# jbelyeu/unfazed

Measured on NVIDIA B200. Metric: DNMs phased/sec, higher is better.
Workload: dtype int32/u8 + f64 allele balance

## Files before the change

include/unfazed_sm100.h:

```cpp
#ifndef UNFAZED_SM100_H
#define UNFAZED_SM100_H

#include <stdint.h>

#ifdef __cplusplus
extern "C" {
#endif

#define UNFZ_ABI_VERSION 2

#define UNFZ_CLS_HET        0x01
#define UNFZ_CLS_CAND       0x02
#define UNFZ_CLS_ALT_IS_DAD 0x04
#define UNFZ_CLS_KID_ALT    0x08

#define UNFZ_MODE_READ    0
#define UNFZ_MODE_CNV_DEL 1
#define UNFZ_MODE_CNV_DUP 2
#define UNFZ_MODE_CNV_NA  3

#define UNFZ_RS_GOOD_CONC 0x01
#define UNFZ_RS_GOOD_DISC 0x02
#define UNFZ_RS_NONE_OK   0x04
#define UNFZ_RS_EXT_OK    0x08
#define UNFZ_RS_INS_OK    0x10
#define UNFZ_RS_HAS_MATE  0x20

#define UNFZ_KIND_SKIP  0
#define UNFZ_KIND_SNV   1
#define UNFZ_KIND_INDEL 2
#define UNFZ_KIND_SV    3

#define UNFZ_ORIGIN_NONE 0
#define UNFZ_ORIGIN_DAD  1
#define UNFZ_ORIGIN_MOM  2
#define UNFZ_ORIGIN_BOTH 3

#define UNFZ_EV_READBACKED        0x01
#define UNFZ_EV_ALLELE_BALANCE    0x02
#define UNFZ_EV_AMBIG_READBACKED  0x04
#define UNFZ_EV_AMBIG_ALLELE_BAL  0x08
#define UNFZ_EV_AMBIG_BOTH        0x10
#define UNFZ_EV_SEX_CHROM         0x20

typedef struct {
    int64_t         n_rows;
    int32_t         n_blocks;
    int32_t         _pad;
    const int64_t*  blk_off;
    const int32_t*  pos;
    const uint8_t*  ref;
    const uint8_t*  alt;
    const uint32_t* meta;
    const float*    rec;
    const int32_t*  dep;
} UnfzSiteCols;

typedef struct {
    int32_t  start;
    int32_t  tlen;
    int32_t  mate;
    uint32_t cigar_off;
    uint32_t qoff_lo;
    int32_t  l_seq;
    uint16_t flag;
    uint16_t n_cigar;
    uint8_t  mapq;
    uint8_t  aux;
    uint8_t  qoff_hi;
    uint8_t  pad;
} UnfzRead;

typedef struct {
    int64_t         n_reads;
    int32_t         n_blocks;
    int32_t         _pad;
    const int64_t*  blk_off;
    const int32_t*  blk_sblk;
    const double*   blk_cul;
    const UnfzRead* hdr;
    const int32_t*  start;
    const uint32_t* cigar;
    const uint32_t* lowq;
    const uint32_t* nmask;
    const uint8_t*  seq2;
    int64_t         n_qual;
    int64_t         n_cigar;
} UnfzReadCols;

typedef struct {
    int32_t  end;
    int32_t  fmark;
    uint16_t flags;
    uint16_t cnt;
    uint32_t hoff;
    int32_t  start;
    int32_t  mate;
    int32_t  row_lb;
    int32_t  _pad;
} UnfzReadSum;

typedef struct {
    double  ab_homref[2];
    double  ab_homalt[2];
    double  ab_het[2];
    double  min_gt_qual;
    int32_t min_depth;
    int32_t min_map_qual;
    int32_t readlen;
    int32_t ext_read_goal;
    int32_t no_extended;
    int32_t evidence_min_ratio;
    int32_t split_error_margin;
    int32_t _pad;
} UnfzParams;

typedef struct {
    int32_t sblk;
    int32_t lo_pos;
    int32_t hi_pos;
    int32_t mult;
    int32_t dnm;
    int32_t excl_lo;
    int32_t excl_hi;
    int32_t mode;
} UnfzSegIn;

typedef struct {
    int32_t pos;
    int32_t end;
    int32_t rblk;
    int32_t kind;
    int32_t seg_lo;
    int32_t seg_hi;
    int32_t ref_off;
    int32_t ref_len;
    int32_t alt_off;
    int32_t alt_len;
    int32_t cnv_entry;
    int32_t flags;
} UnfzDnm;

typedef struct {
    int32_t n_dad_sites, n_mom_sites;
    int32_t n_dad_reads, n_mom_reads;
    int32_t cnv_dad, cnv_mom;
    int32_t has_record;
    int32_t status;
} UnfzTally;

typedef struct {
    int32_t origin;
    int32_t evidence_count;
    int32_t evidence_types;
    int32_t emitted;
} UnfzCall;

typedef struct UnfzCtx UnfzCtx;

int         unfz_abi_version(void);
int         unfz_ctx_create(int device, UnfzCtx** out);
void        unfz_ctx_destroy(UnfzCtx* ctx);
const char* unfz_last_error(UnfzCtx* ctx);

int unfz_ctx_set_guard(UnfzCtx*, const int32_t* flag);
int unfz_check_caps(UnfzCtx*, int32_t k, const int64_t* const* h_totals, const int64_t* h_caps, int32_t* flag,
                    int64_t* actual, void* stream);

int64_t unfz_scan_work_bytes(int64_t n);
int unfz_exclusive_scan_i64(UnfzCtx*, const int64_t* in, int64_t* out, int64_t n, void* work, void* stream);
int unfz_exclusive_scan_u8_i32(UnfzCtx*, const uint8_t* in, int32_t* out, int64_t n, void* work, void* stream);
int unfz_exclusive_scan_u32(UnfzCtx*, const uint32_t* in, uint32_t* out , int64_t n, int64_t* total_out,
                            void* work, void* stream);
int unfz_exclusive_scan_rows_i64(UnfzCtx*, const int64_t* in, int64_t* out, int32_t n_rows, int64_t n, void* stream);

int unfz_window_search(UnfzCtx*, const UnfzSiteCols* sites, const UnfzSegIn* segs, int32_t n_segs,
                       int32_t* seg_row_lo, int64_t* seg_count, void* stream);

int unfz_classify_sites(UnfzCtx*, const UnfzSiteCols* sites, const UnfzSegIn* segs,
                        const int32_t* seg_row_lo, const int64_t* seg_pair_off, int32_t n_segs,
                        int64_t n_pairs, const UnfzParams* h_params, uint8_t* out_class, void* stream);

int unfz_compact_sites(UnfzCtx*, const UnfzDnm* dnms, int32_t n_dnms, const UnfzSegIn* segs,
                       const int32_t* seg_row_lo, const int64_t* seg_pair_off, const uint8_t* cls,
                       int32_t* het_list, int32_t* n_het, uint32_t* cand_list, int32_t* n_cand,
                       int32_t* cnv_dad, int32_t* cnv_mom, uint8_t* row_mark, void* stream);

int unfz_pack_site_rows(UnfzCtx*, int64_t n_rows, const int32_t* pos, const uint8_t* flag, const uint8_t* gt,
                        const float* gq, const int32_t* rd, const int32_t* ad, uint32_t* meta, float* rec,
                        int32_t* dep, void* stream);

int unfz_expand_nlist(UnfzCtx*, const UnfzReadCols* reads, UnfzRead* hdr_rw, uint32_t* nmask_rw,
                      const int64_t* nidx, int64_t n_idx, void* stream);
int unfz_read_starts(UnfzCtx*, const UnfzReadCols* reads, int32_t* start_rw, void* stream);

int32_t unfz_read_scan_tile_reads(int32_t max_l_seq);
int unfz_read_scan(UnfzCtx*, const UnfzReadCols* reads, const UnfzSiteCols* sites,
                   const int32_t* mark_prefix, const UnfzParams* h_params,
                   int32_t max_l_seq , UnfzReadSum* out,
                   int32_t* blk_maxspan ,
                   uint32_t* tile_tot ,
                   uint32_t* tile_info ,
                   void* stream);

int unfz_read_site_alleles(UnfzCtx*, const UnfzReadCols* reads, const UnfzSiteCols* sites,
                           const uint8_t* row_mark, const int32_t* mark_prefix,
                           const UnfzReadSum* rsum, const uint32_t* tile_base,
                           int32_t tile_reads, uint32_t* hits, const uint32_t* tile_info ,
                           void* stream);

int unfz_chain_size(UnfzCtx*, const UnfzDnm* dnms, int32_t n_dnms, const UnfzSegIn* segs,
                    const int64_t* seg_pair_off, const UnfzSiteCols* sites,
                    const UnfzReadCols* reads, const UnfzReadSum* rsum, const int32_t* blk_maxspan,
                    const int32_t* het_list, const int32_t* n_het, const uint32_t* cand_list,
                    const int32_t* n_cand, int32_t* win ,
                    int64_t* need,
                    int32_t* site_lo, int32_t* site_n ,
                    int32_t* seed_win , void* stream);

int unfz_chain_tally(UnfzCtx*, const UnfzDnm* dnms, int32_t n_dnms, const UnfzSegIn* segs,
                     const int64_t* seg_pair_off, const UnfzSiteCols* sites,
                     const UnfzReadCols* reads, const UnfzReadSum* rsum, const int32_t* blk_maxspan,
                     const uint32_t* hits, const uint32_t* hit_tile_base, int32_t hit_tile_reads,
                     const int32_t* mark_prefix,
                     const int32_t* het_list, const int32_t* n_het, const uint32_t* cand_list,
                     const int32_t* n_cand, const uint8_t* alleles, const int32_t* win,
                     const int32_t* site_lo, const int32_t* site_n, const int32_t* seed_win, const int64_t* off, const int64_t* h_totals ,
                     const UnfzParams* h_params, void* scratch, int64_t scratch_bytes,
                     uint8_t* slot_label, uint8_t* slot_evid, uint8_t* cand_evid,
                     UnfzTally* tally,
                     int64_t* ev_need ,
                     void* stream);

int unfz_evidence_lists(UnfzCtx*, const UnfzDnm* dnms, int32_t n_dnms, const int64_t* seg_pair_off,
                        const UnfzSiteCols* sites, const uint32_t* cand_list, const int32_t* n_cand,
                        const uint8_t* cand_evid, const int32_t* win, const int64_t* slot_off,
                        const uint8_t* slot_evid, const int64_t* ev_off, int32_t* ev_read_dad, int32_t* ev_read_mom,
                        int32_t* ev_pos_dad, int32_t* ev_pos_mom, void* stream);
int64_t unfz_chain_scratch_bytes(int64_t slots, int64_t incs, int64_t seeds, int64_t seed_incs,
                                 int64_t het_sites, int64_t cand_sites, int64_t n_dnms);

int64_t unfz_insert_size_work_bytes(void);
int unfz_insert_size_order_stats(UnfzCtx*, const UnfzReadCols* reads, const int64_t* h_first, const int64_t* h_count,
                                 int32_t n_ranges, int32_t readlen, const uint64_t* h_ranks, void* work,
                                 uint32_t* out, void* stream);

int unfz_summarize(UnfzCtx*, const UnfzDnm* dnms, int32_t n_dnms, const UnfzTally* tally,
                   const int32_t* cnv_dad, const int32_t* cnv_mom, const int32_t* n_cand,
                   const UnfzParams* h_params,
                   UnfzCall* calls_strict, UnfzCall* calls_ambiguous, void* stream);

typedef struct {
    const UnfzSiteCols* sites;
    const UnfzReadCols* reads;
    const UnfzParams*   h_params;
    const UnfzDnm*  dnms;     int32_t n_dnms;  int32_t n_segs;
    const UnfzSegIn* segs;    const uint8_t* alleles;
    int32_t max_l_seq;        int32_t tile_reads;
    int64_t n_tiles;
    int64_t cap_pairs, cap_hits, cap_chain[6];
    int32_t* seg_row_lo;  int64_t* seg_count;  int64_t* seg_pair_off;  void* scan_work;
    uint8_t* row_mark;    int32_t* mark_prefix;
    int32_t* guard;       int64_t* actual;
    int32_t* n_het;  int32_t* n_cand;  int32_t* cnv_dad;  int32_t* cnv_mom;
    UnfzTally* tally;  UnfzCall* calls_strict;  UnfzCall* calls_ambiguous;  int32_t* win;
    int32_t* blk_maxspan;  int64_t* need;  int64_t* off;
    UnfzReadSum* rsum;  uint32_t* tile_tot;  uint32_t* tile_base;  uint32_t* tile_info;
    uint8_t* cls;  int32_t* het_list;  uint32_t* cand_list;  int32_t* site_lo;  int32_t* site_n;  int32_t* seed_win;
    uint8_t* cand_evid;
    uint32_t* hits;  void* scratch;  int64_t scratch_bytes;  uint8_t* slot_label;  uint8_t* slot_evid;
    int64_t* ev_need;  int64_t* ev_off;  int32_t* ev_read_dad;  int32_t* ev_read_mom;  int32_t* ev_pos_dad;  int32_t* ev_pos_mom;
} UnfzBatch;
int unfz_run_batch(UnfzCtx*, const UnfzBatch* h_batch, void* stream);

typedef struct { void* ptr; int64_t bytes; } UnfzSpan;
int unfz_run_batch_graph(UnfzCtx*, const UnfzBatch* h_batch, const UnfzSpan* h_zero, int32_t n_zero,
                         void* h_dst, const void* d_src, int64_t d2h_bytes, void* stream);
int unfz_batch_struct_bytes(void);

#ifdef __cplusplus
}
#endif
#endif
```

unfazed_b200/_lib.py:

```python
from __future__ import annotations

import ctypes as C
import os

import numpy as np

_HERE = os.path.dirname(os.path.abspath(__file__))
LIB_PATH = os.environ.get("UNFZ_LIB") or os.path.join(_HERE, "libunfazed_sm100.so")

c_void_p, c_int32, c_int64, c_double = C.c_void_p, C.c_int32, C.c_int64, C.c_double


class SiteCols(C.Structure):
    _fields_ = [
        ("n_rows", c_int64), ("n_blocks", c_int32), ("_pad", c_int32),
        ("blk_off", c_void_p), ("pos", c_void_p), ("ref", c_void_p), ("alt", c_void_p),
        ("meta", c_void_p), ("rec", c_void_p), ("dep", c_void_p),
    ]


class ReadCols(C.Structure):
    _fields_ = [
        ("n_reads", c_int64), ("n_blocks", c_int32), ("_pad", c_int32),
        ("blk_off", c_void_p), ("blk_sblk", c_void_p), ("blk_cul", c_void_p),
        ("hdr", c_void_p), ("start", c_void_p), ("cigar", c_void_p), ("lowq", c_void_p), ("nmask", c_void_p), ("seq2", c_void_p),
        ("n_qual", c_int64), ("n_cigar", c_int64),
    ]


class Params(C.Structure):
    _fields_ = [
        ("ab_homref", c_double * 2), ("ab_homalt", c_double * 2), ("ab_het", c_double * 2),
        ("min_gt_qual", c_double),
        ("min_depth", c_int32), ("min_map_qual", c_int32), ("readlen", c_int32),
        ("ext_read_goal", c_int32), ("no_extended", c_int32), ("evidence_min_ratio", c_int32),
        ("split_error_margin", c_int32), ("_pad", c_int32),
    ]


class Batch(C.Structure):
    _fields_ = [
        ("sites", c_void_p), ("reads", c_void_p), ("h_params", c_void_p),
        ("dnms", c_void_p), ("n_dnms", c_int32), ("n_segs", c_int32),
        ("segs", c_void_p), ("alleles", c_void_p),
        ("max_l_seq", c_int32), ("tile_reads", c_int32),
        ("n_tiles", c_int64),
        ("cap_pairs", c_int64), ("cap_hits", c_int64), ("cap_chain", c_int64 * 6),
        ("seg_row_lo", c_void_p), ("seg_count", c_void_p), ("seg_pair_off", c_void_p), ("scan_work", c_void_p),
        ("row_mark", c_void_p), ("mark_prefix", c_void_p),
        ("guard", c_void_p), ("actual", c_void_p),
        ("n_het", c_void_p), ("n_cand", c_void_p), ("cnv_dad", c_void_p), ("cnv_mom", c_void_p),
        ("tally", c_void_p), ("calls_strict", c_void_p), ("calls_ambiguous", c_void_p), ("win", c_void_p),
        ("blk_maxspan", c_void_p), ("need", c_void_p), ("off", c_void_p),
        ("rsum", c_void_p), ("tile_tot", c_void_p), ("tile_base", c_void_p), ("tile_info", c_void_p),
        ("cls", c_void_p), ("het_list", c_void_p), ("cand_list", c_void_p), ("site_lo", c_void_p), ("site_n", c_void_p),
        ("seed_win", c_void_p), ("cand_evid", c_void_p),
        ("hits", c_void_p), ("scratch", c_void_p), ("scratch_bytes", c_int64), ("slot_label", c_void_p), ("slot_evid", c_void_p),
        ("ev_need", c_void_p), ("ev_off", c_void_p), ("ev_read_dad", c_void_p), ("ev_read_mom", c_void_p),
        ("ev_pos_dad", c_void_p), ("ev_pos_mom", c_void_p),
    ]


class Span(C.Structure):
    _fields_ = [("ptr", c_void_p), ("bytes", c_int64)]


SEG_DTYPE = np.dtype([
    ("sblk", "<i4"), ("lo_pos", "<i4"), ("hi_pos", "<i4"), ("mult", "<i4"),
    ("dnm", "<i4"), ("excl_lo", "<i4"), ("excl_hi", "<i4"), ("mode", "<i4"),
])
DNM_DTYPE = np.dtype([
    ("pos", "<i4"), ("end", "<i4"), ("rblk", "<i4"), ("kind", "<i4"), ("seg_lo", "<i4"), ("seg_hi", "<i4"),
    ("ref_off", "<i4"), ("ref_len", "<i4"), ("alt_off", "<i4"), ("alt_len", "<i4"),
    ("cnv_entry", "<i4"), ("flags", "<i4"),
])
TALLY_DTYPE = np.dtype([
    ("n_dad_sites", "<i4"), ("n_mom_sites", "<i4"), ("n_dad_reads", "<i4"), ("n_mom_reads", "<i4"),
    ("cnv_dad", "<i4"), ("cnv_mom", "<i4"), ("has_record", "<i4"), ("status", "<i4"),
])
CALL_DTYPE = np.dtype([("origin", "<i4"), ("evidence_count", "<i4"), ("evidence_types", "<i4"), ("emitted", "<i4")])
RSUM_DTYPE = np.dtype([("end", "<i4"), ("fmark", "<i4"), ("flags", "<u2"), ("cnt", "<u2"), ("hoff", "<u4"),
                       ("start", "<i4"), ("mate", "<i4"), ("row_lb", "<i4"), ("pad", "<i4")])
assert SEG_DTYPE.itemsize == 32 and DNM_DTYPE.itemsize == 48 and RSUM_DTYPE.itemsize == 32

CLS_HET, CLS_CAND, CLS_ALT_IS_DAD, CLS_KID_ALT = 1, 2, 4, 8
MODE_READ, MODE_CNV_DEL, MODE_CNV_DUP, MODE_CNV_NA = 0, 1, 2, 3
KIND_SKIP, KIND_SNV, KIND_INDEL, KIND_SV = 0, 1, 2, 3
ORIGIN_NONE, ORIGIN_DAD, ORIGIN_MOM, ORIGIN_BOTH = 0, 1, 2, 3
EV_READBACKED, EV_ALLELE_BALANCE, EV_AMBIG_READBACKED, EV_AMBIG_ALLELE_BAL, EV_AMBIG_BOTH, EV_SEX_CHROM = 1, 2, 4, 8, 16, 32
DNM_AUTOPHASE, DNM_AUTOPHASE_Y, DNM_SV_QUIRK, DNM_FALLBACK_FETCH = 1, 2, 4, 8
ABI_VERSION = 2
RS_GOOD_CONC, RS_GOOD_DISC, RS_NONE_OK, RS_EXT_OK, RS_INS_OK, RS_HAS_MATE = 1, 2, 4, 8, 16, 32

_P = c_void_p
SYMBOLS = {
    "unfz_abi_version": (C.c_int, []),
    "unfz_ctx_create": (C.c_int, [C.c_int, C.POINTER(_P)]),
    "unfz_ctx_destroy": (None, [_P]),
    "unfz_last_error": (C.c_char_p, [_P]),
    "unfz_ctx_set_guard": (C.c_int, [_P, _P]),
    "unfz_check_caps": (C.c_int, [_P, c_int32, _P, _P, _P, _P, _P]),
    "unfz_run_batch": (C.c_int, [_P, C.POINTER(Batch), _P]),
    "unfz_run_batch_graph": (C.c_int, [_P, C.POINTER(Batch), _P, c_int32, _P, _P, c_int64, _P]),
    "unfz_batch_struct_bytes": (C.c_int, []),
    "unfz_scan_work_bytes": (c_int64, [c_int64]),
    "unfz_exclusive_scan_i64": (C.c_int, [_P, _P, _P, c_int64, _P, _P]),
    "unfz_exclusive_scan_u8_i32": (C.c_int, [_P, _P, _P, c_int64, _P, _P]),
    "unfz_exclusive_scan_u32": (C.c_int, [_P, _P, _P, c_int64, _P, _P, _P]),
    "unfz_exclusive_scan_rows_i64": (C.c_int, [_P, _P, _P, c_int32, c_int64, _P]),
    "unfz_window_search": (C.c_int, [_P, C.POINTER(SiteCols), _P, c_int32, _P, _P, _P]),
    "unfz_classify_sites": (C.c_int, [_P, C.POINTER(SiteCols), _P, _P, _P, c_int32, c_int64, C.POINTER(Params), _P, _P]),
    "unfz_compact_sites": (C.c_int, [_P, _P, c_int32, _P, _P, _P, _P, _P, _P, _P, _P, _P, _P, _P, _P]),
    "unfz_pack_site_rows": (C.c_int, [_P, c_int64, _P, _P, _P, _P, _P, _P, _P, _P, _P, _P]),
    "unfz_expand_nlist": (C.c_int, [_P, C.POINTER(ReadCols), _P, _P, _P, c_int64, _P]),
    "unfz_read_scan_tile_reads": (c_int32, [c_int32]),
    "unfz_read_scan": (C.c_int, [_P, C.POINTER(ReadCols), C.POINTER(SiteCols), _P, C.POINTER(Params), c_int32, _P, _P, _P, _P, _P]),
    "unfz_read_site_alleles": (C.c_int, [_P, C.POINTER(ReadCols), C.POINTER(SiteCols), _P, _P, _P, _P, c_int32, _P, _P, _P]),
    "unfz_read_starts": (C.c_int, [_P, C.POINTER(ReadCols), _P, _P]),
    "unfz_chain_size": (C.c_int, [_P, _P, c_int32, _P, _P, C.POINTER(SiteCols), C.POINTER(ReadCols), _P, _P,
                                  _P, _P, _P, _P, _P, _P, _P, _P, _P, _P]),
    "unfz_chain_scratch_bytes": (c_int64, [c_int64] * 7),
    "unfz_chain_tally": (C.c_int, [_P, _P, c_int32, _P, _P, C.POINTER(SiteCols), C.POINTER(ReadCols), _P, _P, _P, _P, c_int32, _P,
                                   _P, _P, _P, _P, _P, _P, _P, _P, _P, _P, _P, C.POINTER(Params), _P, c_int64,
                                   _P, _P, _P, _P, _P, _P]),
    "unfz_evidence_lists": (C.c_int, [_P, _P, c_int32, _P, C.POINTER(SiteCols), _P, _P, _P, _P, _P, _P, _P, _P, _P, _P, _P, _P]),
    "unfz_insert_size_work_bytes": (c_int64, []),
    "unfz_insert_size_order_stats": (C.c_int, [_P, C.POINTER(ReadCols), _P, _P, c_int32, c_int32, _P, _P, _P, _P]),
    "unfz_summarize": (C.c_int, [_P, _P, c_int32, _P, _P, _P, _P, C.POINTER(Params), _P, _P, _P]),
}

_lib = None


class LibraryMissing(RuntimeError):
    pass


def load():
    global _lib
    if _lib is not None:
        return _lib
    if not os.path.exists(LIB_PATH):
        raise LibraryMissing(
            "%s not found: build it with `python -c 'import __graft_entry__ as g; g.build()'` "
            "or `make -C unfazed_b200/csrc`" % LIB_PATH)
    lib = C.CDLL(LIB_PATH)
    for name, (res, args) in SYMBOLS.items():
        fn = getattr(lib, name)
        fn.restype = res
        fn.argtypes = args
    if lib.unfz_abi_version() != ABI_VERSION:
        raise LibraryMissing("ABI version mismatch in %s" % LIB_PATH)
    if lib.unfz_batch_struct_bytes() != C.sizeof(Batch):
        raise LibraryMissing("UnfzBatch layout mismatch between %s and _lib.Batch" % LIB_PATH)
    _lib = lib
    return lib
```

unfazed_b200/csrc/abi.cu:

```cuda
#include <stdlib.h>

#include "common.cuh"

extern "C" int unfz_abi_version(void) { return UNFZ_ABI_VERSION; }

extern "C" int unfz_ctx_create(int device, UnfzCtx** out) {
    if (!out) return -1;
    *out = nullptr;
    int count = 0;
    if (cudaGetDeviceCount(&count) != cudaSuccess || device < 0 || device >= count) return -2;
    cudaDeviceProp prop;
    if (cudaGetDeviceProperties(&prop, device) != cudaSuccess) return -3;
    if (prop.major < 10) return -4;
    if (cudaSetDevice(device) != cudaSuccess) return -5;
    UnfzCtx* c = new UnfzCtx();
    c->device = device;
    c->sm_count = prop.multiProcessorCount;
    c->guard = nullptr;
    c->scan_smem_attr = 0;
    c->chain_carveout_set = false;
    c->cls_params = nullptr;
    c->cls_tab_dev = nullptr;
    memset(c->graphs, 0, sizeof(c->graphs));
    c->graph_tick = 0;
    c->err[0] = 0;
    *out = c;
    return 0;
}

extern "C" void unfz_ctx_destroy(UnfzCtx* ctx) {
    if (!ctx) return;
    for (auto& g : ctx->graphs)
        if (g.key) cudaGraphExecDestroy(g.exec);
    free(ctx->cls_params);
    if (ctx->cls_tab_dev) cudaFree(ctx->cls_tab_dev);
    delete ctx;
}

extern "C" const char* unfz_last_error(UnfzCtx* ctx) { return ctx ? ctx->err : "null context"; }

namespace {
struct CapArgs {
    const int64_t* totals[8];
    int64_t caps[8];
};
__global__ void check_caps_kernel(CapArgs a, int k, int32_t* flag, int64_t* actual) {
    const int i = threadIdx.x;
    if (i < k) {
        const int64_t v = *a.totals[i];
        actual[i] = v;
        if (v > a.caps[i]) atomicOr(flag, 1);
    }
}
}

extern "C" int unfz_ctx_set_guard(UnfzCtx* ctx, const int32_t* flag) {
    if (!ctx) return -1;
    ctx->guard = flag;
    return 0;
}

extern "C" int unfz_check_caps(UnfzCtx* ctx, int32_t k, const int64_t* const* totals, const int64_t* caps,
                               int32_t* flag, int64_t* actual, void* stream) {
    if (k < 0 || k > 8) return unfz_fail(ctx, -30, "unfz_check_caps: at most 8 totals");
    if (k == 0) return 0;
    CapArgs a;
    for (int i = 0; i < 8; ++i) { a.totals[i] = i < k ? totals[i] : nullptr; a.caps[i] = i < k ? caps[i] : 0; }
    check_caps_kernel<<<1, 32, 0, (cudaStream_t)stream>>>(a, k, flag, actual);
    UNFZ_LAUNCH_CHECK(ctx);
    return 0;
}

#define UNFZ_RC(expr) do { const int rc_ = (expr); if (rc_ != 0) { ctx->guard = nullptr; return rc_; } } while (0)

extern "C" int unfz_batch_struct_bytes(void) { return (int)sizeof(UnfzBatch); }

extern "C" int unfz_run_batch(UnfzCtx* ctx, const UnfzBatch* b, void* s) {
    if (!ctx || !b) return -1;
    const int32_t n = b->n_dnms, S = b->n_segs;
    const int64_t V = b->sites->n_rows;
    ctx->guard = b->guard;
    UNFZ_RC(unfz_window_search(ctx, b->sites, b->segs, S, b->seg_row_lo, b->seg_count, s));
    UNFZ_RC(unfz_exclusive_scan_i64(ctx, b->seg_count, b->seg_pair_off, S, b->scan_work, s));
    {
        const int64_t* t[1] = {b->seg_pair_off + S};
        const int64_t c[1] = {b->cap_pairs};
        UNFZ_RC(unfz_check_caps(ctx, 1, t, c, b->guard, b->actual, s));
    }
    UNFZ_RC(unfz_classify_sites(ctx, b->sites, b->segs, b->seg_row_lo, b->seg_pair_off, S, b->cap_pairs, b->h_params, b->cls, s));
    UNFZ_RC(unfz_compact_sites(ctx, b->dnms, n, b->segs, b->seg_row_lo, b->seg_pair_off, b->cls, b->het_list, b->n_het,
                               b->cand_list, b->n_cand, b->cnv_dad, b->cnv_mom, b->row_mark, s));
    UNFZ_RC(unfz_exclusive_scan_u8_i32(ctx, b->row_mark, b->mark_prefix, V, b->scan_work, s));
    if (b->reads != nullptr) {
        int64_t* total_hits = b->off + 6 * ((int64_t)n + 1);
        UNFZ_RC(unfz_read_scan(ctx, b->reads, b->sites, b->mark_prefix, b->h_params, b->max_l_seq, b->rsum,
                               b->blk_maxspan, b->tile_tot, b->tile_info, s));
        UNFZ_RC(unfz_exclusive_scan_u32(ctx, b->tile_tot, b->tile_base, b->n_tiles, total_hits, b->scan_work, s));
        UNFZ_RC(unfz_chain_size(ctx, b->dnms, n, b->segs, b->seg_pair_off, b->sites, b->reads, b->rsum, b->blk_maxspan,
                                b->het_list, b->n_het, b->cand_list, b->n_cand, b->win, b->need, b->site_lo, b->site_n,
                                b->seed_win, s));
        UNFZ_RC(unfz_exclusive_scan_rows_i64(ctx, b->need, b->off, 6, n, s));
        {
            const int64_t* t[7];
            int64_t c[7];
            for (int i = 0; i < 6; ++i) { t[i] = b->off + (int64_t)(i + 1) * (n + 1) - 1; c[i] = b->cap_chain[i]; }
            t[6] = total_hits;
            c[6] = b->cap_hits;
            UNFZ_RC(unfz_check_caps(ctx, 7, t, c, b->guard, b->actual + 1, s));
        }
        UNFZ_RC(unfz_read_site_alleles(ctx, b->reads, b->sites, b->row_mark, b->mark_prefix, b->rsum, b->tile_base,
                                       b->tile_reads, b->hits, b->tile_info, s));
        UNFZ_RC(unfz_chain_tally(ctx, b->dnms, n, b->segs, b->seg_pair_off, b->sites, b->reads, b->rsum, b->blk_maxspan,
                                 b->hits, b->tile_base, b->tile_reads, b->mark_prefix, b->het_list, b->n_het, b->cand_list,
                                 b->n_cand, b->alleles, b->win, b->site_lo, b->site_n, b->seed_win, b->off, b->cap_chain,
                                 b->h_params, b->scratch, b->scratch_bytes, b->slot_label, b->slot_evid, b->cand_evid,
                                 b->tally, b->ev_need, s));
        if (b->ev_need != nullptr) {
            UNFZ_RC(unfz_exclusive_scan_rows_i64(ctx, b->ev_need, b->ev_off, 4, n, s));
            UNFZ_RC(unfz_evidence_lists(ctx, b->dnms, n, b->seg_pair_off, b->sites, b->cand_list, b->n_cand, b->cand_evid,
                                        b->win, b->off, b->slot_evid, b->ev_off, b->ev_read_dad, b->ev_read_mom, b->ev_pos_dad,
                                        b->ev_pos_mom, s));
        }
    }
    UNFZ_RC(unfz_summarize(ctx, b->dnms, n, b->tally, b->cnv_dad, b->cnv_mom, b->n_cand, b->h_params, b->calls_strict,
                           b->calls_ambiguous, s));
    ctx->guard = nullptr;
    return 0;
}

static uint64_t fnv1a(uint64_t h, const void* p, size_t n) {
    const unsigned char* b = static_cast<const unsigned char*>(p);
    for (size_t i = 0; i < n; ++i) { h ^= b[i]; h *= 1099511628211ull; }
    return h;
}

extern "C" int unfz_run_batch_graph(UnfzCtx* ctx, const UnfzBatch* b, const UnfzSpan* zero, int32_t n_zero,
                                    void* h_dst, const void* d_src, int64_t d2h_bytes, void* stream) {
    if (!ctx || !b) return -1;
    cudaStream_t s = (cudaStream_t)stream;
    uint64_t key = 1469598103934665603ull;
    key = fnv1a(key, b, sizeof(*b));
    key = fnv1a(key, b->sites, sizeof(*b->sites));
    if (b->reads) key = fnv1a(key, b->reads, sizeof(*b->reads));
    key = fnv1a(key, b->h_params, sizeof(*b->h_params));
    key = fnv1a(key, zero, sizeof(UnfzSpan) * (size_t)(n_zero > 0 ? n_zero : 0));
    key = fnv1a(key, &h_dst, sizeof(h_dst));
    key = fnv1a(key, &d_src, sizeof(d_src));
    key = fnv1a(key, &d2h_bytes, sizeof(d2h_bytes));
    if (key == 0) key = 1;
    UnfzGraphSlot* slot = nullptr;
    UnfzGraphSlot* victim = nullptr;
    for (auto& g : ctx->graphs) {
        if (g.key == key) { slot = &g; break; }
        if (!victim || (victim->key != 0 && (g.key == 0 || g.tick < victim->tick))) victim = &g;
    }
    if (!slot) {
        cudaGraph_t graph = nullptr;
        { const int rc0 = unfz_classify_prepare(ctx, b->h_params); if (rc0) return rc0; }
        UNFZ_CHECK(ctx, cudaStreamBeginCapture(s, cudaStreamCaptureModeThreadLocal));
        int rc = 0;
        for (int i = 0; i < n_zero && rc == 0; ++i)
            if (zero[i].bytes > 0 && cudaMemsetAsync(zero[i].ptr, 0, (size_t)zero[i].bytes, s) != cudaSuccess) rc = -40;
        if (rc == 0) rc = unfz_run_batch(ctx, b, s);
        if (rc == 0 && d2h_bytes > 0 && cudaMemcpyAsync(h_dst, d_src, (size_t)d2h_bytes, cudaMemcpyDeviceToHost, s) != cudaSuccess) rc = -41;
        const cudaError_t e = cudaStreamEndCapture(s, &graph);
        if (rc != 0 || e != cudaSuccess) {
            if (graph) cudaGraphDestroy(graph);
            cudaGetLastError();
            return rc != 0 ? rc : unfz_fail(ctx, -42, "unfz_run_batch_graph: stream capture failed (legacy default stream?)");
        }
        cudaGraphExec_t exec = nullptr;
        const cudaError_t ei = cudaGraphInstantiate(&exec, graph, 0);
        cudaGraphDestroy(graph);
        if (ei != cudaSuccess) return unfz_fail(ctx, -43, cudaGetErrorString(ei));
        if (victim->key) cudaGraphExecDestroy(victim->exec);
        victim->key = key;
        victim->exec = exec;
        slot = victim;
    }
    slot->tick = ++ctx->graph_tick;
    UNFZ_CHECK(ctx, cudaGraphLaunch(slot->exec, s));
    return 0;
}
```

unfazed_b200/csrc/chain.cu:

```cuda
#include <stdlib.h>

#include <type_traits>

#include "common.cuh"

namespace {

constexpr unsigned long long KEY_NONE = ~0ull;
#ifndef UNFZ_CHAIN_WIDE_MIN_INC
#define UNFZ_CHAIN_WIDE_MIN_INC 2048
#endif
constexpr int CH_SMEM_SITES = 128;

struct __align__(16) SlotRec {
    unsigned long long key;
    int32_t dense;
    int32_t pad;
};

struct Scratch {
    SlotRec* slot;
    int32_t* inc_r; int32_t* inc_x; int32_t* inc_site; uint8_t* inc_al;
    int32_t* seed_e; uint8_t* seed_hap; uint32_t* seed_reg;
    int32_t* sinc_px; int32_t* sinc_site; uint32_t* sinc_sidx; uint8_t* sinc_al;
    int32_t* x_of; int32_t* prim;
    uint32_t* p_ord; int32_t* p_fpos; int32_t* p_tmp; unsigned long long* p_minkey; uint8_t* p_label;
    int32_t* adj; int32_t* adj_off; int32_t* front0; int32_t* front1;
    int32_t* spos; uint8_t* sref; uint8_t* salt; int32_t* site_off; int32_t* cand_off;
    unsigned long long* bestkey; int32_t* site_cnt; int32_t* site_base; int32_t* active;
    int32_t* cpos;
    int32_t* meta;
};

struct ChainArgs {
    const UnfzDnm* dnms; int32_t n_dnms;
    const UnfzSegIn* segs; const int64_t* seg_pair_off;
    UnfzSiteCols sites; UnfzReadCols reads;
    const UnfzReadSum* rsum; const int32_t* blk_maxspan; const uint32_t* hits; const int32_t* mp;
    const int32_t* het_list; const int32_t* n_het; const uint32_t* cand_list; const int32_t* n_cand;
    const uint8_t* alleles; const int32_t* win; const int64_t* off;
    int32_t split_margin;
    const uint32_t* hit_tile_base; int32_t hit_tile_reads;
    const int32_t* site_lo; const int32_t* site_n; const int32_t* seed_win;
    int32_t readlen, ext_goal, no_extended;
    uint8_t* slot_label; uint8_t* slot_evid; uint8_t* cand_evid; UnfzTally* tally;
    int64_t* ev_need;
    const int32_t* guard;
    Scratch S;
};

#ifdef CH_PREFETCH
__device__ __forceinline__ void prefetch_l2(const void* p) { asm volatile("prefetch.global.L2 [%0];" ::"l"(p)); }
#endif

__device__ __forceinline__ int32_t rs_start(const UnfzReadSum* __restrict__ S, int64_t r) { return __ldg(&S[r].start); }
__device__ __forceinline__ int32_t rs_mate(const UnfzReadSum* __restrict__ S, int64_t r) { return __ldg(&S[r].mate); }

__device__ __forceinline__ int64_t lb_start(const int32_t* __restrict__ R, int64_t lo, int64_t hi, int64_t v) {
    while (lo < hi) {
        const int64_t mid = (lo + hi) >> 1;
        if ((int64_t)__ldg(R + mid) < v) lo = mid + 1; else hi = mid;
    }
    return lo;
}

__device__ __forceinline__ int cigar_qpos2(const uint32_t* __restrict__ cg, int n_cigar, int32_t start, int32_t p) {
    int32_t cur = start;
    int q = 0;
    for (int k = 0; k < n_cigar; ++k) {
        const uint32_t w = __ldg(cg + k);
        const uint32_t op = w & 15u;
        const int32_t ln = (int32_t)(w >> 4);
        if (op == 0 || op == 7 || op == 8) {
            if (p < cur + ln) return p >= cur ? q + (p - cur) : -1;
            cur += ln; q += ln;
        } else if (op == 1 || op == 4) {
            q += ln;
        } else if (op == 2 || op == 3) {
            if (p < cur + ln) return -1;
            cur += ln;
        }
    }
    return -1;
}

__device__ __forceinline__ uint32_t plane_bit(const uint32_t* __restrict__ plane, int64_t g) {
    return (__ldg(plane + (g >> 5)) >> (g & 31)) & 1u;
}
__device__ __forceinline__ char base_char(const UnfzReadCols& R, int64_t g) {
    const uint32_t code = (__ldg(R.seq2 + (g >> 2)) >> ((g & 3) << 1)) & 3u;
    if (plane_bit(R.nmask, g)) return code == 0 ? 'N' : '?';
    return "ACGT"[code];
}
__device__ __forceinline__ char hit_char(uint32_t w) {
    const uint32_t code = (w >> 24) & 3u;
    if (w & (0x80u << 16)) return code == 0 ? 'N' : '?';
    return "ACGT"[code];
}

__device__ __forceinline__ uint32_t hit_lookup(const ChainArgs& A, int64_t e, int64_t row) {
    const UnfzReadSum s = load_rsum(A.rsum + e);
    const int mp = __ldg(A.mp + row);
    const uint32_t tb = __ldg(A.hit_tile_base + (uint32_t)e / (uint32_t)A.hit_tile_reads);
    const int k = mp - s.fmark;
    if (k < 0 || k >= (int)s.cnt) return 0;
    return __ldg(A.hits + (int64_t)tb + s.hoff + k);
}

__device__ bool pair_ok(const ChainArgs& A, int64_t r, bool ext) {
    const UnfzReadSum s = load_rsum(A.rsum + r);
    uint32_t need = UNFZ_RS_GOOD_CONC | UNFZ_RS_INS_OK | UNFZ_RS_HAS_MATE | UNFZ_RS_NONE_OK;
    if (ext) need |= UNFZ_RS_EXT_OK;
    const bool ok_r = (s.flags & need) == need;
    const int64_t m = ok_r ? (int64_t)s.mate : r;
    const UnfzReadSum sm = load_rsum(A.rsum + m);
    const uint32_t needm = UNFZ_RS_GOOD_CONC | UNFZ_RS_NONE_OK;
    const int32_t r0 = s.start, r1 = s.end, m0 = sm.start, m1 = sm.end;
    return ok_r && (sm.flags & needm) == needm && !((m0 <= r0 && r0 <= m1) || (m0 <= r1 && r1 <= m1));
}

struct QPos { int q; int l_seq; int64_t g0; int32_t mate; };
__device__ __forceinline__ QPos qpos_of(const ChainArgs& A, int64_t e, int32_t p) {
    const UnfzRead h = load_read(A.reads.hdr + e);
    QPos o;
    if (h.aux & 0x40u) o.q = (p >= h.start && p < h.start + h.l_seq) ? (int)(p - h.start) : -1;
    else o.q = cigar_qpos2(A.reads.cigar + h.cigar_off, h.n_cigar, h.start, p);
    o.l_seq = h.l_seq;
    o.g0 = read_qoff(h);
    o.mate = h.mate;
    return o;
}

__device__ int seed_snv(const ChainArgs& A, const UnfzDnm& dn, int64_t r) {
    QPos h = qpos_of(A, r, dn.pos);
    int q = h.q;
    if (q < 0) {
        h = qpos_of(A, h.mate, dn.pos);
        q = h.q;
        if (q < 0) return 0;
    }
    if (q < 4 || q > A.readlen - 4) return 0;
    const int n = dn.ref_len > dn.alt_len ? dn.ref_len : dn.alt_len;
    if (!(h.l_seq > q + n)) return 0;
    const int64_t g = h.g0 + q;
    bool is_ref = true;
    for (int i = 0; i < dn.ref_len; ++i)
        if (base_char(A.reads, g + i) != (char)A.alleles[dn.ref_off + i]) { is_ref = false; break; }
    if (is_ref) return 1;
    bool is_alt = true;
    for (int i = 0; i < dn.alt_len; ++i)
        if (base_char(A.reads, g + i) != (char)A.alleles[dn.alt_off + i]) { is_alt = false; break; }
    return is_alt ? 2 : 0;
}

__device__ int seed_indel(const ChainArgs& A, const UnfzDnm& dn, int64_t r) {
    const UnfzRead h = load_read(A.reads.hdr + r);
    const uint32_t* cg = A.reads.cigar + h.cigar_off;
    const bool simple = (h.aux & 0x40u) != 0;
    const int q = simple ? ((dn.pos >= h.start && dn.pos < h.start + h.l_seq) ? (int)(dn.pos - h.start) : -1)
                         : cigar_qpos2(cg, h.n_cigar, h.start, dn.pos);
    if (q < 0) return 0;
    const int n = dn.ref_len > dn.alt_len ? dn.ref_len : dn.alt_len;
    const int64_t g0 = read_qoff(h);
    for (int i = q; i < q + n && i < h.l_seq; ++i)
        if (plane_bit(A.reads.lowq, g0 + i)) return 0;
    if (simple) return (7 < q && q < h.l_seq - 7) ? 1 : 0;
    bool has_id = false;
    int64_t eo = 0, npos = 0;
    for (int k = 0; k < h.n_cigar; ++k) {
        const uint32_t w = __ldg(cg + k);
        const uint32_t op = w & 15u;
        const int64_t ln = w >> 4;
        if ((op == 1 || op == 2) && eo < (int64_t)q + n && eo + ln > q) has_id = true;
        eo += ln;
        if (op == 0 || op == 1 || op == 4 || op == 7 || op == 8) npos += ln;
    }
    if (has_id) return 2;
    if (7 < q && q < npos - 7) return 1;
    return 0;
}


__device__ bool sv_bad_ends(const uint32_t* __restrict__ cg, int n) {
    int s_m = 0, left = 10;
    for (int k = 0; k < n && left > 0; ++k) {
        const uint32_t w = __ldg(cg + k);
        const int take = min(left, (int)(w >> 4));
        if ((w & 15u) == 0 || (w & 15u) == 7) s_m += take;
        left -= take;
    }
    int e_m = 0;
    left = 10;
    for (int k = n - 1; k >= 0 && left > 0; --k) {
        const uint32_t w = __ldg(cg + k);
        const int take = min(left, (int)(w >> 4));
        if ((w & 15u) == 0 || (w & 15u) == 7) e_m += take;
        left -= take;
    }
    return e_m < 7 && s_m < 7;
}

__device__ bool sv_goodok(const ChainArgs& A, int64_t r) {
    const UnfzReadSum s = load_rsum(A.rsum + r);
    const uint32_t need = UNFZ_RS_GOOD_DISC | UNFZ_RS_HAS_MATE;
    if ((s.flags & need) != need) return false;
    const int64_t m = rs_mate(A.rsum, r);
    return (load_rsum(A.rsum + m).flags & UNFZ_RS_GOOD_DISC) != 0;
}

__device__ bool sv_banned(const ChainArgs& A, int64_t r) {
    if (!sv_goodok(A, r)) return false;
    const UnfzRead h = load_read(A.reads.hdr + r);
    return sv_bad_ends(A.reads.cigar + h.cigar_off, h.n_cigar);
}

__device__ int sv_support(const ChainArgs& A, const UnfzDnm& dn, int64_t r, int64_t position, double cul) {
    const UnfzRead h = load_read(A.reads.hdr + r);
    const UnfzReadSum s = load_rsum(A.rsum + r);
    const int64_t r0 = h.start, r1 = s.end;
    if (h.aux & 2u) {
        const int64_t em = A.split_margin;
        if ((position - em <= r0 && r0 <= position + em) || (position - em <= r1 && r1 <= position + em)) return 1;
        return 0;
    }
    long long ins = (long long)h.tlen - 2ll * A.readlen;
    if (ins < 0) ins = -ins;
    const double var_len = fabs((double)dn.end - (double)dn.pos);
    if ((double)ins > cul) {
        const double ratio = fabs(var_len / (double)ins);
        if (0.7 < ratio && ratio < 1.3) {
            const int64_t m0 = rs_start(A.rsum, h.mate);
            const int64_t left0 = min(m0, r0), right0 = max(m0, r0);
            const int64_t w = (int64_t)cul;
            if ((dn.pos - w) < left0 && left0 < (dn.pos + w) && (dn.end - w) < right0 && right0 < (dn.end + w)) return 2;
            return 0;
        }
    }
    const uint32_t* cg = A.reads.cigar + h.cigar_off;
    int k = cigar_qpos2(cg, h.n_cigar, h.start, (int32_t)position);
    if (k < 0) k = cigar_qpos2(cg, h.n_cigar, h.start, (int32_t)position - 1);
    if (k < 0) k = cigar_qpos2(cg, h.n_cigar, h.start, (int32_t)position + 1);
    if (k < 0) return 0;
    int64_t npos = 0, lead = 0, trail = 0;
    bool seen = false;
    for (int i = 0; i < h.n_cigar; ++i) {
        const uint32_t w = __ldg(cg + i);
        const uint32_t op = w & 15u;
        const int64_t ln = w >> 4;
        if (op == 0 || op == 7 || op == 8) { npos += ln; seen = true; trail = 0; }
        else if (op == 1 || op == 4) { npos += ln; if (!seen) lead += ln; else trail += ln; }
    }
    if (k < 2 || k > npos - 4) return 0;
    const int64_t first_al = lead, last_al = npos - 1 - trail;
    const bool before_none = first_al >= k - 1;
    const bool after_none = (k + 1 < npos) && last_al <= k;
    return (before_none || after_none) ? 2 : 0;
}


__device__ int bisect_pivot(const int32_t* __restrict__ spos, int n, int32_t start, int32_t end) {
    int lo = 0, hi = n - 1, plo = -1, phi = -1;
    while (hi > -1) {
        if (lo > hi) break;
        if (lo == plo && hi == phi) break;
        plo = lo; phi = hi;
        const int mid = (hi + lo) / 2;
        const int32_t x = spos[mid];
        if (start <= x && x < end) return mid;
        else if (x > start) hi = mid - 1;
        else if (x < start) lo = mid + 1;
    }
    return -1;
}

__device__ uint8_t allele_info(const ChainArgs& A, const Scratch& S, int64_t e0, int64_t row, char ref, char alt) {
    if (e0 < 0) return 0;
    const int64_t e1 = rs_mate(A.rsum, e0);
    const uint32_t h0 = hit_lookup(A, e0, row);
    uint32_t h = h0;
    if (!(h0 & 0xffffu)) {
        if (e1 < 0) return 0;
        h = hit_lookup(A, e1, row);
        if (!(h & 0xffffu)) return 0;
    }
    const int q = (int)(h & 0xffffu) - 1;
    if (q < 4 || q > A.readlen - 4) return 0;
    if (!(h & (1u << 26))) return 0;
    const char c = hit_char(h);
    const uint8_t code = c == ref ? 1 : (c == alt ? 2 : 0);
    if (!code) return 0;
    uint8_t out = code;
    if ((h0 & 0xffffu) && !(h0 & (1u << 16))) out |= code << 2;
    return out;
}

#ifdef CH_DEBUG
__device__ unsigned long long g_ch_dbg[16];
#define CH_MARK(i) do { if (threadIdx.x == 0) { const long long t_ = clock64(); atomicAdd(&g_ch_dbg[i], (unsigned long long)(t_ - ch_t0)); ch_t0 = t_; } } while (0)
#else
#define CH_MARK(i)
#endif

#ifndef CH_THREADS_N
#define CH_THREADS_N 128
#endif
#ifndef CH_MINB
#define CH_MINB 16
#endif
#ifndef CH_BFS_MINB
#define CH_BFS_MINB 8
#endif
#define CH_NS cta_small
#include "chain_cta.inc"
#undef CH_NS
#undef CH_THREADS_N
#undef CH_MINB
#undef CH_BFS_MINB
#define CH_NS cta_wide
#define CH_THREADS_N 512
#define CH_MINB 4
#define CH_BFS_MINB 2
#include "chain_cta.inc"
#undef CH_NS
#undef CH_THREADS_N
#undef CH_MINB
#undef CH_BFS_MINB


__global__ void __launch_bounds__(128)
evidence_lists_kernel(const UnfzDnm* __restrict__ dnms, int32_t n_dnms, const int64_t* __restrict__ seg_pair_off,
                      const int32_t* __restrict__ site_pos, const uint32_t* __restrict__ cand_list,
                      const int32_t* __restrict__ n_cand, const uint8_t* __restrict__ cand_evid,
                      const int32_t* __restrict__ win, const int64_t* __restrict__ slot_off,
                      const uint8_t* __restrict__ slot_evid, const int64_t* __restrict__ ev_off,
                      int32_t* __restrict__ ev_read_dad, int32_t* __restrict__ ev_read_mom,
                      int32_t* __restrict__ ev_pos_dad, int32_t* __restrict__ ev_pos_mom,
                      const int32_t* __restrict__ guard) {
    UNFZ_GUARD(guard);
    const int lane = threadIdx.x & 31;
    const int d = (blockIdx.x * blockDim.x + threadIdx.x) >> 5;
    if (d >= n_dnms) return;
    const unsigned below = (1u << lane) - 1u;
    const int64_t n1 = (int64_t)n_dnms + 1;
    int64_t kd = ev_off[d], km = ev_off[n1 + d];
    if (ev_off[d + 1] > kd || ev_off[n1 + d + 1] > km) {
        const int64_t nd = n_dnms;
        const int64_t a_lo = win[d], a_hi = win[nd + d], b_lo = win[2 * nd + d], b_hi = win[3 * nd + d];
        const int na = (int)(a_hi - a_lo), W = na + (int)(b_hi - b_lo);
        const uint8_t* ev = slot_evid + slot_off[d];
        for (int x0 = 0; x0 < W; x0 += 32) {
            const int x = x0 + lane;
            const uint8_t e = x < W ? ev[x] : 0;
            const int32_t r = (int32_t)(x < na ? a_lo + x : b_lo + (x - na));
            const unsigned bd = __ballot_sync(0xffffffffu, e & 1), bm = __ballot_sync(0xffffffffu, e & 2);
            if (e & 1) ev_read_dad[kd + __popc(bd & below)] = r;
            if (e & 2) ev_read_mom[km + __popc(bm & below)] = r;
            kd += __popc(bd);
            km += __popc(bm);
        }
    }
    kd = ev_off[2 * n1 + d];
    km = ev_off[3 * n1 + d];
    if (ev_off[2 * n1 + d + 1] > kd || ev_off[3 * n1 + d + 1] > km) {
        const UnfzDnm dn = dnms[d];
        const int64_t lbase = seg_pair_off[dn.seg_lo];
        const int nc = n_cand[d];
        for (int j0 = 0; j0 < nc; j0 += 32) {
            const int j = j0 + lane;
            const uint8_t e = j < nc ? cand_evid[lbase + j] : 0;
            const int32_t p = e ? __ldg(site_pos + (int64_t)(cand_list[lbase + j] & 0x3fffffffu)) : 0;
            const unsigned bd = __ballot_sync(0xffffffffu, e & 1), bm = __ballot_sync(0xffffffffu, e & 2);
            if (e & 1) ev_pos_dad[kd + __popc(bd & below)] = p;
            if (e & 2) ev_pos_mom[km + __popc(bm & below)] = p;
            kd += __popc(bd);
            km += __popc(bm);
        }
    }
}

__device__ __forceinline__ int64_t warp_sum64(int64_t v) {
#pragma unroll
    for (int o = 16; o > 0; o >>= 1) v += __shfl_xor_sync(0xffffffffu, v, o);
    return v;
}
__device__ __forceinline__ int64_t warp_min64(int64_t v) {
#pragma unroll
    for (int o = 16; o > 0; o >>= 1) v = min(v, __shfl_xor_sync(0xffffffffu, v, o));
    return v;
}
__device__ __forceinline__ int64_t warp_max64(int64_t v) {
#pragma unroll
    for (int o = 16; o > 0; o >>= 1) v = max(v, __shfl_xor_sync(0xffffffffu, v, o));
    return v;
}

__device__ __forceinline__ int64_t warp_lb_start(const int32_t* __restrict__ R, int64_t lo, int64_t hi, int64_t v, int lane) {
    while (hi - lo > 32) {
        const int64_t step = (hi - lo + 32) / 33;
        const int64_t i = lo + (int64_t)(lane + 1) * step - 1;
        const bool lt = i < hi && (int64_t)__ldg(R + i) < v;
        const int k = __popc(__ballot_sync(0xffffffffu, lt));
        const int64_t nhi = k < 32 ? min(hi, lo + (int64_t)(k + 1) * step - 1) : hi;
        lo += (int64_t)k * step;
        hi = nhi;
    }
    const bool lt = lo + lane < hi && (int64_t)__ldg(R + lo + lane) < v;
    return lo + __popc(__ballot_sync(0xffffffffu, lt));
}
__device__ __forceinline__ int64_t lb_start_near(const int32_t* __restrict__ R, int64_t lo, int64_t hi, int64_t v) {
    int64_t step = 32, top = lo;
    while (top + step < hi && (int64_t)__ldg(R + top + step - 1) < v) { top += step; step <<= 1; }
    return lb_start(R, top, min(hi, top + step), v);
}

constexpr int CS_HP = 128;

__global__ void __launch_bounds__(128)
chain_size_kernel(const UnfzDnm* __restrict__ dnms, int32_t n_dnms, const int64_t* __restrict__ seg_pair_off,
                  UnfzSiteCols sites, UnfzReadCols reads, const UnfzReadSum* __restrict__ rsum,
                  const int32_t* __restrict__ blk_maxspan, const int32_t* __restrict__ het_list,
                  const int32_t* __restrict__ n_het, const uint32_t* __restrict__ cand_list,
                  const int32_t* __restrict__ n_cand, int32_t* __restrict__ win, int64_t* __restrict__ need,
                  int32_t* __restrict__ site_lo, int32_t* __restrict__ site_n, int32_t* __restrict__ seed_win,
                  const int32_t* __restrict__ guard) {
    UNFZ_GUARD(guard);
    __shared__ int32_t s_hp[4][CS_HP];
    const int lane = threadIdx.x & 31;
    const int d = (blockIdx.x * blockDim.x + threadIdx.x) >> 5;
    if (d >= n_dnms) return;
    int32_t* hp = s_hp[threadIdx.x >> 5];
    const UnfzDnm dn = dnms[d];
    int64_t nd[6] = {0, 0, 0, 0, 0, 0};
    int64_t a_lo = 0, a_hi = 0, b_lo = 0, b_hi = 0;
    const int nh = n_het[d], nc = n_cand[d];
    if (!(dn.kind == UNFZ_KIND_SKIP || dn.rblk < 0 || nc <= 0 || dn.seg_hi <= dn.seg_lo)) {
        const int64_t lbase = seg_pair_off[dn.seg_lo];
        const int32_t* H = het_list + lbase;
        const int64_t blk_lo = reads.blk_off[dn.rblk], blk_hi = reads.blk_off[dn.rblk + 1];
        const int64_t maxspan = blk_maxspan[dn.rblk];
        const double cul = reads.blk_cul[dn.rblk];
        const bool sv = dn.kind == UNFZ_KIND_SV;
        int64_t sa_lo, sa_hi, sb_lo = 0, sb_hi = 0;
        if (sv) {
            const double l0 = (double)dn.pos - cul, l1 = (double)dn.end - cul;
            sa_lo = l0 > 0.0 ? (int64_t)l0 : 0; sa_hi = (int64_t)((double)dn.pos + cul);
            sb_lo = l1 > 0.0 ? (int64_t)l1 : 0; sb_hi = (int64_t)((double)dn.end + cul);
        } else {
            sa_lo = (dn.flags & 8) ? (int64_t)dn.pos : (int64_t)dn.pos - 1;
            sa_hi = (int64_t)dn.pos + 1;
        }
        const int64_t mid = sv ? ((int64_t)dn.pos + (int64_t)dn.end) / 2 : (int64_t)1 << 40;
        int64_t minA = sa_lo, maxA = sa_hi, minB = sv ? sb_lo : ((int64_t)1 << 40), maxB = sv ? sb_hi : -1;
        int64_t incs = 0;
        for (int i = lane; i < nh; i += 32) {
            const int64_t p = sites.pos[H[i]];
            if (i < CS_HP) hp[i] = (int32_t)p;
            if (p < mid) { minA = min(minA, p); maxA = max(maxA, p + 1); }
            else { minB = min(minB, p); maxB = max(maxB, p + 1); }
            const int64_t a = lb_start(reads.start, blk_lo, blk_hi, p - maxspan + 1);
            const int64_t b = lb_start_near(reads.start, a, blk_hi, p + 1);
            site_lo[lbase + i] = (int32_t)(a - blk_lo);
            site_n[lbase + i] = (int32_t)(b - a);
            incs += b - a;
        }
        minA = warp_min64(minA); maxA = warp_max64(maxA); minB = warp_min64(minB); maxB = warp_max64(maxB);
        nd[1] = warp_sum64(incs);
        __syncwarp();
        a_lo = warp_lb_start(reads.start, blk_lo, blk_hi, minA - maxspan + 1, lane);
        a_hi = warp_lb_start(reads.start, a_lo, blk_hi, maxA, lane);
        if (maxB > minB) {
            b_lo = warp_lb_start(reads.start, blk_lo, blk_hi, minB - maxspan + 1, lane);
            b_hi = warp_lb_start(reads.start, b_lo, blk_hi, maxB, lane);
            if (b_lo <= a_hi) { a_hi = max(a_hi, b_hi); a_lo = min(a_lo, b_lo); b_lo = b_hi = 0; }
        }
        nd[0] = ((a_hi - a_lo) + (b_hi - b_lo) + 3) & ~(int64_t)3;
        int64_t seeds = 0, sincs = 0;
        for (int wdx = 0; wdx < (sv ? 2 : 1); ++wdx) {
            const int64_t flo = wdx ? sb_lo : sa_lo, fhi = wdx ? sb_hi : sa_hi;
            const int64_t a = warp_lb_start(reads.start, blk_lo, blk_hi, flo - maxspan + 1, lane);
            const int64_t b = warp_lb_start(reads.start, a, blk_hi, fhi, lane);
            if (lane == 0) { seed_win[4 * (int64_t)d + 2 * wdx] = (int32_t)a; seed_win[4 * (int64_t)d + 2 * wdx + 1] = (int32_t)b; }
            seeds += 2 * (b - a);
            for (int64_t r = a + lane; r < b; r += 32) {
                const int64_t ents[2] = {r, (int64_t)rsum[r].mate};
                for (int t = 0; t < 2; ++t) {
                    const int64_t e = ents[t];
                    if (e < 0) continue;
                    const int64_t st = rsum[e].start, en = rsum[e].end;
                    int l = 0, h = nh;
                    int u;
                    if (nh <= CS_HP) {
                        while (l < h) { const int m2 = (l + h) >> 1; if (hp[m2] < st) l = m2 + 1; else h = m2; }
                        u = l; h = nh;
                        while (u < h) { const int m2 = (u + h) >> 1; if (hp[m2] <= en) u = m2 + 1; else h = m2; }
                    } else {
                        while (l < h) { const int m2 = (l + h) >> 1; if (sites.pos[H[m2]] < st) l = m2 + 1; else h = m2; }
                        u = l; h = nh;
                        while (u < h) { const int m2 = (u + h) >> 1; if (sites.pos[H[m2]] <= en) u = m2 + 1; else h = m2; }
                    }
                    sincs += u - l;
                }
            }
        }
        nd[2] = seeds;
        nd[3] = warp_sum64(sincs);
        nd[4] = nh;
        nd[5] = nc;
    }
    if (lane == 0) {
        win[d] = (int32_t)a_lo; win[(int64_t)n_dnms + d] = (int32_t)a_hi;
        win[2 * (int64_t)n_dnms + d] = (int32_t)b_lo; win[3 * (int64_t)n_dnms + d] = (int32_t)b_hi;
        for (int k = 0; k < 6; ++k) need[(int64_t)k * n_dnms + d] = nd[k];
    }
}

__device__ UnfzCall summarize_one(const UnfzDnm& dn, int nd_reads, int nm_reads, int nd_sites, int nm_sites,
                                  int cd, int cm, bool has_read_rec, bool has_cnv_rec, int ratio, bool include_ambiguous) {
    UnfzCall c;
    c.origin = UNFZ_ORIGIN_NONE; c.evidence_count = 0; c.evidence_types = 0; c.emitted = 0;
    const bool autoph = dn.flags & 1;
    const bool sv_quirk = dn.flags & 4;
    if (autoph && !sv_quirk) {
        c.origin = (dn.flags & 2) ? UNFZ_ORIGIN_DAD : UNFZ_ORIGIN_MOM;
        c.evidence_count = 1;
        c.evidence_types = UNFZ_EV_SEX_CHROM;
        c.emitted = 1;
        return c;
    }
    if (!autoph && !has_read_rec && !has_cnv_rec) return c;
    if (sv_quirk) { nd_reads = nm_reads = nd_sites = nm_sites = 0; cd = cm = 2; }
    if (!has_read_rec && !sv_quirk) nd_reads = nm_reads = nd_sites = nm_sites = 0;
    if (!has_cnv_rec && !sv_quirk) cd = cm = 0;
    int origin = UNFZ_ORIGIN_NONE, count = 0, types = 0;
    bool ambig = false;
    if (nd_reads > 0 && nd_reads >= ratio * nm_reads) { origin = UNFZ_ORIGIN_DAD; count = nd_sites; types |= UNFZ_EV_READBACKED; }
    else if (nm_reads > 0 && nm_reads >= ratio * nd_reads) { origin = UNFZ_ORIGIN_MOM; count = nm_sites; types |= UNFZ_EV_READBACKED; }
    else if (nd_reads > 0 && nm_reads > 0) { origin = UNFZ_ORIGIN_BOTH; count = nd_reads + nm_reads; types |= UNFZ_EV_AMBIG_READBACKED; ambig = true; }
    if (cd > 0 && cd >= ratio * cm) {
        if (origin == UNFZ_ORIGIN_MOM && !(types & UNFZ_EV_READBACKED)) {
            origin = UNFZ_ORIGIN_NONE; count += cd + cm; types = UNFZ_EV_AMBIG_BOTH; ambig = true;
        } else {
            origin = UNFZ_ORIGIN_DAD; count = cd;
            if (types & UNFZ_EV_AMBIG_READBACKED) { types &= ~UNFZ_EV_AMBIG_READBACKED; ambig = false; }
            types |= UNFZ_EV_ALLELE_BALANCE;
        }
    } else if (cm > 0 && cm >= ratio * cd) {
        if (origin == UNFZ_ORIGIN_DAD && !(types & UNFZ_EV_READBACKED)) {
            origin = UNFZ_ORIGIN_NONE; count += cd + cm; types = UNFZ_EV_AMBIG_BOTH; ambig = true;
        } else {
            origin = UNFZ_ORIGIN_MOM; count = cm;
            if (types & UNFZ_EV_AMBIG_READBACKED) types &= ~UNFZ_EV_AMBIG_READBACKED;
            types |= UNFZ_EV_ALLELE_BALANCE;
        }
    } else if ((cd + cm) > 0 && !(types & UNFZ_EV_READBACKED)) {
        origin = UNFZ_ORIGIN_NONE; count += cd + cm; types |= UNFZ_EV_AMBIG_ALLELE_BAL; ambig = true;
    }
    c.origin = origin; c.evidence_count = count; c.evidence_types = types;
    c.emitted = ((origin == UNFZ_ORIGIN_NONE || ambig) && !include_ambiguous) ? 0 : 1;
    return c;
}

__global__ void summarize_kernel(const UnfzDnm* __restrict__ dnms, int32_t n_dnms, const UnfzTally* __restrict__ tally,
                                 const int32_t* __restrict__ cnv_dad, const int32_t* __restrict__ cnv_mom,
                                 const int32_t* __restrict__ n_cand, int ratio, UnfzCall* __restrict__ strict,
                                 UnfzCall* __restrict__ ambiguous) {
    const int d = blockIdx.x * blockDim.x + threadIdx.x;
    if (d >= n_dnms) return;
    const UnfzDnm dn = dnms[d];
    const UnfzTally t = tally[d];
    int cd = 0, cm = 0;
    bool has_cnv = false;
    if (dn.cnv_entry >= 0) {
        cd = cnv_dad[dn.cnv_entry];
        cm = cnv_mom[dn.cnv_entry];
        has_cnv = n_cand[dn.cnv_entry] > 0;
    }
    strict[d] = summarize_one(dn, t.n_dad_reads, t.n_mom_reads, t.n_dad_sites, t.n_mom_sites, cd, cm,
                              t.has_record != 0, has_cnv, ratio, false);
    ambiguous[d] = summarize_one(dn, t.n_dad_reads, t.n_mom_reads, t.n_dad_sites, t.n_mom_sites, cd, cm,
                                 t.has_record != 0, has_cnv, ratio, true);
}

template <typename T>
char* carve(char*& p, int64_t n) {
    char* out = p;
    p += ((n * (int64_t)sizeof(T)) + 15) & ~(int64_t)15;
    return out;
}

Scratch carve_all(char* base, int64_t slots, int64_t incs, int64_t seeds, int64_t sincs, int64_t hets, int64_t cands,
                  int64_t n_dnms, int64_t* total) {
    Scratch S;
    char* p = base;
    const int64_t pairs = incs + seeds, adjs = incs + sincs;
    S.slot = (SlotRec*)carve<SlotRec>(p, slots);
    S.p_minkey = (unsigned long long*)carve<unsigned long long>(p, pairs);
    S.inc_r = (int32_t*)carve<int32_t>(p, incs); S.inc_x = (int32_t*)carve<int32_t>(p, incs);
    S.inc_site = (int32_t*)carve<int32_t>(p, incs); S.inc_al = (uint8_t*)carve<uint8_t>(p, incs);
    S.seed_e = (int32_t*)carve<int32_t>(p, seeds); S.seed_hap = (uint8_t*)carve<uint8_t>(p, seeds);
    S.seed_reg = (uint32_t*)carve<uint32_t>(p, seeds);
    S.sinc_px = (int32_t*)carve<int32_t>(p, sincs); S.sinc_site = (int32_t*)carve<int32_t>(p, sincs);
    S.sinc_sidx = (uint32_t*)carve<uint32_t>(p, sincs); S.sinc_al = (uint8_t*)carve<uint8_t>(p, sincs);
    S.x_of = (int32_t*)carve<int32_t>(p, pairs); S.prim = (int32_t*)carve<int32_t>(p, pairs);
    S.p_ord = (uint32_t*)carve<uint32_t>(p, pairs); S.p_fpos = (int32_t*)carve<int32_t>(p, pairs);
    S.p_tmp = (int32_t*)carve<int32_t>(p, pairs); S.p_label = (uint8_t*)carve<uint8_t>(p, pairs);
    S.adj = (int32_t*)carve<int32_t>(p, adjs); S.adj_off = (int32_t*)carve<int32_t>(p, pairs + 2 * n_dnms + 2);
    S.front0 = (int32_t*)carve<int32_t>(p, pairs); S.front1 = (int32_t*)carve<int32_t>(p, pairs);
    S.spos = (int32_t*)carve<int32_t>(p, hets); S.sref = (uint8_t*)carve<uint8_t>(p, hets);
    S.salt = (uint8_t*)carve<uint8_t>(p, hets); S.site_off = (int32_t*)carve<int32_t>(p, hets + n_dnms + 1);
    S.cand_off = (int32_t*)carve<int32_t>(p, hets + n_dnms + 1);
    S.bestkey = (unsigned long long*)carve<unsigned long long>(p, hets);
    S.site_cnt = (int32_t*)carve<int32_t>(p, hets); S.site_base = (int32_t*)carve<int32_t>(p, hets);
    S.active = (int32_t*)carve<int32_t>(p, hets);
    S.cpos = (int32_t*)carve<int32_t>(p, cands);
    S.meta = (int32_t*)carve<int32_t>(p, n_dnms * 8);
    *total = (int64_t)(p - base);
    return S;
}

}

extern "C" int64_t unfz_chain_scratch_bytes(int64_t slots, int64_t incs, int64_t seeds, int64_t seed_incs,
                                            int64_t het_sites, int64_t cand_sites, int64_t n_dnms) {
    int64_t total = 0;
    carve_all(nullptr, slots, incs, seeds, seed_incs, het_sites, cand_sites, n_dnms, &total);
    return total + 256;
}

extern "C" int unfz_chain_size(UnfzCtx* ctx, const UnfzDnm* dnms, int32_t n_dnms, const UnfzSegIn* segs,
                               const int64_t* seg_pair_off, const UnfzSiteCols* sites, const UnfzReadCols* reads,
                               const UnfzReadSum* rsum, const int32_t* blk_maxspan, const int32_t* het_list,
                               const int32_t* n_het, const uint32_t* cand_list, const int32_t* n_cand,
                               int32_t* win, int64_t* need, int32_t* site_lo, int32_t* site_n, int32_t* seed_win,
                               void* stream) {
    (void)segs;
    if (n_dnms <= 0) return 0;
    chain_size_kernel<<<(n_dnms + 3) / 4, 128, 0, (cudaStream_t)stream>>>(
        dnms, n_dnms, seg_pair_off, *sites, *reads, rsum, blk_maxspan, het_list, n_het, cand_list, n_cand, win, need,
        site_lo, site_n, seed_win, ctx->guard);
    UNFZ_LAUNCH_CHECK(ctx);
    return 0;
}

#ifdef CH_DEBUG
extern "C" int unfz_debug_chain(unsigned long long* out16) {
    cudaDeviceSynchronize();
    cudaMemcpyFromSymbol(out16, g_ch_dbg, sizeof(g_ch_dbg));
    unsigned long long z[16] = {0};
    cudaMemcpyToSymbol(g_ch_dbg, z, sizeof(z));
    return 0;
}
#endif

extern "C" int unfz_chain_tally(UnfzCtx* ctx, const UnfzDnm* dnms, int32_t n_dnms, const UnfzSegIn* segs,
                                const int64_t* seg_pair_off, const UnfzSiteCols* sites, const UnfzReadCols* reads,
                                const UnfzReadSum* rsum, const int32_t* blk_maxspan, const uint32_t* hits,
                                const uint32_t* hit_tile_base, int32_t hit_tile_reads, const int32_t* mark_prefix, const int32_t* het_list, const int32_t* n_het,
                                const uint32_t* cand_list, const int32_t* n_cand, const uint8_t* alleles,
                                const int32_t* win, const int32_t* site_lo, const int32_t* site_n, const int32_t* seed_win,
                                const int64_t* off, const int64_t* h_totals, const UnfzParams* hp, void* scratch, int64_t scratch_bytes,
                                uint8_t* slot_label, uint8_t* slot_evid, uint8_t* cand_evid, UnfzTally* tally,
                                int64_t* ev_need, void* stream) {
    if (n_dnms <= 0) return 0;
    ChainArgs A;
    A.ev_need = ev_need;
    A.dnms = dnms; A.n_dnms = n_dnms; A.segs = segs; A.seg_pair_off = seg_pair_off;
    A.sites = *sites; A.reads = *reads; A.rsum = rsum; A.blk_maxspan = blk_maxspan; A.hits = hits; A.mp = mark_prefix;
    A.het_list = het_list; A.n_het = n_het; A.cand_list = cand_list; A.n_cand = n_cand; A.alleles = alleles;
    A.win = win; A.off = off; A.split_margin = hp->split_error_margin;
    A.hit_tile_base = hit_tile_base; A.hit_tile_reads = hit_tile_reads;
    A.site_lo = site_lo; A.site_n = site_n; A.seed_win = seed_win;
    A.readlen = hp->readlen;
    A.ext_goal = hp->ext_read_goal;
    A.no_extended = hp->no_extended;
    A.slot_label = slot_label; A.slot_evid = slot_evid; A.cand_evid = cand_evid; A.tally = tally;
    int64_t total = 0;
    uintptr_t base = ((uintptr_t)scratch + 255) & ~(uintptr_t)255;
    A.S = carve_all((char*)base, h_totals[0], h_totals[1], h_totals[2], h_totals[3], h_totals[4], h_totals[5], n_dnms, &total);
    if ((int64_t)(base - (uintptr_t)scratch) + total > scratch_bytes) return unfz_fail(ctx, -20, "chain scratch too small");
    A.guard = ctx->guard;
    if (!ctx->chain_carveout_set) {
        UNFZ_CHECK(ctx, cudaFuncSetAttribute(cta_small::chain_bfs_kernel, cudaFuncAttributePreferredSharedMemoryCarveout, 100));
        UNFZ_CHECK(ctx, cudaFuncSetAttribute(cta_wide::chain_bfs_kernel, cudaFuncAttributePreferredSharedMemoryCarveout, 100));
        ctx->chain_carveout_set = true;
    }
    bool wide = h_totals[1] / n_dnms >= UNFZ_CHAIN_WIDE_MIN_INC;
    if (const char* force = getenv("UNFZ_CHAIN_SHAPE")) wide = force[0] == 'w' ? true : (force[0] == 's' ? false : wide);
    if (wide) {
        cta_wide::chain_setup_kernel<<<n_dnms, cta_wide::CH_THREADS, 0, (cudaStream_t)stream>>>(A);
        UNFZ_LAUNCH_CHECK(ctx);
        cta_wide::chain_bfs_kernel<<<n_dnms, cta_wide::CH_THREADS, 0, (cudaStream_t)stream>>>(A);
        UNFZ_LAUNCH_CHECK(ctx);
        cta_wide::chain_evidence_kernel<<<n_dnms, cta_wide::CH_THREADS, 0, (cudaStream_t)stream>>>(A);
        UNFZ_LAUNCH_CHECK(ctx);
        return 0;
    }
    cta_small::chain_setup_kernel<<<n_dnms, cta_small::CH_THREADS, 0, (cudaStream_t)stream>>>(A);
    UNFZ_LAUNCH_CHECK(ctx);
    cta_small::chain_bfs_kernel<<<n_dnms, cta_small::CH_THREADS, 0, (cudaStream_t)stream>>>(A);
    UNFZ_LAUNCH_CHECK(ctx);
    cta_small::chain_evidence_kernel<<<n_dnms, cta_small::CH_THREADS, 0, (cudaStream_t)stream>>>(A);
    UNFZ_LAUNCH_CHECK(ctx);
    return 0;
}

extern "C" int unfz_evidence_lists(UnfzCtx* ctx, const UnfzDnm* dnms, int32_t n_dnms, const int64_t* seg_pair_off,
                                   const UnfzSiteCols* sites, const uint32_t* cand_list, const int32_t* n_cand,
                                   const uint8_t* cand_evid, const int32_t* win, const int64_t* slot_off,
                                   const uint8_t* slot_evid, const int64_t* ev_off, int32_t* ev_read_dad, int32_t* ev_read_mom,
                                   int32_t* ev_pos_dad, int32_t* ev_pos_mom, void* stream) {
    if (n_dnms <= 0) return 0;
    evidence_lists_kernel<<<(n_dnms + 3) / 4, 128, 0, (cudaStream_t)stream>>>(
        dnms, n_dnms, seg_pair_off, sites->pos, cand_list, n_cand, cand_evid, win, slot_off, slot_evid, ev_off,
        ev_read_dad, ev_read_mom, ev_pos_dad, ev_pos_mom, ctx->guard);
    UNFZ_LAUNCH_CHECK(ctx);
    return 0;
}

extern "C" int unfz_summarize(UnfzCtx* ctx, const UnfzDnm* dnms, int32_t n_dnms, const UnfzTally* tally,
                              const int32_t* cnv_dad, const int32_t* cnv_mom, const int32_t* n_cand,
                              const UnfzParams* hp, UnfzCall* calls_strict, UnfzCall* calls_ambiguous, void* stream) {
    if (n_dnms <= 0) return 0;
    summarize_kernel<<<(n_dnms + 127) / 128, 128, 0, (cudaStream_t)stream>>>(
        dnms, n_dnms, tally, cnv_dad, cnv_mom, n_cand, hp->evidence_min_ratio, calls_strict, calls_ambiguous);
    UNFZ_LAUNCH_CHECK(ctx);
    return 0;
}
```

unfazed_b200/csrc/chain_cta.inc:

```
namespace CH_NS {
constexpr int CH_THREADS = CH_THREADS_N;
constexpr int CH_WARPS = CH_THREADS / 32;
__device__ __forceinline__ int block_prefix(bool flag, int* total) {
    __shared__ int wsum[CH_WARPS];
    const unsigned b = __ballot_sync(0xffffffffu, flag);
    const int lane = threadIdx.x & 31, w = threadIdx.x >> 5;
    if (lane == 0) wsum[w] = __popc(b);
    __syncthreads();
    int base = 0, tot = 0;
#pragma unroll
    for (int i = 0; i < CH_WARPS; ++i) { if (i < w) base += wsum[i]; tot += wsum[i]; }
    __syncthreads();
    *total = tot;
    return base + __popc(b & ((1u << lane) - 1u));
}

__device__ __forceinline__ int block_prefix_sum(int v, int* total) {
    __shared__ int wsum3[CH_WARPS];
    const int lane = threadIdx.x & 31, w = threadIdx.x >> 5;
    int x = v;
#pragma unroll
    for (int o = 1; o < 32; o <<= 1) { const int y = __shfl_up_sync(0xffffffffu, x, o); if (lane >= o) x += y; }
    if (lane == 31) wsum3[w] = x;
    __syncthreads();
    int base = 0, tot = 0;
#pragma unroll
    for (int i = 0; i < CH_WARPS; ++i) { if (i < w) base += wsum3[i]; tot += wsum3[i]; }
    __syncthreads();
    *total = tot;
    return base + x - v;
}

__device__ __forceinline__ int block_sum(int v) {
    __shared__ int wsum2[CH_WARPS];
#pragma unroll
    for (int o = 16; o > 0; o >>= 1) v += __shfl_xor_sync(0xffffffffu, v, o);
    if ((threadIdx.x & 31) == 0) wsum2[threadIdx.x >> 5] = v;
    __syncthreads();
    int tot = 0;
#pragma unroll
    for (int i = 0; i < CH_WARPS; ++i) tot += wsum2[i];
    __syncthreads();
    return tot;
}

template <typename PT, typename ST>
struct BfsView {
    uint32_t* ord; int32_t* fpos; int32_t* tmp; unsigned long long* minkey; uint8_t* label;
    PT* inc_px; ST* inc_site; uint8_t* inc_al;
    PT* sinc_px; ST* sinc_site; uint32_t* sinc_sidx; uint8_t* sinc_al;
    PT* adj; PT* adj_off;
    PT* front[2];
    const int32_t* spos; const int32_t* site_off; unsigned long long* bestkey; int32_t* site_cnt; int32_t* site_base;
    ST* active;
};

template <typename PT, typename ST>
__device__ void bfs_levels(const BfsView<PT, ST>& V, int nh, int n_inc, int n_front0) {
    __shared__ int s_nact, s_nnext;
    const int tid = threadIdx.x, lane = tid & 31, warp = tid >> 5;
    int n_front = n_front0;
    PT* fcur = V.front[0];
    PT* fnext = V.front[1];
    for (;;) {
        for (int i = tid; i < nh; i += CH_THREADS) V.bestkey[i] = KEY_NONE;
        if (tid == 0) { s_nact = 0; s_nnext = 0; }
        __syncthreads();
        for (int f = tid; f < n_front; f += CH_THREADS) {
            const int p = (int)fcur[f];
            const uint8_t fh = (V.label[p] & 2) ? 2 : 1;
            const unsigned long long okey = (unsigned long long)V.ord[p] << 36;
            const int32_t fp = V.fpos[p];
            const int q1 = (int)V.adj_off[p + 1];
            for (int q = (int)V.adj_off[p]; q < q1; ++q) {
                const int e = (int)V.adj[q];
                const bool sd = e >= n_inc;
                const int kk = sd ? e - n_inc : e;
                const int i = sd ? (int)V.sinc_site[kk] : (int)V.inc_site[kk];
                if (V.spos[i] == fp) continue;
                const uint8_t al = sd ? V.sinc_al[kk] : V.inc_al[kk];
                const uint32_t sidx = sd ? V.sinc_sidx[kk] : (uint32_t)i;
                atomicMin(V.bestkey + i, okey | ((unsigned long long)sidx << 4) | (unsigned long long)((fh << 2) | (al & 3)));
            }
        }
        __syncthreads();
        for (int i = tid; i < nh; i += CH_THREADS)
            if (V.bestkey[i] != KEY_NONE) V.active[atomicAdd(&s_nact, 1)] = (ST)i;
        __syncthreads();
        const int n_act = s_nact;
        if (n_act == 0) break;
        for (int a = warp; a < n_act; a += CH_WARPS) {
            const int i = (int)V.active[a];
            const unsigned long long bk = V.bestkey[i];
            const int k1 = V.site_off[i + 1];
            for (int k = V.site_off[i] + lane; k < k1; k += 32) {
                const int p = (int)V.inc_px[k];
                if (V.label[p] == 0 && (V.inc_al[k] >> 2)) atomicMin(V.minkey + p, bk);
            }
        }
        __syncthreads();
        for (int a = warp; a < n_act; a += CH_WARPS) {
            const int i = (int)V.active[a];
            const unsigned long long bk = V.bestkey[i];
            const int k0 = V.site_off[i], k1 = V.site_off[i + 1];
            int cnt = 0;
            for (int kb = k0; kb < k1; kb += 32) {
                const int k = kb + lane;
                bool claim = false;
                int p = 0;
                uint8_t ta = 0;
                if (k < k1) {
                    p = (int)V.inc_px[k];
                    ta = V.inc_al[k] >> 2;
                    claim = V.label[p] == 0 && ta && V.minkey[p] == bk;
                }
                const unsigned b = __ballot_sync(0xffffffffu, claim);
                if (claim) {
                    const uint8_t fh = (uint8_t)((bk >> 2) & 3), fa = (uint8_t)(bk & 3);
                    const uint8_t nh_ = (ta == fa) ? fh : (uint8_t)(3 - fh);
                    V.tmp[p] = (i << 8) | (nh_ << 4) | 1;
                    V.ord[p] = (uint32_t)(cnt + __popc(b & ((1u << lane) - 1u)));
                }
                cnt += __popc(b);
            }
            if (lane == 0) V.site_cnt[i] = cnt;
        }
        __syncthreads();
        int assigned = 0;
        for (int a = tid; a < n_act; a += CH_THREADS) {
            const int i = (int)V.active[a];
            const int c = V.site_cnt[i];
            int base = 0;
            if (c > 0) {
                const unsigned long long bk = V.bestkey[i];
                for (int b = 0; b < n_act; ++b) {
                    const int j = (int)V.active[b];
                    if (V.site_cnt[j] > 0 && V.bestkey[j] < bk) base += V.site_cnt[j];
                }
            }
            V.site_base[i] = base;
            assigned += c;
        }
        assigned = block_sum(assigned);
        if (assigned == 0) break;
        for (int a = warp; a < n_act; a += CH_WARPS) {
            const int i = (int)V.active[a];
            const unsigned long long bk = V.bestkey[i];
            const int k1 = V.site_off[i + 1];
            for (int k = V.site_off[i] + lane; k < k1; k += 32) {
                const int p = (int)V.inc_px[k];
                if (V.label[p] != 0) continue;
                const int t = V.tmp[p];
                if (!(t & 1)) { V.minkey[p] = KEY_NONE; continue; }
                if ((t >> 8) != i || V.minkey[p] != bk || !(V.inc_al[k] >> 2)) continue;
                const uint8_t nhap = (t >> 4) & 3;
                V.ord[p] = ((nhap == 1 ? 0u : 1u) << 24) | ((uint32_t)V.site_base[i] + V.ord[p]);
                V.fpos[p] = V.spos[i];
                V.tmp[p] = 0;
                V.label[p] = nhap;
                fnext[atomicAdd(&s_nnext, 1)] = (PT)p;
            }
        }
        __syncthreads();
        n_front = s_nnext;
        { PT* t_ = fcur; fcur = fnext; fnext = t_; }
        __syncthreads();
    }
    __syncthreads();
}

constexpr int META_INTS = 8;

__global__ void __launch_bounds__(CH_THREADS, CH_MINB)
chain_setup_kernel(ChainArgs A) {
    UNFZ_GUARD(A.guard);
#ifdef CH_DEBUG
    long long ch_t0 = clock64();
#endif
    const int d = blockIdx.x;
    const int tid = threadIdx.x, lane = tid & 31, warp = tid >> 5;
    const UnfzDnm dn = A.dnms[d];
    const Scratch& S0 = A.S;

    UnfzTally T;
    T.n_dad_sites = T.n_mom_sites = T.n_dad_reads = T.n_mom_reads = 0;
    T.cnv_dad = T.cnv_mom = 0;
    T.has_record = 0;
    T.status = 0;
    const int nh = A.n_het[d], nc = A.n_cand[d];
    if (dn.kind == UNFZ_KIND_SKIP || dn.rblk < 0 || nc <= 0 || dn.seg_hi <= dn.seg_lo) {
        if (tid == 0) {
            A.tally[d] = T;
            if (A.ev_need) for (int q = 0; q < 4; ++q) A.ev_need[(int64_t)q * A.n_dnms + d] = 0;
            S0.meta[(int64_t)d * META_INTS] = -1;
        }
        return;
    }
    const int64_t lbase = A.seg_pair_off[dn.seg_lo];
    const int32_t* H = A.het_list + lbase;
    const uint32_t* C = A.cand_list + lbase;
    const int64_t* off = A.off;
    const int64_t n1 = (int64_t)A.n_dnms + 1;
    const int64_t o_slot = off[0 * n1 + d], o_inc = off[1 * n1 + d], o_seed = off[2 * n1 + d];
    const int64_t o_sinc = off[3 * n1 + d], o_het = off[4 * n1 + d], o_cand = off[5 * n1 + d];
    const int64_t cap_inc = off[1 * n1 + d + 1] - o_inc, cap_seed = off[2 * n1 + d + 1] - o_seed;
    const int64_t cap_sinc = off[3 * n1 + d + 1] - o_sinc;
    const int64_t o_pair = o_inc + o_seed, o_adj = o_inc + o_sinc;

    SlotRec* rec = S0.slot + o_slot;
    int32_t* inc_r = S0.inc_r + o_inc; int32_t* inc_x = S0.inc_x + o_inc; int32_t* inc_site = S0.inc_site + o_inc;
    int32_t* seed_e = S0.seed_e + o_seed; uint8_t* seed_hap = S0.seed_hap + o_seed; uint32_t* seed_reg = S0.seed_reg + o_seed;
    int32_t* x_of = S0.x_of + o_pair; int32_t* prim = S0.prim + o_pair;
    __shared__ int32_t sh_spos[CH_SMEM_SITES], sh_site_off[CH_SMEM_SITES + 1], sh_cand_off[CH_SMEM_SITES + 1];
    __shared__ int32_t sh_site_cnt[CH_SMEM_SITES], sh_site_base[CH_SMEM_SITES];
    __shared__ uint8_t sh_sref[CH_SMEM_SITES], sh_salt[CH_SMEM_SITES];
    const bool small_sites = nh <= CH_SMEM_SITES;
    int32_t* spos = small_sites ? sh_spos : S0.spos + o_het;
    uint8_t* sref = small_sites ? sh_sref : S0.sref + o_het;
    uint8_t* salt = small_sites ? sh_salt : S0.salt + o_het;
    int32_t* site_off = small_sites ? sh_site_off : S0.site_off + o_het + d;
    int32_t* cand_off = small_sites ? sh_cand_off : S0.cand_off + o_het + d;
    int32_t* site_cnt = small_sites ? sh_site_cnt : S0.site_cnt + o_het;
    int32_t* site_base = small_sites ? sh_site_base : S0.site_base + o_het;
    int32_t* cpos = S0.cpos + o_cand;

    const UnfzReadCols& R = A.reads;
    const int64_t blk_lo = R.blk_off[dn.rblk];
    const int64_t nd_ = A.n_dnms;
    const int64_t a_lo = A.win[d], a_hi = A.win[nd_ + d], b_lo = A.win[2 * nd_ + d], b_hi = A.win[3 * nd_ + d];
    auto slot_of = [&](int64_t r) -> int {
        if (r >= a_lo && r < a_hi) return (int)(r - a_lo);
        if (r >= b_lo && r < b_hi) return (int)((a_hi - a_lo) + (r - b_lo));
        return -1;
    };
    auto canon = [&](int64_t r) -> int {
        const int64_t m = rs_mate(A.rsum, r);
        const int sr = slot_of(r), sm = m >= 0 ? slot_of(m) : -1;
        if (sr < 0) return sm;
        if (sm < 0) return sr;
        return m < r ? sm : sr;
    };
    const double cul = R.blk_cul[dn.rblk];

    auto init_slot = [&](int x) { *reinterpret_cast<int4*>(rec + x) = make_int4(0, 0, -1, 0); };
#ifdef CH_PREFETCH
    {
        const char* p0 = reinterpret_cast<const char*>(A.rsum + a_lo);
        const char* p1 = reinterpret_cast<const char*>(A.rsum + a_hi);
        for (const char* q = p0 + (size_t)tid * 128; q < p1; q += (size_t)CH_THREADS * 128) prefetch_l2(q);
        p0 = reinterpret_cast<const char*>(R.hdr + a_lo);
        p1 = reinterpret_cast<const char*>(R.hdr + a_hi);
        for (const char* q = p0 + (size_t)tid * 128; q < p1; q += (size_t)CH_THREADS * 128) prefetch_l2(q);
        if (b_hi > b_lo) {
            p0 = reinterpret_cast<const char*>(A.rsum + b_lo);
            p1 = reinterpret_cast<const char*>(A.rsum + b_hi);
            for (const char* q = p0 + (size_t)tid * 128; q < p1; q += (size_t)CH_THREADS * 128) prefetch_l2(q);
            p0 = reinterpret_cast<const char*>(R.hdr + b_lo);
            p1 = reinterpret_cast<const char*>(R.hdr + b_hi);
            for (const char* q = p0 + (size_t)tid * 128; q < p1; q += (size_t)CH_THREADS * 128) prefetch_l2(q);
        }
    }
#endif
    for (int i = tid; i < nh; i += CH_THREADS) {
        const int64_t row = H[i];
        spos[i] = __ldg(A.sites.pos + row);
        sref[i] = __ldg(A.sites.ref + row);
        salt[i] = __ldg(A.sites.alt + row);
    }
    for (int j = tid; j < nc; j += CH_THREADS) {
        cpos[j] = __ldg(A.sites.pos + (int64_t)(C[j] & 0x3fffffffu));
    }
    __syncthreads();

    CH_MARK(0);
    int n_seed = 0;
    if (dn.kind == UNFZ_KIND_SNV || dn.kind == UNFZ_KIND_INDEL) {
        const int64_t flo = (dn.flags & 8) ? (int64_t)dn.pos : (int64_t)dn.pos - 1;
        const int64_t lo = A.seed_win[4 * (int64_t)d], hi = A.seed_win[4 * (int64_t)d + 1];
        for (int64_t base = lo; base < hi; base += CH_THREADS) {
            const int64_t r = base + tid;
            int hap = 0;
            if (r < hi && (int64_t)A.rsum[r].end > flo && pair_ok(A, r, false))
                hap = dn.kind == UNFZ_KIND_SNV ? seed_snv(A, dn, r) : seed_indel(A, dn, r);
            int tot;
            const int k = n_seed + 2 * block_prefix(hap != 0, &tot);
            if (hap && k + 1 < cap_seed) {
                seed_e[k] = (int32_t)r; seed_hap[k] = (uint8_t)hap;
                seed_e[k + 1] = rs_mate(A.rsum, r); seed_hap[k + 1] = (uint8_t)hap;
            }
            n_seed += 2 * tot;
        }
        if (n_seed > cap_seed) { n_seed = (int)cap_seed & ~1; T.status |= 1; }
    } else if (dn.kind == UNFZ_KIND_SV) {
        int64_t e_lo = 0, e_hi = 0, e_flo = 0, e_fhi = 0;
        for (int wdx = 0; wdx < 2; ++wdx) {
            const int64_t position = wdx == 0 ? dn.pos : dn.end;
            const double dlo = (double)position - cul;
            const int64_t flo = dlo > 0.0 ? (int64_t)dlo : 0;
            const int64_t fhi = (int64_t)((double)position + cul);
            const int64_t lo = A.seed_win[4 * (int64_t)d + 2 * wdx], hi = A.seed_win[4 * (int64_t)d + 2 * wdx + 1];
            if (wdx == 1) { e_lo = lo; e_hi = hi; e_flo = flo; e_fhi = fhi; }
            for (int64_t base = lo; base < hi; base += CH_THREADS) {
                const int64_t r = base + tid;
                int sup = 0;
                if (r < hi && (int64_t)A.rsum[r].end > flo && sv_goodok(A, r)) {
                    const UnfzRead h = load_read(R.hdr + r);
                    const int64_t m = h.mate;
                    const bool skip = m < r && m >= lo && (int64_t)A.rsum[m].end > flo && sv_banned(A, m);
                    if (!skip && !sv_bad_ends(R.cigar + h.cigar_off, h.n_cigar)) sup = sv_support(A, dn, r, position, cul);
                }
                int tot;
                const int k = n_seed + 2 * block_prefix(sup != 0, &tot);
                if (sup && k + 1 < cap_seed) {
                    const int32_t m = rs_mate(A.rsum, r);
                    seed_e[k] = sup == 1 ? (int32_t)r : m; seed_hap[k] = 2;
                    seed_e[k + 1] = sup == 1 ? m : (int32_t)r; seed_hap[k + 1] = 2;
                }
                n_seed += 2 * tot;
            }
        }
        if (n_seed > cap_seed) { n_seed = (int)cap_seed & ~1; T.status |= 1; }
        __syncthreads();
        int kept = 0;
        for (int base = 0; base < n_seed; base += CH_THREADS) {
            const int k = base + tid;
            bool keep = false;
            int32_t e = 0;
            if (k < n_seed) {
                e = seed_e[k];
                const int64_t m = rs_mate(A.rsum, e);
                auto in_end_fetch = [&](int64_t z) {
                    return z >= e_lo && z < e_hi && (int64_t)A.rsum[z].end > e_flo && (int64_t)rs_start(A.rsum, z) < e_fhi;
                };
                const bool banned = (in_end_fetch(e) && sv_banned(A, e)) || (m >= 0 && in_end_fetch(m) && sv_banned(A, m));
                keep = !banned;
            }
            int tot;
            const int kk = kept + block_prefix(keep, &tot);
            if (keep) { seed_e[kk] = e; seed_hap[kk] = 2; }
            kept += tot;
            __syncthreads();
        }
        n_seed = kept < 2 ? 0 : kept;
    }
    __syncthreads();

    CH_MARK(1);
    for (int k = tid; k < n_seed; k += CH_THREADS) { const int x = canon(seed_e[k]); if (x >= 0) init_slot(x); }
    __syncthreads();
    int n_inc = 0, n_sinc = 0;
    int P = 0;
    const int nh_reg = A.no_extended ? 0 : nh;
    if (!A.no_extended) {
        for (int i = tid; i < nh; i += CH_THREADS) {
            site_base[i] = A.site_lo[lbase + i];
            site_cnt[i] = A.site_n[lbase + i];
        }
        __syncthreads();
        if (warp == 0) {
            int run = 0;
            for (int b0 = 0; b0 < nh; b0 += 32) {
                const int i = b0 + lane;
                const int v = i < nh ? site_cnt[i] : 0;
                int x = v;
#pragma unroll
                for (int o = 1; o < 32; o <<= 1) { const int y = __shfl_up_sync(0xffffffffu, x, o); if (lane >= o) x += y; }
                if (i < nh) cand_off[i] = run + x - v;
                run += __shfl_sync(0xffffffffu, x, 31);
            }
            if (lane == 0) cand_off[nh] = run;
        }
        for (int i = tid; i <= nh; i += CH_THREADS) site_off[i] = 0x7fffffff;
        __syncthreads();
        const int n_candidates = cand_off[nh];
    CH_MARK(2);
        constexpr int CH_SB = 32;
        __shared__ uint32_t s_bal[CH_SB * CH_WARPS];
        __shared__ int32_t s_bpre[CH_SB * CH_WARPS];
        __shared__ int32_t s_btot;
        for (int c0 = 0; c0 < n_candidates; c0 += CH_SB * CH_THREADS) {
            const int nb = min(CH_SB, (n_candidates - c0 + CH_THREADS - 1) / CH_THREADS);
            int i0 = 0;
            if (c0 + tid < n_candidates) {
                int lo = 0, hi = nh;
                while (hi - lo > 1) { const int mid = (lo + hi) >> 1; if (cand_off[mid] <= c0 + tid) lo = mid; else hi = mid; }
                i0 = lo;
            }
            int i = i0;
#pragma unroll 4
            for (int b = 0; b < nb; ++b) {
                const int c = c0 + b * CH_THREADS + tid;
                bool ok = false;
                if (c < n_candidates) {
                    while (cand_off[i + 1] <= c) ++i;
                    const int64_t r = blk_lo + site_base[i] + (c - cand_off[i]);
                    const int32_t p = spos[i];
                    bool ov = A.rsum[r].end > p;
                    if (ov && site_cnt[i] > A.ext_goal) {
                        int idx = 0;
                        for (int64_t q = blk_lo + site_base[i]; q < r; ++q) idx += A.rsum[q].end > p;
                        ov = idx <= A.ext_goal;
                    }
                    ok = ov && pair_ok(A, r, true);
                }
                const unsigned bal = __ballot_sync(0xffffffffu, ok);
                if (lane == 0) s_bal[b * CH_WARPS + warp] = bal;
            }
            __syncthreads();
            if (warp == 0) {
                int run = 0;
                for (int j0 = 0; j0 < nb * CH_WARPS; j0 += 32) {
                    const int j = j0 + lane;
                    const int v = j < nb * CH_WARPS ? __popc(s_bal[j]) : 0;
                    int x = v;
#pragma unroll
                    for (int o = 1; o < 32; o <<= 1) { const int y = __shfl_up_sync(0xffffffffu, x, o); if (lane >= o) x += y; }
                    if (j < nb * CH_WARPS) s_bpre[j] = run + x - v;
                    run += __shfl_sync(0xffffffffu, x, 31);
                }
                if (lane == 0) s_btot = run;
            }
            __syncthreads();
            i = i0;
            for (int b = 0; b < nb; ++b) {
                const int c = c0 + b * CH_THREADS + tid;
                const unsigned bal = s_bal[b * CH_WARPS + warp];
                if (c < n_candidates && ((bal >> lane) & 1u)) {
                    while (cand_off[i + 1] <= c) ++i;
                    const int64_t r = blk_lo + site_base[i] + (c - cand_off[i]);
                    const int k = n_inc + s_bpre[b * CH_WARPS + warp] + __popc(bal & ((1u << lane) - 1u));
                    if (k < cap_inc) {
                        inc_r[k] = (int32_t)r;
                        inc_x[k] = canon(r);
                        inc_site[k] = i;
                    }
                }
            }
            n_inc += s_btot;
            __syncthreads();
        }
    CH_MARK(3);
        if (n_inc > cap_inc) { n_inc = (int)cap_inc; T.status |= 2; }
        __syncthreads();
        for (int k = tid; k < n_inc; k += CH_THREADS) {
            if (k == 0 || inc_site[k - 1] != inc_site[k]) site_off[inc_site[k]] = k;
            init_slot(inc_x[k]);
        }
        __syncthreads();
        for (int k = tid; k < n_inc; k += CH_THREADS)
            atomicMax(&rec[inc_x[k]].key, ((unsigned long long)(uint32_t)(inc_site[k] + 1) << 32) | (uint32_t)inc_r[k]);
        __syncthreads();
        for (int base = 0; base < n_inc; base += CH_THREADS) {
            const int k = base + tid;
            bool rep = false;
            int x = 0;
            if (k < n_inc) {
                x = inc_x[k];
                rep = rec[x].key == (((unsigned long long)(uint32_t)(inc_site[k] + 1) << 32) | (uint32_t)inc_r[k]);
            }
            int tot;
            const int id = P + block_prefix(rep, &tot);
            if (rep) { rec[x].dense = id; x_of[id] = x; prim[id] = inc_r[k]; }
            P += tot;
        }
        if (tid == 0) {
            int nxt = n_inc;
            site_off[nh] = n_inc;
            for (int i = nh - 1; i >= 0; --i) { if (site_off[i] == 0x7fffffff) site_off[i] = nxt; else nxt = site_off[i]; }
        }
        __syncthreads();
    }
    CH_MARK(4);
    int n_ref_entries = 0;
    for (int base = 0; base < n_seed; base += CH_THREADS) {
        const int k = base + tid;
        int tot;
        block_prefix(k < n_seed && seed_hap[k] == 1, &tot);
        n_ref_entries += tot;
    }
    for (int k = tid; k < n_inc; k += CH_THREADS) rec[inc_x[k]].key = 0ull;
    for (int k = tid; k < n_seed; k += CH_THREADS) { const int x = canon(seed_e[k]); if (x >= 0) rec[x].key = 0ull; }
    __syncthreads();
    {
        int ref_seen = 0, alt_seen = 0;
        for (int base = 0; base < n_seed; base += CH_THREADS) {
            const int k = base + tid;
            const bool live = k < n_seed;
            const int hap = live ? seed_hap[k] : 0;
            int tot_ref, tot_alt;
            const int pr = block_prefix(hap == 1, &tot_ref);
            const int pa = block_prefix(hap == 2, &tot_alt);
            if (live) {
                const int32_t e = seed_e[k];
                const int x = canon(e);
                const unsigned reg = hap == 1 ? (unsigned)(ref_seen + pr) : (unsigned)(n_ref_entries + alt_seen + pa);
                const unsigned visit = hap == 2 ? (unsigned)(alt_seen + pa) : (unsigned)(ref_seen + pr);
                seed_reg[k] = reg;
                seed_e[k] = x >= 0 ? e : -1 - e;
                if (x >= 0) atomicMax(&rec[x].key, ((unsigned long long)(reg + 1u) << 32) | (uint32_t)e);
                (void)visit;
            }
            ref_seen += tot_ref;
            alt_seen += tot_alt;
        }
        __syncthreads();
        for (int base = 0; base < n_seed; base += CH_THREADS) {
            const int k = base + tid;
            bool rep = false, fresh = false;
            int x = -1;
            int32_t e = -1;
            if (k < n_seed && (e = seed_e[k]) >= 0) {
                x = canon(e);
                rep = rec[x].key == (((unsigned long long)(seed_reg[k] + 1u) << 32) | (uint32_t)e);
                fresh = rep && rec[x].dense < 0;
            }
            int tot;
            const int id = P + block_prefix(fresh, &tot);
            if (fresh) { rec[x].dense = id; x_of[id] = x; }
            if (rep) prim[fresh ? id : rec[x].dense] = e;
            P += tot;
        }
        __syncthreads();
    }
    if ((int64_t)P > cap_inc + cap_seed) { P = (int)(cap_inc + cap_seed); T.status |= 8; }

    int n_front0 = 0;
    auto setup = [&](auto& V) {
        using PT = typename std::remove_reference<decltype(V.inc_px[0])>::type;
        using ST = typename std::remove_reference<decltype(V.inc_site[0])>::type;
        __shared__ int s_front;
        for (int p = tid; p < P; p += CH_THREADS) {
            V.ord[p] = 0xffffffffu; V.fpos[p] = -1; V.tmp[p] = 0; V.minkey[p] = KEY_NONE; V.label[p] = 0;
        }
        if (tid == 0) s_front = 0;
        for (int k = tid; k < n_inc; k += CH_THREADS) {
            const int px = rec[inc_x[k]].dense;
            const int st = inc_site[k];
            V.inc_px[k] = (PT)px;
            V.inc_site[k] = (ST)st;
        }
        __syncthreads();
        int ref_seen = 0, alt_seen = 0, ns_total = 0;
        for (int base = 0; base < n_seed; base += CH_THREADS) {
            const int k = base + tid;
            const bool live = k < n_seed;
            const int hap = live ? seed_hap[k] : 0;
            int tot_ref, tot_alt;
            const int pr = block_prefix(hap == 1, &tot_ref);
            const int pa = block_prefix(hap == 2, &tot_alt);
            int n_match = 0, piv = -1, px = -1;
            int32_t st = 0, en = 0;
            unsigned reg = 0;
            if (live && seed_e[k] >= 0) {
                const int32_t e = seed_e[k];
                const int x = canon(e);
                px = rec[x].dense;
                reg = seed_reg[k];
                const unsigned visit = hap == 2 ? (unsigned)(alt_seen + pa) : (unsigned)(ref_seen + pr);
                atomicMin(V.ord + px, (hap == 2 ? 0u : (1u << 24)) | (visit & 0xffffffu));
                atomicOr(V.tmp + px, hap);
                if (rec[x].key == (((unsigned long long)(reg + 1u) << 32) | (uint32_t)e))
                    V.front[0][atomicAdd(&s_front, 1)] = (PT)px;
                if (nh_reg > 0) {
                    st = rs_start(A.rsum, e);
                    en = A.rsum[e].end;
                    piv = bisect_pivot(spos, nh_reg, st, en);
                    if (piv >= 0) {
                        n_match = 1;
                        for (int j = piv + 1; j < nh_reg && st <= spos[j] && spos[j] <= en; ++j) ++n_match;
                        for (int j = piv - 1; j >= 0 && st <= spos[j] && spos[j] <= en; --j) ++n_match;
                    }
                }
            }
            int tm;
            const int off_m = block_prefix_sum(n_match, &tm);
            if (n_match > 0) {
                int w = 0;
                const unsigned keybase = (unsigned)nh + reg * (unsigned)(nh + 1);
                const int dst0 = ns_total + off_m;
                auto push = [&](int i) {
                    const int dst = dst0 + w;
                    if (dst < cap_sinc) { V.sinc_px[dst] = (PT)px; V.sinc_site[dst] = (ST)i; V.sinc_sidx[dst] = keybase + (unsigned)w; }
                    ++w;
                };
                push(piv);
                for (int j = piv + 1; j < nh_reg && st <= spos[j] && spos[j] <= en; ++j) push(j);
                for (int j = piv - 1; j >= 0 && st <= spos[j] && spos[j] <= en; --j) push(j);
            }
            ref_seen += tot_ref;
            alt_seen += tot_alt;
            ns_total += tm;
        }
        n_sinc = ns_total;
        if (n_sinc > cap_sinc) { n_sinc = (int)cap_sinc; T.status |= 4; }
        __syncthreads();
        n_front0 = s_front;
        for (int p = tid; p < P; p += CH_THREADS) { V.label[p] = (uint8_t)V.tmp[p]; V.tmp[p] = 0; }
        __syncthreads();
        if (A.no_extended) return;
    CH_MARK(5);
        for (int k = tid; k < n_inc; k += CH_THREADS) {
            const int i = (int)V.inc_site[k], px = (int)V.inc_px[k];
            const uint8_t al = allele_info(A, S0, (int64_t)prim[px], (int64_t)H[i], (char)sref[i], (char)salt[i]);
            V.inc_al[k] = al;
            if (al & 3) atomicAdd(V.tmp + px, 1);
        }
        for (int k = tid; k < n_sinc; k += CH_THREADS) {
            const int i = (int)V.sinc_site[k], px = (int)V.sinc_px[k];
            const uint8_t al = allele_info(A, S0, (int64_t)prim[px], (int64_t)H[i], (char)sref[i], (char)salt[i]);
            V.sinc_al[k] = al;
            if (al & 3) atomicAdd(V.tmp + px, 1);
        }
        __syncthreads();
        int run = 0;
        for (int base = 0; base < P; base += CH_THREADS) {
            const int p = base + tid;
            const int c = p < P ? V.tmp[p] : 0;
            int tot;
            const int o = run + block_prefix_sum(c, &tot);
            if (p < P) { V.adj_off[p] = (PT)o; V.tmp[p] = 0; }
            run += tot;
        }
        if (tid == 0) V.adj_off[P] = (PT)run;
        __syncthreads();
        for (int k = tid; k < n_inc; k += CH_THREADS)
            if (V.inc_al[k] & 3) { const int px = (int)V.inc_px[k]; V.adj[(int)V.adj_off[px] + atomicAdd(V.tmp + px, 1)] = (PT)k; }
        for (int k = tid; k < n_sinc; k += CH_THREADS)
            if (V.sinc_al[k] & 3) { const int px = (int)V.sinc_px[k]; V.adj[(int)V.adj_off[px] + atomicAdd(V.tmp + px, 1)] = (PT)(n_inc + k); }
        __syncthreads();
        for (int p = tid; p < P; p += CH_THREADS) V.tmp[p] = 0;
        __syncthreads();
    };
    BfsView<int32_t, int32_t> VG;
    VG.ord = S0.p_ord + o_pair; VG.fpos = S0.p_fpos + o_pair; VG.tmp = S0.p_tmp + o_pair; VG.minkey = S0.p_minkey + o_pair;
    VG.label = S0.p_label + o_pair;
    VG.inc_px = inc_x; VG.inc_site = inc_site; VG.inc_al = S0.inc_al + o_inc;
    VG.sinc_px = S0.sinc_px + o_sinc; VG.sinc_site = S0.sinc_site + o_sinc;
    VG.sinc_sidx = S0.sinc_sidx + o_sinc; VG.sinc_al = S0.sinc_al + o_sinc;
    VG.adj = S0.adj + o_adj; VG.adj_off = S0.adj_off + o_pair + 2 * (int64_t)d;
    VG.front[0] = S0.front0 + o_pair; VG.front[1] = S0.front1 + o_pair;
    VG.spos = spos; VG.site_off = site_off; VG.bestkey = nullptr; VG.site_cnt = site_cnt; VG.site_base = site_base;
    VG.active = S0.active + o_het;

    setup(VG);
    __syncthreads();
    if (small_sites) {
        int32_t* g_spos = S0.spos + o_het;
        int32_t* g_off = S0.site_off + o_het + d;
        for (int i = tid; i < nh; i += CH_THREADS) g_spos[i] = spos[i];
        for (int i = tid; i <= nh; i += CH_THREADS) g_off[i] = A.no_extended ? 0 : site_off[i];
    }
    if (tid == 0) {
        int32_t* m = S0.meta + (int64_t)d * META_INTS;
        m[0] = P; m[1] = n_inc; m[2] = n_sinc; m[3] = n_front0; m[4] = T.status;
    }
    CH_MARK(6);
}

constexpr int SM_P = 512;
constexpr int SM_I = 768;
constexpr int SM_SI = 256;

__global__ void __launch_bounds__(CH_THREADS, CH_BFS_MINB)
chain_bfs_kernel(ChainArgs A) {
    UNFZ_GUARD(A.guard);
    const int d = blockIdx.x;
    const int tid = threadIdx.x;
    const Scratch& S0 = A.S;
    const int32_t* meta = S0.meta + (int64_t)d * META_INTS;
    const int P = meta[0], n_inc = meta[1], n_sinc = meta[2], n_front0 = meta[3];
    if (P <= 0 || n_front0 <= 0 || A.no_extended) return;
    const int nh = A.n_het[d];
    const int64_t* off = A.off;
    const int64_t n1 = (int64_t)A.n_dnms + 1;
    const int64_t o_inc = off[1 * n1 + d], o_seed = off[2 * n1 + d], o_sinc = off[3 * n1 + d], o_het = off[4 * n1 + d];
    const int64_t o_pair = o_inc + o_seed, o_adj = o_inc + o_sinc;
    BfsView<int32_t, int32_t> G;
    G.ord = S0.p_ord + o_pair; G.fpos = S0.p_fpos + o_pair; G.tmp = S0.p_tmp + o_pair; G.minkey = S0.p_minkey + o_pair;
    G.label = S0.p_label + o_pair;
    G.inc_px = S0.inc_x + o_inc; G.inc_site = S0.inc_site + o_inc; G.inc_al = S0.inc_al + o_inc;
    G.sinc_px = S0.sinc_px + o_sinc; G.sinc_site = S0.sinc_site + o_sinc;
    G.sinc_sidx = S0.sinc_sidx + o_sinc; G.sinc_al = S0.sinc_al + o_sinc;
    G.adj = S0.adj + o_adj; G.adj_off = S0.adj_off + o_pair + 2 * (int64_t)d;
    G.front[0] = S0.front0 + o_pair; G.front[1] = S0.front1 + o_pair;
    G.spos = S0.spos + o_het; G.site_off = S0.site_off + o_het + d; G.bestkey = S0.bestkey + o_het;
    G.site_cnt = S0.site_cnt + o_het; G.site_base = S0.site_base + o_het; G.active = S0.active + o_het;
    const int n_adj = G.adj_off[P];
    if (!(nh <= CH_SMEM_SITES && P <= SM_P && n_inc <= SM_I && n_sinc <= SM_SI)) {
        bfs_levels(G, nh, n_inc, n_front0);
        return;
    }
    __shared__ __align__(8) unsigned long long sm_minkey[SM_P], sm_bestkey[CH_SMEM_SITES];
    __shared__ uint32_t sm_ord[SM_P], sm_sinc_sidx[SM_SI];
    __shared__ int32_t sm_fpos[SM_P], sm_tmp[SM_P], sm_spos[CH_SMEM_SITES], sm_site_off[CH_SMEM_SITES + 1];
    __shared__ int32_t sm_site_cnt[CH_SMEM_SITES], sm_site_base[CH_SMEM_SITES];
    __shared__ uint16_t sm_inc_px[SM_I], sm_sinc_px[SM_SI], sm_adj[SM_I + SM_SI], sm_adj_off[SM_P + 2], sm_front[2][SM_P];
    __shared__ uint8_t sm_label[SM_P], sm_inc_site[SM_I], sm_inc_al[SM_I], sm_sinc_site[SM_SI], sm_sinc_al[SM_SI];
    __shared__ uint8_t sm_active[CH_SMEM_SITES];
    for (int p = tid; p < P; p += CH_THREADS) {
        sm_ord[p] = G.ord[p]; sm_label[p] = G.label[p]; sm_adj_off[p] = (uint16_t)G.adj_off[p];
        sm_fpos[p] = -1; sm_tmp[p] = 0; sm_minkey[p] = KEY_NONE;
    }
    if (tid == 0) sm_adj_off[P] = (uint16_t)n_adj;
    for (int k = tid; k < n_inc; k += CH_THREADS) {
        sm_inc_px[k] = (uint16_t)G.inc_px[k]; sm_inc_site[k] = (uint8_t)G.inc_site[k]; sm_inc_al[k] = G.inc_al[k];
    }
    for (int k = tid; k < n_sinc; k += CH_THREADS) {
        sm_sinc_px[k] = (uint16_t)G.sinc_px[k]; sm_sinc_site[k] = (uint8_t)G.sinc_site[k];
        sm_sinc_sidx[k] = G.sinc_sidx[k]; sm_sinc_al[k] = G.sinc_al[k];
    }
    for (int q = tid; q < n_adj; q += CH_THREADS) sm_adj[q] = (uint16_t)G.adj[q];
    for (int f = tid; f < n_front0; f += CH_THREADS) sm_front[0][f] = (uint16_t)G.front[0][f];
    for (int i = tid; i < nh; i += CH_THREADS) sm_spos[i] = G.spos[i];
    for (int i = tid; i <= nh; i += CH_THREADS) sm_site_off[i] = G.site_off[i];
    __syncthreads();
    BfsView<uint16_t, uint8_t> V;
    V.ord = sm_ord; V.fpos = sm_fpos; V.tmp = sm_tmp; V.minkey = sm_minkey; V.label = sm_label;
    V.inc_px = sm_inc_px; V.inc_site = sm_inc_site; V.inc_al = sm_inc_al;
    V.sinc_px = sm_sinc_px; V.sinc_site = sm_sinc_site; V.sinc_sidx = sm_sinc_sidx; V.sinc_al = sm_sinc_al;
    V.adj = sm_adj; V.adj_off = sm_adj_off; V.front[0] = sm_front[0]; V.front[1] = sm_front[1];
    V.spos = sm_spos; V.site_off = sm_site_off; V.bestkey = sm_bestkey; V.site_cnt = sm_site_cnt; V.site_base = sm_site_base;
    V.active = sm_active;
    bfs_levels(V, nh, n_inc, n_front0);
    for (int p = tid; p < P; p += CH_THREADS) G.label[p] = sm_label[p];
}

__global__ void __launch_bounds__(CH_THREADS, CH_MINB)
chain_evidence_kernel(ChainArgs A) {
    UNFZ_GUARD(A.guard);
#ifdef CH_DEBUG
    long long ch_t0 = clock64();
#endif
    const int d = blockIdx.x;
    const int tid = threadIdx.x;
    const Scratch& S0 = A.S;
    const int32_t* meta = S0.meta + (int64_t)d * META_INTS;
    const int P = meta[0];
    if (P < 0) return;
    const UnfzDnm dn = A.dnms[d];
    UnfzTally T;
    T.n_dad_sites = T.n_mom_sites = T.n_dad_reads = T.n_mom_reads = 0;
    T.cnv_dad = T.cnv_mom = 0;
    T.has_record = 0;
    T.status = meta[4];
    const int nc = A.n_cand[d];
    const int64_t lbase = A.seg_pair_off[dn.seg_lo];
    const uint32_t* C = A.cand_list + lbase;
    const int64_t* off = A.off;
    const int64_t n1 = (int64_t)A.n_dnms + 1;
    const int64_t o_slot = off[0 * n1 + d], o_inc = off[1 * n1 + d], o_seed = off[2 * n1 + d], o_cand = off[5 * n1 + d];
    const int64_t o_pair = o_inc + o_seed;
    uint8_t* label_out = A.slot_label + o_slot; uint8_t* evid_out = A.slot_evid + o_slot;
    const int32_t* x_of = S0.x_of + o_pair; const int32_t* prim = S0.prim + o_pair;
    const int32_t* cpos = S0.cpos + o_cand;
    uint8_t* cev = A.cand_evid + lbase;

    CH_MARK(7);
    int has_rec = 0, dr = 0, mr = 0;
    const uint8_t* final_label = S0.p_label + o_pair;
    for (int p = tid; p < P; p += CH_THREADS) {
        const uint8_t lab = final_label[p];
        if (!lab) continue;
        const int64_t e0 = prim[p];
        const int64_t ents[2] = {e0, (int64_t)rs_mate(A.rsum, e0)};
        uint8_t ev = 0;
        for (int t = 0; t < 2; ++t) {
            const int64_t e = ents[t];
            if (e < 0) continue;
            const int32_t st = rs_start(A.rsum, e), en = A.rsum[e].end;
            int lb = 0, hi = nc;
            while (lb < hi) { const int mid = (lb + hi) >> 1; if (cpos[mid] < st) lb = mid + 1; else hi = mid; }
            if (lb >= nc || cpos[lb] >= en) continue;
            int ub = lb;
            while (ub < nc && cpos[ub] <= en) ++ub;
            bool consistent = true;
            for (int j = lb + 1; j < ub; ++j)
                if ((C[j] ^ C[lb]) & 0x80000000u) { consistent = false; break; }
            if (!consistent) continue;
            has_rec = 1;
            for (int j = lb; j < ub; ++j) {
                const uint32_t cw = C[j];
                const int64_t row = cw & 0x3fffffffu;
                const uint32_t h = hit_lookup(A, e, row);
                if (!(h & 0xffffu)) continue;
                const char c = hit_char(h);
                bool origin_ref;
                if (c == (char)__ldg(A.sites.ref + row)) origin_ref = true;
                else if (c == (char)__ldg(A.sites.alt + row)) origin_ref = false;
                else continue;
                const bool alt_is_dad = (cw & 0x80000000u) != 0;
                uint8_t bits = 0;
                for (int hp = 1; hp <= 2; ++hp) {
                    if (!(lab & hp)) continue;
                    const bool to_alt = origin_ref == (hp == 1);
                    bits |= (to_alt == alt_is_dad) ? 1 : 2;
                }
                ev |= bits;
                unsigned* wp = reinterpret_cast<unsigned*>(reinterpret_cast<uintptr_t>(cev + j) & ~(uintptr_t)3);
                atomicOr(wp, (unsigned)bits << (8 * (reinterpret_cast<uintptr_t>(cev + j) & 3)));
            }
        }
        const int x = x_of[p];
        label_out[x] = lab;
        evid_out[x] = ev;
        dr += ev & 1;
        mr += (ev >> 1) & 1;
    }
    __syncthreads();

    CH_MARK(8);
    int ds = 0, ms = 0, esd = 0, esm = 0;
    for (int j = tid; j < nc; j += CH_THREADS) {
        const uint8_t b = cev[j];
        esd += b & 1;
        esm += (b >> 1) & 1;
        for (int bit = 1; bit <= 2; ++bit) {
            if (!(b & bit)) continue;
            bool first = true;
            for (int j2 = j - 1; j2 >= 0 && cpos[j2] == cpos[j]; --j2)
                if (cev[j2] & bit) { first = false; break; }
            if (first) { if (bit == 1) ++ds; else ++ms; }
        }
    }
    if (A.ev_need) { esd = block_sum(esd); esm = block_sum(esm); }
    ds = block_sum(ds); ms = block_sum(ms); dr = block_sum(dr); mr = block_sum(mr);
    has_rec = block_sum(has_rec);
    if (tid == 0) {
        T.n_dad_sites = ds; T.n_mom_sites = ms; T.n_dad_reads = dr; T.n_mom_reads = mr;
        T.has_record = has_rec > 0;
        A.tally[d] = T;
        if (A.ev_need) {
            const int64_t n = A.n_dnms;
            A.ev_need[d] = dr; A.ev_need[n + d] = mr; A.ev_need[2 * n + d] = esd; A.ev_need[3 * n + d] = esm;
        }
    }
    CH_MARK(9);
}

}
```

unfazed_b200/engine.py:

```python
from __future__ import annotations

import contextlib
import ctypes as C
import collections
import os
from dataclasses import dataclass, field
from typing import Dict, List, Optional

import numpy as np
import torch

from . import _lib as L
from .plan import Plan
from .schema import ReadTable, SiteTable, min_base_qual


def make_params(ab_homref=(0.0, 0.2), ab_homalt=(0.8, 1.0), ab_het=(0.2, 0.8), min_gt_qual=20, min_depth=10,
                min_map_qual=1, readlen=151, insert_size_max_sample=1000000, no_extended=False,
                evidence_min_ratio=10, split_error_margin=5) -> L.Params:
    p = L.Params()
    p.ab_homref[0], p.ab_homref[1] = float(ab_homref[0]), float(ab_homref[1])
    p.ab_homalt[0], p.ab_homalt[1] = float(ab_homalt[0]), float(ab_homalt[1])
    p.ab_het[0], p.ab_het[1] = float(ab_het[0]), float(ab_het[1])
    p.min_gt_qual = float(min_gt_qual)
    p.min_depth = int(min_depth)
    p.min_map_qual = int(min_map_qual)
    p.readlen = int(readlen)
    p.ext_read_goal = int(min(insert_size_max_sample, 2**31 - 1))
    p.no_extended = int(bool(no_extended))
    p.evidence_min_ratio = int(evidence_min_ratio)
    p.split_error_margin = int(split_error_margin)
    return p


def pack_site_rows(pos, flag, gt, gq, rd, ad):
    g = gt.to(torch.int32)
    meta = (flag.to(torch.int32) | (g[0] << 8) | (g[1] << 16) | (g[2] << 24)).contiguous()
    rec = torch.stack([pos.view(torch.float32), gq[0], gq[1], gq[2]], dim=1).contiguous()
    dep = torch.stack([rd[0], ad[0], rd[1], ad[1], rd[2], ad[2]], dim=1).contiguous()
    return meta, rec, dep


class DeviceSites:
    def __init__(self, table: SiteTable, device: torch.device, pin: bool = False, engine: "Engine" = None):
        self.table = table
        self.n_rows = table.n_rows
        up = lambda a: _to_device(np.ascontiguousarray(a), device, pin)
        self.blk_off = up(table.blk_off.astype(np.int64))
        self.pos, self.ref, self.alt = up(table.pos), up(table.ref), up(table.alt)
        flag, gt, gq, rd, ad = up(table.flag), up(table.gt), up(table.gq), up(table.rd), up(table.ad)
        self.h2d_bytes = sum(t.numel() * t.element_size() for t in (self.pos, self.ref, self.alt, flag, gt, gq, rd, ad))
        if engine is not None:
            V = max(self.n_rows, 1)
            self.meta = torch.empty((V,), dtype=torch.int32, device=device)
            self.rec = torch.empty((V, 4), dtype=torch.float32, device=device)
            self.dep = torch.empty((V, 6), dtype=torch.int32, device=device)
            st = C.c_void_p(torch.cuda.current_stream(device).cuda_stream)
            engine._check(engine.lib.unfz_pack_site_rows(engine.ctx, self.n_rows, self.pos.data_ptr(), flag.data_ptr(), gt.data_ptr(),
                                                         gq.data_ptr(), rd.data_ptr(), ad.data_ptr(), self.meta.data_ptr(),
                                                         self.rec.data_ptr(), self.dep.data_ptr(), st), "pack_site_rows")
        else:
            self.meta, self.rec, self.dep = pack_site_rows(self.pos, flag, gt, gq, rd, ad)
        self.cols = make_site_cols(table.n_rows, table.n_blocks, self.blk_off, self.pos, self.ref, self.alt,
                                   self.meta, self.rec, self.dep)

    @property
    def nbytes(self) -> int:
        return self.h2d_bytes


def make_site_cols(n_rows, n_blocks, blk_off, pos, ref, alt, meta, rec, dep) -> L.SiteCols:
    c = L.SiteCols()
    c.n_rows, c.n_blocks = n_rows, n_blocks
    c.blk_off, c.pos, c.ref, c.alt = blk_off.data_ptr(), pos.data_ptr(), ref.data_ptr(), alt.data_ptr()
    c.meta, c.rec, c.dep = meta.data_ptr(), rec.data_ptr(), dep.data_ptr()
    return c


class PackedReads:

    def __init__(self, table: ReadTable, min_bq: int, pin: bool = False):
        self.table, self.min_bq = table, int(min_bq)
        conv = (lambda a: torch.from_numpy(np.ascontiguousarray(a)).pin_memory().numpy()) if pin else np.ascontiguousarray
        self.hdr = conv(table.hdr.view(np.uint8).reshape(-1))
        self.cigar = conv(table.cigar)
        self.lowq = conv(table.lowq_plane(self.min_bq))
        self.seq2 = conv(table.seq2)
        self.nidx = conv(table.n_index())

    @property
    def nbytes(self) -> int:
        return sum(int(a.nbytes) for a in (self.hdr, self.cigar, self.lowq, self.seq2, self.nidx))


class DeviceReads:
    def __init__(self, table, device: torch.device, pin: bool = False, min_bq: int = 20, engine: "Engine" = None):
        packed = table if isinstance(table, PackedReads) else PackedReads(table, min_bq)
        table = packed.table
        self.table, self.min_bq = table, packed.min_bq
        self.n_reads = table.n_reads
        self.max_l_seq = table.max_l_seq()
        up = lambda a, pad=0: _to_device(a, device, pin, pad)
        self.blk_off = up(np.ascontiguousarray(table.blk_off.astype(np.int64)))
        self.hdr = up(packed.hdr)
        self.cigar = up(packed.cigar)
        nq = int(table.qual.shape[0])
        plane_bytes = (nq + 7) // 8
        self.lowq = up(packed.lowq, 48 + (-plane_bytes) % 4)
        self.seq2 = up(packed.seq2, 16)
        self.nidx = up(packed.nidx)
        self.nmask = torch.zeros(self.lowq.shape[0], dtype=torch.uint8, device=device)
        self.h2d_bytes = packed.nbytes
        self.blk_sblk = torch.full((max(table.n_blocks, 1),), -1, dtype=torch.int32, device=device)
        self.blk_cul = torch.zeros((max(table.n_blocks, 1),), dtype=torch.float64, device=device)
        c = L.ReadCols()
        c.n_reads, c.n_blocks = table.n_reads, table.n_blocks
        c.blk_off, c.blk_sblk, c.blk_cul = self.blk_off.data_ptr(), self.blk_sblk.data_ptr(), self.blk_cul.data_ptr()
        self.start = torch.empty((max(table.n_reads, 1),), dtype=torch.int32, device=device)
        c.hdr, c.cigar, c.seq2 = self.hdr.data_ptr(), self.cigar.data_ptr(), self.seq2.data_ptr()
        c.start = self.start.data_ptr()
        c.lowq, c.nmask = self.lowq.data_ptr(), self.nmask.data_ptr()
        c.n_qual, c.n_cigar = nq, int(table.cigar.shape[0])
        self.cols = c
        st = C.c_void_p(torch.cuda.current_stream(device).cuda_stream)
        if engine is not None:
            engine._check(engine.lib.unfz_read_starts(engine.ctx, C.byref(c), self.start.data_ptr(), st), "read_starts")
        else:
            self.start.copy_(self.hdr.view(torch.int32).view(-1, 8)[:, 0]) if table.n_reads else None
        if engine is not None and packed.nidx.shape[0]:
            engine._check(engine.lib.unfz_expand_nlist(engine.ctx, C.byref(c), self.hdr.data_ptr(), self.nmask.data_ptr(),
                                                       self.nidx.data_ptr(), int(packed.nidx.shape[0]), st), "expand_nlist")

    @property
    def nbytes(self) -> int:
        return self.h2d_bytes


def _to_device(a: np.ndarray, device, pin: bool, pad: int = 0) -> torch.Tensor:
    t = torch.from_numpy(a.view(np.uint8).reshape(-1)) if a.dtype.fields is not None else torch.from_numpy(a)
    if not t.is_pinned() and (pin or t.numel() * t.element_size() <= (1 << 20)):
        t = t.pin_memory()
    out = torch.empty(t.shape[:-1] + (t.shape[-1] + pad,), dtype=t.dtype, device=device) if pad else torch.empty_like(t, device=device)
    if pad:
        out[..., t.shape[-1]:].zero_()
        out[..., : t.shape[-1]].copy_(t, non_blocking=True)
    else:
        out.copy_(t, non_blocking=True)
    return out


@dataclass
class BatchResult:
    plan: Plan
    n_pairs: int
    n_hits: int
    seg_row_lo: np.ndarray
    seg_pair_off: np.ndarray
    n_het: np.ndarray
    n_cand: np.ndarray
    cnv_dad: np.ndarray
    cnv_mom: np.ndarray
    tally: Optional[np.ndarray] = None
    calls_strict: Optional[np.ndarray] = None
    calls_ambiguous: Optional[np.ndarray] = None
    win: Optional[np.ndarray] = None
    slot_off: Optional[np.ndarray] = None
    ev: Optional[dict] = None
    timings_ms: Dict[str, float] = field(default_factory=dict)
    launches: int = 0
    _dev: dict = field(default_factory=dict)

    def _np(self, name):
        key = "_np_" + name
        if key not in self._dev:
            self._dev[key] = self._dev[name].cpu().numpy()
        return self._dev[key]

    def class_codes(self) -> np.ndarray:
        return self._np("cls")

    def het_rows(self, d: int) -> np.ndarray:
        base = int(self.seg_pair_off[self.plan.dnm["seg_lo"][d]]) if self.plan.dnm["seg_hi"][d] > self.plan.dnm["seg_lo"][d] else 0
        return self._np("het_list")[base: base + int(self.n_het[d])]

    def cand_words(self, d: int) -> np.ndarray:
        base = int(self.seg_pair_off[self.plan.dnm["seg_lo"][d]]) if self.plan.dnm["seg_hi"][d] > self.plan.dnm["seg_lo"][d] else 0
        return self._np("cand_list")[base: base + int(self.n_cand[d])]

    def cand_evidence(self, d: int) -> np.ndarray:
        base = int(self.seg_pair_off[self.plan.dnm["seg_lo"][d]]) if self.plan.dnm["seg_hi"][d] > self.plan.dnm["seg_lo"][d] else 0
        return self._np("cand_evid")[base: base + int(self.n_cand[d])]

    def slot_labels(self, d: int) -> np.ndarray:
        a, b = int(self.slot_off[d]), int(self.slot_off[d + 1])
        return self._np("slot_label")[a:b]

    def slot_evidence(self, d: int) -> np.ndarray:
        a, b = int(self.slot_off[d]), int(self.slot_off[d + 1])
        return self._np("slot_evid")[a:b]

    def slot_reads(self, d: int, slots: np.ndarray) -> np.ndarray:
        a_lo, a_hi, b_lo, _b_hi = (int(x) for x in self.win[:, d])
        na = a_hi - a_lo
        slots = np.asarray(slots, dtype=np.int64)
        return np.where(slots < na, a_lo + slots, b_lo + (slots - na))

    def read_summaries(self) -> np.ndarray:
        return self._np("rsum").view(L.RSUM_DTYPE)


class PendingBatch:

    def __init__(self, finish):
        self._finish = finish

    def finish(self) -> "BatchResult":
        f, self._finish = self._finish, None
        if f is None:
            raise RuntimeError("PendingBatch.finish() called twice")
        return f()


class Engine:

    def __init__(self, device: int = 0):
        if not torch.cuda.is_available():
            raise RuntimeError("unfazed_b200 needs a CUDA device (sm_100a); none is visible -- there is no CPU path")
        self.lib = L.load()
        self.device = torch.device("cuda", device)
        torch.cuda.set_device(self.device)
        ctx = C.c_void_p()
        rc = self.lib.unfz_ctx_create(device, C.byref(ctx))
        if rc != 0:
            raise RuntimeError("unfz_ctx_create failed (%d): libunfazed_sm100.so targets sm_100a only" % rc)
        self.ctx = ctx
        self.stream = torch.cuda.Stream(self.device)
        self.stream2 = torch.cuda.Stream(self.device)
        self.use_graph = not os.environ.get("UNFZ_NO_GRAPH")
        self._caps = None
        self.spec_fallbacks = 0
        self._pinned_free: Dict[int, list] = {}
        self._stage_new: list = []
        self._stage_busy: list = []
        self._pool_limit = int(0.35 * torch.cuda.get_device_properties(self.device).total_memory)

    def on_stream(self):
        cur = torch.cuda.current_stream(self.device)
        if cur == self.stream:
            return contextlib.nullcontext()
        self.stream.wait_stream(cur)
        return torch.cuda.stream(self.stream)

    def __del__(self):
        try:
            if getattr(self, "ctx", None):
                self.lib.unfz_ctx_destroy(self.ctx)
                self.ctx = None
        except Exception:
            pass

    def concordant_upper_lens(self, dreads: "DeviceReads", readlen: int, insert_size_max_sample: int, stdevs: int) -> np.ndarray:
        with self.on_stream():
            return self._concordant_upper_lens(dreads, readlen, insert_size_max_sample, stdevs)

    def _concordant_upper_lens(self, dreads, readlen, insert_size_max_sample, stdevs):
        t = dreads.table
        lib, dev = self.lib, self.device
        st = C.c_void_p(torch.cuda.current_stream(dev).cuda_stream)
        out = np.zeros(max(t.n_blocks, 1), dtype=np.float64)
        nwork = int(lib.unfz_insert_size_work_bytes())
        head = getattr(t, "head_tlen", None) or {}
        for k, kid in enumerate(t.kids):
            blocks = [b for b in range(t.n_blocks) if int(t.blk_kid[b]) == k]
            cols = dreads.cols
            if kid in head:
                h = np.asarray(head[kid][: insert_size_max_sample + 1], dtype=np.int64)
                tmp_hdr = torch.zeros((max(h.shape[0], 1), 8), dtype=torch.int32, device=dev)
                if h.shape[0]:
                    tmp_hdr[: h.shape[0], 1] = torch.from_numpy(h.astype(np.int32)).to(dev)
                cols = L.ReadCols()
                cols.n_reads, cols.n_blocks, cols.hdr = int(h.shape[0]), 0, tmp_hdr.data_ptr()
                first, count = [0], [int(h.shape[0])]
            else:
                first, count, left = [], [], insert_size_max_sample + 1
                for b in blocks:
                    if left <= 0:
                        break
                    lo, hi = int(t.blk_off[b]), int(t.blk_off[b + 1])
                    take = min(left, hi - lo)
                    first.append(lo)
                    count.append(take)
                    left -= take
            n = int(sum(count))
            if n == 0:
                continue
            k0 = int(np.floor((n - 1) * 0.995))
            ranks = np.clip(np.array([k0 - 1, k0, k0 + 1, k0 + 2], dtype=np.int64), 0, n - 1).astype(np.uint64)
            work = torch.zeros(nwork, dtype=torch.uint8, device=dev)
            vals = torch.zeros(4, dtype=torch.int32, device=dev)
            hf, hc = np.array(first, dtype=np.int64), np.array(count, dtype=np.int64)
            self._check(lib.unfz_insert_size_order_stats(self.ctx, C.byref(cols), hf.ctypes.data, hc.ctypes.data, len(first),
                                                         int(readlen), ranks.ctypes.data, work.data_ptr(), vals.data_ptr(), st),
                        "insert_size_order_stats")
            v = vals.cpu().numpy().view(np.uint32).astype(np.int64)
            surrogate = np.empty(n, dtype=np.int64)
            r = ranks.astype(np.int64)
            surrogate[: r[1]] = v[0]
            surrogate[r[1]] = v[1]
            surrogate[r[2]:] = v[3]
            surrogate[r[2]] = v[2]
            pct = np.percentile(surrogate, 99.5)
            cul = float(int(np.mean(pct)) + (np.std(pct) * stdevs))
            for b in blocks:
                out[b] = cul
        return out

    def upload_sites(self, table: SiteTable, pin: bool = False) -> DeviceSites:
        if table.n_rows >= 2 ** 30:
            raise ValueError("a SiteTable holds %d rows; one upload is limited to 2^30 - 1 (split the cohort)" % table.n_rows)
        with self.on_stream():
            return DeviceSites(table, self.device, pin, self)

    def upload_reads(self, table, pin: bool = False, min_gt_qual=20) -> DeviceReads:
        with self.on_stream():
            return DeviceReads(table, self.device, pin, min_base_qual(min_gt_qual), self)

    def pack_reads(self, table: ReadTable, min_gt_qual=20, pin: bool = True) -> PackedReads:
        return PackedReads(table, min_base_qual(min_gt_qual), pin)

    def _pinned(self, a: np.ndarray) -> torch.Tensor:
        a = np.ascontiguousarray(a)
        nb = int(a.nbytes)
        st = torch.cuda.current_stream(self.device)
        if self._stage_new:
            ev = torch.cuda.Event()
            ev.record(st)
            self._stage_busy += [(blk, ev) for blk in self._stage_new]
            self._stage_new = []
        size = 4096
        while size < nb:
            size *= 2
        blk = None
        for i, (b_, ev) in enumerate(self._stage_busy):
            if b_.numel() == size and ev.query():
                blk = b_
                del self._stage_busy[i]
                break
        if blk is None:
            blk = torch.empty((size,), dtype=torch.uint8, pin_memory=True)
        host = blk[:nb]
        if nb:
            host.numpy()[:] = a.reshape(-1).view(np.uint8)
        self._stage_new.append(blk)
        return host.view(torch.from_numpy(np.empty(0, dtype=a.dtype)).dtype).reshape(a.shape)

    def _pinned_block(self, nbytes: int) -> torch.Tensor:
        size = 4096
        while size < nbytes:
            size *= 2
        free = self._pinned_free.get(size)
        return free.pop() if free else torch.empty((size,), dtype=torch.uint8, pin_memory=True)

    def _h2d(self, a: np.ndarray) -> torch.Tensor:
        return self._pinned(a).to(self.device, non_blocking=True)

    def _check(self, rc: int, what: str):
        if rc != 0:
            raise RuntimeError("%s failed (%d): %s" % (what, rc, self.lib.unfz_last_error(self.ctx).decode()))

    def _empty(self, n, dtype):
        return torch.empty((max(int(n), 1),), dtype=dtype, device=self.device)

    def _zeros(self, n, dtype):
        return torch.zeros((max(int(n), 1),), dtype=dtype, device=self.device)

    def _scan_work(self, n):
        return self._empty(self.lib.unfz_scan_work_bytes(int(n)), torch.uint8)

    def run(self, *args, **kw) -> BatchResult:
        with self.on_stream():
            return self._run(*args, **kw)

    def _run(self, dsites: DeviceSites, dreads: Optional[DeviceReads], plan: Plan, params: L.Params,
             blk_cul: Optional[np.ndarray] = None, time_stages: bool = False, download: bool = True,
             keep_device: bool = True, speculative: bool = True, evidence: bool = False, defer: bool = False):
        lib, ctx, dev = self.lib, self.ctx, self.device
        st = torch.cuda.current_stream(dev)
        s = C.c_void_p(st.cuda_stream)
        n, S = int(plan.dnm.shape[0]), int(plan.seg.shape[0])
        V = int(dsites.n_rows)
        N = int(dreads.n_reads) if dreads is not None else 0
        ev: List = []
        launches = 0
        caps = getattr(self, "_caps", None)
        spec = bool(speculative and download and caps is not None)
        reuse = not keep_device and not os.environ.get("UNFZ_NO_ARENA_REUSE")
        graph = bool(spec and not time_stages and reuse and self.use_graph)
        pool = self.__dict__.setdefault("_arena_pool", {})
        arenas: List = []

        def mark(name):
            if time_stages:
                e_ = torch.cuda.Event(enable_timing=True)
                e_.record(st)
                ev.append((name, e_))

        class Arena:
            def __init__(self, zero: bool):
                self.items, self.size, self.zero, self.buf = [], 0, zero, None

            def add(self, name, nbytes):
                self.items.append((name, self.size, int(nbytes)))
                self.size += (int(nbytes) + 255) & ~255

            def alloc(self_, clear=True):
                self_.key = (self_.zero, tuple(self_.items))
                q_ = pool.get(self_.key) if reuse else None
                buf = q_.popleft() if q_ else None
                if buf is None:
                    fn = torch.zeros if self_.zero else torch.empty
                    buf = fn((max(self_.size, 256),), dtype=torch.uint8, device=dev)
                elif self_.zero and clear:
                    buf.zero_()
                self_.buf = buf
                arenas.append(self_)
                base = self_.buf.data_ptr()
                self_.ptr = {nm: base + off for nm, off, _ in self_.items}
                self_.view = {nm: self_.buf[off: off + nb] for nm, off, nb in self_.items}

        cached = getattr(plan, "_resident", None)
        if cached is not None and cached[0] == dev and cached[2] == (plan.dnm.nbytes, plan.seg.nbytes, plan.alleles.nbytes):
            d_plan = cached[1]
        else:
            hp = np.concatenate([plan.dnm.view(np.uint8).reshape(-1), plan.seg.view(np.uint8).reshape(-1), plan.alleles,
                                 np.zeros(16, np.uint8)])
            d_plan = self._h2d(hp)
            try:
                plan._resident = (dev, d_plan, (plan.dnm.nbytes, plan.seg.nbytes, plan.alleles.nbytes))
            except AttributeError:
                pass
        p_dnm = d_plan.data_ptr()
        p_seg = p_dnm + plan.dnm.nbytes
        p_all = p_seg + plan.seg.nbytes
        sc = C.byref(dsites.cols)
        has_reads = dreads is not None and N > 0 and bool((plan.dnm["rblk"] >= 0).any())
        if has_reads and dreads.min_bq != min_base_qual(params.min_gt_qual):
            raise ValueError("the read columns on the device hold the low-quality plane of base quality < %d, the call "
                             "asks for < %d: upload them again with upload_reads(table, min_gt_qual=...)"
                             % (dreads.min_bq, min_base_qual(params.min_gt_qual)))

        z1, e1 = Arena(True), Arena(False)
        r_fields = [("n_het", n), ("n_cand", n), ("cnv_dad", n), ("cnv_mom", n), ("tally", 8 * n), ("calls_s", 4 * n),
                    ("calls_a", 4 * n), ("win", 4 * n), ("seg_row_lo", S)]
        r_off, acc = {}, 0
        for nm, cnt in r_fields:
            r_off[nm] = acc
            acc += cnt
        z1.add("result", 4 * acc)
        z1.add("guard", 256)
        z1.add("seg_pair_off", 8 * (S + 1))
        want_ev = bool(evidence and has_reads and download)
        if want_ev:
            z1.add("ev_off", 8 * 4 * (n + 1))
        dl_end = z1.size
        if has_reads:
            z1.add("off", 8 * (6 * (n + 1) + 1))
            dl_end += 8 * (n + 1)
        z1.add("row_mark", V)
        z1.add("mark_prefix", 4 * (V + 1))
        e1.add("seg_count", 8 * S)
        e1.add("scan_work", lib.unfz_scan_work_bytes(max(S, V, N, n) + 1))
        if has_reads:
            z1.add("blk_maxspan", 4 * max(dreads.table.n_blocks, 1))
            z1.add("need", 8 * 6 * n)
            if want_ev:
                z1.add("ev_need", 8 * 4 * n)
            e1.add("rsum", 32 * N)
            tile_reads = int(lib.unfz_read_scan_tile_reads(dreads.max_l_seq))
            n_tiles = (N + tile_reads - 1) // tile_reads
            e1.add("tile_tot", 4 * n_tiles)
            e1.add("tile_base", 4 * (n_tiles + 1))
            e1.add("tile_info", 8 * n_tiles)
        z1.alloc(clear=not graph)
        e1.alloc()
        R = z1.ptr["result"]
        rp = {nm: R + 4 * o for nm, o in r_off.items()}

        def arena2(n_pairs_):
            z, e = Arena(True), Arena(False)
            e.add("cls", n_pairs_)
            e.add("het_list", 4 * n_pairs_)
            e.add("cand_list", 4 * n_pairs_)
            if has_reads:
                e.add("site_lo", 4 * n_pairs_)
                e.add("site_n", 4 * n_pairs_)
                e.add("seed_win", 16 * n)
            z.add("cand_evid", n_pairs_ + 8)
            if want_ev:
                e.add("ev_pos_dad", 4 * n_pairs_ + 16)
                e.add("ev_pos_mom", 4 * n_pairs_ + 16)
            z.alloc(clear=not graph)
            e.alloc()
            return z, e

        def arena3(totals_, n_hits_):
            z, e = Arena(True), Arena(False)
            nb = lib.unfz_chain_scratch_bytes(*(int(x) for x in totals_), n)
            e.add("hits", 4 * max(n_hits_, 1))
            e.add("scratch", nb)
            z.add("slot_label", int(totals_[0]) + 4)
            z.add("slot_evid", int(totals_[0]) + 4)
            if want_ev:
                e.add("ev_read_dad", 4 * int(totals_[0]) + 16)
                e.add("ev_read_mom", 4 * int(totals_[0]) + 16)
            z.alloc(clear=not graph)
            e.alloc()
            return z, e, nb

        if spec:
            z2, e2 = arena2(int(caps["pairs"]))
            if has_reads:
                z3, e3, nbytes = arena3(caps["chain"], int(caps["hits"]))
        mark("start")

        def bind_blocks():
            cul_bytes = None if blk_cul is None else np.ascontiguousarray(blk_cul, dtype=np.float64).tobytes()
            token = getattr(plan, "_token", None)
            if token is None:
                token = object()
                try:
                    plan._token = token
                except AttributeError:
                    pass
            bound = (token, cul_bytes)
            if getattr(dreads, "_bound", None) != bound:
                sb = np.full(max(dreads.table.n_blocks, 1), -1, dtype=np.int32)
                if plan.rblk_sblk:
                    keys = np.fromiter(plan.rblk_sblk.keys(), dtype=np.int64, count=len(plan.rblk_sblk))
                    sb[keys] = np.fromiter(plan.rblk_sblk.values(), dtype=np.int32, count=len(plan.rblk_sblk))
                dreads.blk_sblk.copy_(self._pinned(sb), non_blocking=True)
                if blk_cul is not None:
                    dreads.blk_cul[: blk_cul.shape[0]].copy_(self._pinned(np.frombuffer(cul_bytes, dtype=np.float64).copy()), non_blocking=True)
                dreads._bound = bound

        fast = spec and not time_stages
        if fast:
            if has_reads:
                bind_blocks()
            b = L.Batch()
            b.sites = C.addressof(dsites.cols)
            b.reads = C.addressof(dreads.cols) if has_reads else None
            b.h_params = C.addressof(params)
            b.dnms, b.n_dnms, b.n_segs, b.segs, b.alleles = p_dnm, n, S, p_seg, p_all
            b.cap_pairs = int(caps["pairs"])
            b.seg_row_lo, b.seg_count, b.seg_pair_off = rp["seg_row_lo"], e1.ptr["seg_count"], z1.ptr["seg_pair_off"]
            b.scan_work, b.row_mark, b.mark_prefix = e1.ptr["scan_work"], z1.ptr["row_mark"], z1.ptr["mark_prefix"]
            b.guard, b.actual = z1.ptr["guard"], z1.ptr["guard"] + 64
            b.n_het, b.n_cand, b.cnv_dad, b.cnv_mom = rp["n_het"], rp["n_cand"], rp["cnv_dad"], rp["cnv_mom"]
            b.tally, b.calls_strict, b.calls_ambiguous, b.win = rp["tally"], rp["calls_s"], rp["calls_a"], rp["win"]
            b.cls, b.het_list, b.cand_list = e2.ptr["cls"], e2.ptr["het_list"], e2.ptr["cand_list"]
            b.cand_evid = z2.ptr["cand_evid"]
            if has_reads:
                b.max_l_seq, b.tile_reads, b.n_tiles = dreads.max_l_seq, tile_reads, n_tiles
                b.cap_hits = int(caps["hits"])
                for i_, v_ in enumerate(caps["chain"]):
                    b.cap_chain[i_] = int(v_)
                b.blk_maxspan, b.need, b.off = z1.ptr["blk_maxspan"], z1.ptr["need"], z1.ptr["off"]
                b.rsum = e1.ptr["rsum"]
                b.tile_tot, b.tile_base, b.tile_info = e1.ptr["tile_tot"], e1.ptr["tile_base"], e1.ptr["tile_info"]
                b.site_lo, b.site_n, b.seed_win = e2.ptr["site_lo"], e2.ptr["site_n"], e2.ptr["seed_win"]
                b.hits, b.scratch, b.scratch_bytes = e3.ptr["hits"], e3.ptr["scratch"], nbytes
                b.slot_label, b.slot_evid = z3.ptr["slot_label"], z3.ptr["slot_evid"]
                if want_ev:
                    b.ev_need, b.ev_off = z1.ptr["ev_need"], z1.ptr["ev_off"]
                    b.ev_read_dad, b.ev_read_mom = e3.ptr["ev_read_dad"], e3.ptr["ev_read_mom"]
                    b.ev_pos_dad, b.ev_pos_mom = e2.ptr["ev_pos_dad"], e2.ptr["ev_pos_mom"]
            if graph:
                zs = [z1, z2] + ([z3] if has_reads else [])
                spans = (L.Span * len(zs))(*[L.Span(z_.buf.data_ptr(), z_.buf.numel()) for z_ in zs])
                self._check(lib.unfz_run_batch_graph(ctx, C.byref(b), spans, len(zs), None, None, 0, s), "run_batch_graph")
            else:
                self._check(lib.unfz_run_batch(ctx, C.byref(b), s), "run_batch")
            launches += (22 if has_reads else 11) + (2 if want_ev else 0)
            h_pair_off, h_off = None, None
            res = BatchResult(plan=plan, n_pairs=int(caps["pairs"]), n_hits=int(caps["hits"]) if has_reads else 0,
                              seg_row_lo=None, seg_pair_off=None, n_het=None, n_cand=None, cnv_dad=None, cnv_mom=None)
            dv = res._dev
            dv.update(cls=e2.view["cls"], het_list=e2.view["het_list"].view(torch.int32),
                      cand_list=e2.view["cand_list"].view(torch.int32), cand_evid=z2.view["cand_evid"],
                      _keep=(z1, e1, z2, e2, d_plan))
            if has_reads:
                dv.update(rsum=e1.view["rsum"], hits=e3.view["hits"].view(torch.int32),
                          tile_base=e1.view["tile_base"].view(torch.int32), tile_reads=tile_reads,
                          slot_label=z3.view["slot_label"], slot_evid=z3.view["slot_evid"], row_mark=z1.view["row_mark"],
                          mark_prefix=z1.view["mark_prefix"].view(torch.int32), _keep3=(z3, e3))
        else:
            self._check(lib.unfz_window_search(ctx, sc, p_seg, S, rp["seg_row_lo"], e1.ptr["seg_count"], s), "window_search")
            self._check(lib.unfz_exclusive_scan_i64(ctx, e1.ptr["seg_count"], z1.ptr["seg_pair_off"], S, e1.ptr["scan_work"], s), "scan(pairs)")
            launches += 4
            mark("window_search")
            guard_ptr, actual_ptr = z1.ptr["guard"], z1.ptr["guard"] + 64

            def check_caps(ptrs, limits, slot):
                k = len(ptrs)
                a_t = (C.c_void_p * k)(*ptrs)
                a_c = (C.c_int64 * k)(*[int(x) for x in limits])
                self._check(lib.unfz_check_caps(ctx, k, a_t, a_c, guard_ptr, actual_ptr + 8 * slot, s), "check_caps")

            h_pair_off = None
            if spec:
                lib.unfz_ctx_set_guard(ctx, guard_ptr)
                n_pairs = int(caps["pairs"])
                check_caps([z1.ptr["seg_pair_off"] + 8 * S], [n_pairs], 0)
                launches += 1
            else:
                h_pair_off = z1.view["seg_pair_off"].cpu().numpy().view(np.int64)[: S + 1]
                n_pairs = int(h_pair_off[S]) if S > 0 else 0

            if not spec:
                z2, e2 = arena2(n_pairs)
            mark("alloc1")
            self._check(lib.unfz_classify_sites(ctx, sc, p_seg, rp["seg_row_lo"], z1.ptr["seg_pair_off"], S, n_pairs,
                                                C.byref(params), e2.ptr["cls"], s), "classify_sites")
            launches += 1 if n_pairs else 0
            mark("classify_sites")
            self._check(lib.unfz_compact_sites(ctx, p_dnm, n, p_seg, rp["seg_row_lo"], z1.ptr["seg_pair_off"], e2.ptr["cls"],
                                               e2.ptr["het_list"], rp["n_het"], e2.ptr["cand_list"], rp["n_cand"], rp["cnv_dad"],
                                               rp["cnv_mom"], z1.ptr["row_mark"], s), "compact_sites")
            self._check(lib.unfz_exclusive_scan_u8_i32(ctx, z1.ptr["row_mark"], z1.ptr["mark_prefix"], V, e1.ptr["scan_work"], s), "scan(marks)")
            launches += 4
            mark("compact_sites")

            res = BatchResult(plan=plan, n_pairs=n_pairs, n_hits=0, seg_row_lo=None, seg_pair_off=h_pair_off,
                              n_het=None, n_cand=None, cnv_dad=None, cnv_mom=None)
            dv = res._dev
            dv.update(cls=e2.view["cls"], het_list=e2.view["het_list"].view(torch.int32), cand_list=e2.view["cand_list"].view(torch.int32),
                      cand_evid=z2.view["cand_evid"], _keep=(z1, e1, z2, e2, d_plan))

            if has_reads:
                rc_ = C.byref(dreads.cols)
                bind_blocks()
                off_ptr = z1.ptr["off"]
                total_hits_ptr = off_ptr + 8 * 6 * (n + 1)
                mark("alloc2")
                self._check(lib.unfz_read_scan(ctx, rc_, sc, z1.ptr["mark_prefix"], C.byref(params), dreads.max_l_seq, e1.ptr["rsum"],
                                               z1.ptr["blk_maxspan"], e1.ptr["tile_tot"], e1.ptr["tile_info"], s),
                            "read_scan")
                launches += 1
                mark("read_scan")
                self._check(lib.unfz_exclusive_scan_u32(ctx, e1.ptr["tile_tot"], e1.ptr["tile_base"], n_tiles, total_hits_ptr,
                                                        e1.ptr["scan_work"], s), "scan(hits)")
                launches += 3
                mark("scan_hits")
                self._check(lib.unfz_chain_size(ctx, p_dnm, n, p_seg, z1.ptr["seg_pair_off"], sc, rc_, e1.ptr["rsum"],
                                                z1.ptr["blk_maxspan"], e2.ptr["het_list"], rp["n_het"], e2.ptr["cand_list"],
                                                rp["n_cand"], rp["win"], z1.ptr["need"], e2.ptr["site_lo"], e2.ptr["site_n"],
                                                e2.ptr["seed_win"], s), "chain_size")
                self._check(lib.unfz_exclusive_scan_rows_i64(ctx, z1.ptr["need"], off_ptr, 6, n, s), "scan(need)")
                launches += 2
                h_off = None
                if spec:
                    totals = np.asarray(caps["chain"], dtype=np.int64).copy()
                    n_hits = int(caps["hits"])
                    check_caps([off_ptr + 8 * ((i + 1) * (n + 1) - 1) for i in range(6)] + [total_hits_ptr],
                               list(totals) + [n_hits], 1)
                    launches += 1
                else:
                    h_all = z1.view["off"].cpu().numpy().view(np.int64)
                    h_off = h_all[: 6 * (n + 1)].reshape(6, n + 1)
                    n_hits = int(h_all[6 * (n + 1)])
                    totals = np.ascontiguousarray(h_off[:, n]).astype(np.int64)
                mark("chain_size")
                if n_hits >= 2**32:
                    raise RuntimeError("more than 2^32 read x site hits in one batch")
                res.n_hits = n_hits
                if not spec:
                    z3, e3, nbytes = arena3(totals, n_hits)
                mark("alloc3")
                self._check(lib.unfz_read_site_alleles(ctx, rc_, sc, z1.ptr["row_mark"], z1.ptr["mark_prefix"], e1.ptr["rsum"],
                                                       e1.ptr["tile_base"], tile_reads, e3.ptr["hits"],
                                                       e1.ptr["tile_info"], s),
                            "read_site_alleles")
                launches += 1
                mark("read_site_alleles")
                self._check(lib.unfz_chain_tally(ctx, p_dnm, n, p_seg, z1.ptr["seg_pair_off"], sc, rc_, e1.ptr["rsum"],
                                                 z1.ptr["blk_maxspan"], e3.ptr["hits"], e1.ptr["tile_base"], tile_reads, z1.ptr["mark_prefix"],
                                                 e2.ptr["het_list"],
                                                 rp["n_het"], e2.ptr["cand_list"], rp["n_cand"], p_all, rp["win"], e2.ptr["site_lo"], e2.ptr["site_n"],
                                                 e2.ptr["seed_win"], off_ptr,
                                                 totals.ctypes.data, C.byref(params), e3.ptr["scratch"], nbytes,
                                                 z3.ptr["slot_label"], z3.ptr["slot_evid"], z2.ptr["cand_evid"], rp["tally"],
                                                 z1.ptr["ev_need"] if want_ev else None, s),
                            "chain_tally")
                launches += 3
                mark("chain_tally")
                if want_ev:
                    self._check(lib.unfz_exclusive_scan_rows_i64(ctx, z1.ptr["ev_need"], z1.ptr["ev_off"], 4, n, s), "scan(ev)")
                    self._check(lib.unfz_evidence_lists(ctx, p_dnm, n, z1.ptr["seg_pair_off"], sc, e2.ptr["cand_list"], rp["n_cand"],
                                                        z2.ptr["cand_evid"], rp["win"], off_ptr, z3.ptr["slot_evid"], z1.ptr["ev_off"],
                                                        e3.ptr["ev_read_dad"], e3.ptr["ev_read_mom"], e2.ptr["ev_pos_dad"],
                                                        e2.ptr["ev_pos_mom"], s),
                                "evidence_lists")
                    launches += 2
                    mark("evidence_lists")
                dv.update(rsum=e1.view["rsum"], hits=e3.view["hits"].view(torch.int32),
                          tile_base=e1.view["tile_base"].view(torch.int32), tile_reads=tile_reads, slot_label=z3.view["slot_label"],
                          slot_evid=z3.view["slot_evid"], row_mark=z1.view["row_mark"],
                          mark_prefix=z1.view["mark_prefix"].view(torch.int32), _keep3=(z3, e3))
                if h_off is not None:
                    res.slot_off = h_off[0].copy()
            self._check(lib.unfz_summarize(ctx, p_dnm, n, rp["tally"], rp["cnv_dad"], rp["cnv_mom"], rp["n_cand"], C.byref(params),
                                           rp["calls_s"], rp["calls_a"], s), "summarize")
            launches += 1
            mark("summarize")
        if spec:
            lib.unfz_ctx_set_guard(ctx, None)
        front_buf, done = None, None
        if download:
            pkey = ("pinned", int(dl_end))
            q_ = pool.get(pkey) if reuse else None
            front_buf = q_.popleft() if q_ else torch.empty((dl_end,), dtype=torch.uint8, pin_memory=True)
            front_buf.copy_(z1.buf[:dl_end], non_blocking=True)
            done = torch.cuda.Event()
            done.record(st)

        def finish():
            nonlocal res
            if download:
                done.synchronize()
                front = front_buf.numpy().copy() if reuse else front_buf.numpy()
                self.last_d2h_bytes = int(dl_end)
                item = {nm: (off, nb) for nm, off, nb in z1.items}
                sect = lambda nm: front[item[nm][0]: item[nm][0] + item[nm][1]]
                hr = sect("result").view(np.int32)
                if spec:
                    g_ = sect("guard")
                    actual = g_[64: 64 + 64].view(np.int64)
                    if int(g_[:4].view(np.int32)[0]) != 0:
                        self.spec_fallbacks += 1
                        self._caps = None
                        dv.clear()
                        return self.run(dsites, dreads, plan, params, blk_cul=blk_cul, time_stages=time_stages,
                                        download=download, keep_device=keep_device, speculative=False, evidence=evidence)
                    res.seg_pair_off = sect("seg_pair_off").view(np.int64)[: S + 1].copy()
                    res.n_pairs = int(actual[0])
                    if has_reads:
                        o0 = item["off"][0]
                        res.slot_off = front[o0: o0 + 8 * (n + 1)].view(np.int64).copy()
                        res.n_hits = int(actual[7])
                        chain_now = [int(x) for x in actual[1:7]]
                elif has_reads:
                    chain_now = [int(x) for x in h_off[:, n]]
                need_now = {"pairs": res.n_pairs, "hits": res.n_hits, "chain": chain_now if has_reads else [0] * 6}
                grow = lambda v: int(v * 1.25) + 4096
                cur = getattr(self, "_caps", None)
                if cur is None:
                    self._caps = {"pairs": grow(need_now["pairs"]), "hits": grow(need_now["hits"]),
                                  "chain": [grow(v) for v in need_now["chain"]]}
                else:
                    cur["pairs"] = max(cur["pairs"], grow(need_now["pairs"]) if need_now["pairs"] > 0.9 * cur["pairs"] else 0)
                    cur["hits"] = max(cur["hits"], grow(need_now["hits"]) if need_now["hits"] > 0.9 * cur["hits"] else 0)
                    cur["chain"] = [max(c, grow(v) if v > 0.9 * c else 0) for c, v in zip(cur["chain"], need_now["chain"])]
                g = lambda nm, cnt: hr[r_off[nm]: r_off[nm] + cnt]
                res.seg_row_lo = g("seg_row_lo", S)
                res.n_het, res.n_cand = g("n_het", n), g("n_cand", n)
                res.cnv_dad, res.cnv_mom = g("cnv_dad", n), g("cnv_mom", n)
                res.tally = g("tally", 8 * n).view(L.TALLY_DTYPE)
                res.calls_strict = g("calls_s", 4 * n).view(L.CALL_DTYPE)
                res.calls_ambiguous = g("calls_a", 4 * n).view(L.CALL_DTYPE)
                res.win = g("win", 4 * n).reshape(4, n)
                if want_ev:
                    eo = sect("ev_off").view(np.int64).reshape(4, n + 1).copy()
                    tot = [int(eo[q, n]) for q in range(4)]
                    parts = [(e3.view["ev_read_dad"], 4 * tot[0]), (e3.view["ev_read_mom"], 4 * tot[1]),
                             (e2.view["ev_pos_dad"], 4 * tot[2]), (e2.view["ev_pos_mom"], 4 * tot[3])]
                    bufs, blocks = [], []
                    with torch.cuda.stream(self.stream2):
                        for t_, nb_ in parts:
                            hb = self._pinned_block(nb_)
                            if nb_:
                                hb[:nb_].copy_(t_[:nb_], non_blocking=True)
                            blocks.append(hb)
                    self.stream2.synchronize()
                    for hb, (t_, nb_) in zip(blocks, parts):
                        bufs.append(hb.numpy()[:nb_].copy().view(np.int32))
                        self._pinned_free.setdefault(int(hb.numel()), []).append(hb)
                    res.ev = {"off": eo, "read_dad": bufs[0], "read_mom": bufs[1], "pos_dad": bufs[2], "pos_mom": bufs[3]}
                    self.last_d2h_bytes += 4 * sum(tot)
            mark("download")
            res.launches = launches
            if time_stages:
                torch.cuda.synchronize(dev)
                for (n0, e0), (n1, e1_) in zip(ev[:-1], ev[1:]):
                    res.timings_ms[n1] = res.timings_ms.get(n1, 0.0) + e0.elapsed_time(e1_)
            if not keep_device:
                dv.clear()
                if len(pool) > 48 or sum(b_.numel() for q_ in pool.values() for b_ in q_) > self._pool_limit:
                    pool.clear()
                for a_ in arenas:
                    pool.setdefault(a_.key, collections.deque()).append(a_.buf)
                if download and reuse:
                    pool.setdefault(pkey, collections.deque()).append(front_buf)
            return res

        if defer:
            if time_stages or not download:
                raise ValueError("defer=True needs download=True and no stage timers")
            return PendingBatch(finish)
        return finish()
```

Baseline: 7.296 million.

## Flatten chain incident construction into grid-parallel filter, scan, compact and allele kernels

Result: slower. 6.794 million, median of 6 (-6.9%).

```diff
diff --git a/include/unfazed_sm100.h b/include/unfazed_sm100.h
--- a/include/unfazed_sm100.h
+++ b/include/unfazed_sm100.h
@@ -215,7 +215,7 @@
                     const int32_t* het_list, const int32_t* n_het, const uint32_t* cand_list,
                     const int32_t* n_cand, int32_t* win ,
                     int64_t* need,
-                    int32_t* site_lo, int32_t* site_n ,
+                    int32_t* site_lo, int32_t* site_coff ,
                     int32_t* seed_win , void* stream);
 
 int unfz_chain_tally(UnfzCtx*, const UnfzDnm* dnms, int32_t n_dnms, const UnfzSegIn* segs,
@@ -225,7 +225,7 @@
                      const int32_t* mark_prefix,
                      const int32_t* het_list, const int32_t* n_het, const uint32_t* cand_list,
                      const int32_t* n_cand, const uint8_t* alleles, const int32_t* win,
-                     const int32_t* site_lo, const int32_t* site_n, const int32_t* seed_win, const int64_t* off, const int64_t* h_totals ,
+                     const int32_t* site_lo, const int32_t* site_coff, const int32_t* seed_win, const int64_t* off, const int64_t* h_totals ,
                      const UnfzParams* h_params, void* scratch, int64_t scratch_bytes,
                      uint8_t* slot_label, uint8_t* slot_evid, uint8_t* cand_evid,
                      UnfzTally* tally,
@@ -266,7 +266,7 @@
     UnfzTally* tally;  UnfzCall* calls_strict;  UnfzCall* calls_ambiguous;  int32_t* win;
     int32_t* blk_maxspan;  int64_t* need;  int64_t* off;
     UnfzReadSum* rsum;  uint32_t* tile_tot;  uint32_t* tile_base;  uint32_t* tile_info;
-    uint8_t* cls;  int32_t* het_list;  uint32_t* cand_list;  int32_t* site_lo;  int32_t* site_n;  int32_t* seed_win;
+    uint8_t* cls;  int32_t* het_list;  uint32_t* cand_list;  int32_t* site_lo;  int32_t* site_coff;  int32_t* seed_win;
     uint8_t* cand_evid;
     uint32_t* hits;  void* scratch;  int64_t scratch_bytes;  uint8_t* slot_label;  uint8_t* slot_evid;
     int64_t* ev_need;  int64_t* ev_off;  int32_t* ev_read_dad;  int32_t* ev_read_mom;  int32_t* ev_pos_dad;  int32_t* ev_pos_mom;
diff --git a/unfazed_b200/_lib.py b/unfazed_b200/_lib.py
--- a/unfazed_b200/_lib.py
+++ b/unfazed_b200/_lib.py
@@ -53,7 +53,7 @@
         ("tally", c_void_p), ("calls_strict", c_void_p), ("calls_ambiguous", c_void_p), ("win", c_void_p),
         ("blk_maxspan", c_void_p), ("need", c_void_p), ("off", c_void_p),
         ("rsum", c_void_p), ("tile_tot", c_void_p), ("tile_base", c_void_p), ("tile_info", c_void_p),
-        ("cls", c_void_p), ("het_list", c_void_p), ("cand_list", c_void_p), ("site_lo", c_void_p), ("site_n", c_void_p),
+        ("cls", c_void_p), ("het_list", c_void_p), ("cand_list", c_void_p), ("site_lo", c_void_p), ("site_coff", c_void_p),
         ("seed_win", c_void_p), ("cand_evid", c_void_p),
         ("hits", c_void_p), ("scratch", c_void_p), ("scratch_bytes", c_int64), ("slot_label", c_void_p), ("slot_evid", c_void_p),
         ("ev_need", c_void_p), ("ev_off", c_void_p), ("ev_read_dad", c_void_p), ("ev_read_mom", c_void_p),
diff --git a/unfazed_b200/csrc/abi.cu b/unfazed_b200/csrc/abi.cu
--- a/unfazed_b200/csrc/abi.cu
+++ b/unfazed_b200/csrc/abi.cu
@@ -97,7 +97,7 @@
                                b->blk_maxspan, b->tile_tot, b->tile_info, s));
         UNFZ_RC(unfz_exclusive_scan_u32(ctx, b->tile_tot, b->tile_base, b->n_tiles, total_hits, b->scan_work, s));
         UNFZ_RC(unfz_chain_size(ctx, b->dnms, n, b->segs, b->seg_pair_off, b->sites, b->reads, b->rsum, b->blk_maxspan,
-                                b->het_list, b->n_het, b->cand_list, b->n_cand, b->win, b->need, b->site_lo, b->site_n,
+                                b->het_list, b->n_het, b->cand_list, b->n_cand, b->win, b->need, b->site_lo, b->site_coff,
                                 b->seed_win, s));
         UNFZ_RC(unfz_exclusive_scan_rows_i64(ctx, b->need, b->off, 6, n, s));
         {
@@ -112,7 +112,7 @@
                                        b->tile_reads, b->hits, b->tile_info, s));
         UNFZ_RC(unfz_chain_tally(ctx, b->dnms, n, b->segs, b->seg_pair_off, b->sites, b->reads, b->rsum, b->blk_maxspan,
                                  b->hits, b->tile_base, b->tile_reads, b->mark_prefix, b->het_list, b->n_het, b->cand_list,
-                                 b->n_cand, b->alleles, b->win, b->site_lo, b->site_n, b->seed_win, b->off, b->cap_chain,
+                                 b->n_cand, b->alleles, b->win, b->site_lo, b->site_coff, b->seed_win, b->off, b->cap_chain,
                                  b->h_params, b->scratch, b->scratch_bytes, b->slot_label, b->slot_evid, b->cand_evid,
                                  b->tally, b->ev_need, s));
         if (b->ev_need != nullptr) {
diff --git a/unfazed_b200/csrc/chain.cu b/unfazed_b200/csrc/chain.cu
--- a/unfazed_b200/csrc/chain.cu
+++ b/unfazed_b200/csrc/chain.cu
@@ -26,9 +26,10 @@
     int32_t* x_of; int32_t* prim;
     uint32_t* p_ord; int32_t* p_fpos; int32_t* p_tmp; unsigned long long* p_minkey; uint8_t* p_label;
     int32_t* adj; int32_t* adj_off; int32_t* front0; int32_t* front1;
-    int32_t* spos; uint8_t* sref; uint8_t* salt; int32_t* site_off; int32_t* cand_off;
+    int32_t* spos; int32_t* site_off;
     unsigned long long* bestkey; int32_t* site_cnt; int32_t* site_base; int32_t* active;
     int32_t* cpos;
+    uint8_t* cflag; int32_t* crank; void* scan_work;
     int32_t* meta;
 };
 
@@ -41,7 +42,7 @@
     const uint8_t* alleles; const int32_t* win; const int64_t* off;
     int32_t split_margin;
     const uint32_t* hit_tile_base; int32_t hit_tile_reads;
-    const int32_t* site_lo; const int32_t* site_n; const int32_t* seed_win;
+    const int32_t* site_lo; const int32_t* site_coff; const int32_t* seed_win;
     int32_t readlen, ext_goal, no_extended;
     uint8_t* slot_label; uint8_t* slot_evid; uint8_t* cand_evid; UnfzTally* tally;
     int64_t* ev_need;
@@ -326,6 +327,113 @@
 #undef CH_MINB
 #undef CH_BFS_MINB
 
+
+constexpr int CH_FLAT_THREADS = 256;
+
+struct CandSites {
+    const int32_t* co; const int32_t* lo; int nh; int32_t n; int64_t blk_lo;
+    __device__ __forceinline__ int site_of(int32_t j, int i) const {
+        if (i < 0) {
+            int l = 0, h = nh;
+            while (h - l > 1) { const int mid = (l + h) >> 1; if (__ldg(co + mid) <= j) l = mid; else h = mid; }
+            return l;
+        }
+        while (i + 1 < nh && __ldg(co + i + 1) <= j) ++i;
+        return i;
+    }
+    __device__ __forceinline__ int32_t count(int i) const { return (i + 1 < nh ? __ldg(co + i + 1) : n) - __ldg(co + i); }
+    __device__ __forceinline__ int64_t first_read(int i) const { return blk_lo + __ldg(lo + i); }
+};
+__device__ __forceinline__ CandSites cand_sites(const ChainArgs& A, int d, const UnfzDnm& dn, int32_t n) {
+    const int64_t lbase = A.seg_pair_off[dn.seg_lo];
+    CandSites cs;
+    cs.co = A.site_coff + lbase; cs.lo = A.site_lo + lbase; cs.nh = A.n_het[d]; cs.n = n;
+    cs.blk_lo = A.reads.blk_off[dn.rblk];
+    return cs;
+}
+
+__global__ void __launch_bounds__(CH_FLAT_THREADS)
+chain_filter_kernel(ChainArgs A) {
+    UNFZ_GUARD(A.guard);
+    const int d = blockIdx.x;
+    const int64_t* row = A.off + ((int64_t)A.n_dnms + 1);
+    const int64_t c0 = row[d];
+    const int32_t n = (int32_t)(row[d + 1] - c0);
+    if ((int64_t)blockIdx.y * CH_FLAT_THREADS >= n) return;
+    const UnfzDnm dn = A.dnms[d];
+    const CandSites cs = cand_sites(A, d, dn, n);
+    const int32_t* H = A.het_list + A.seg_pair_off[dn.seg_lo];
+    int i = -1;
+    for (int32_t j = blockIdx.y * CH_FLAT_THREADS + threadIdx.x; j < n; j += gridDim.y * CH_FLAT_THREADS) {
+        i = cs.site_of(j, i);
+        const int64_t r0 = cs.first_read(i);
+        const int64_t r = r0 + (j - __ldg(cs.co + i));
+        const int32_t p = __ldg(A.sites.pos + __ldg(H + i));
+        bool ov = A.rsum[r].end > p;
+        if (ov && cs.count(i) > A.ext_goal) {
+            int idx = 0;
+            for (int64_t q = r0; q < r; ++q) idx += A.rsum[q].end > p;
+            ov = idx <= A.ext_goal;
+        }
+        A.S.cflag[c0 + j] = ov && pair_ok(A, r, true);
+    }
+}
+
+__global__ void __launch_bounds__(CH_FLAT_THREADS)
+chain_compact_kernel(ChainArgs A) {
+    UNFZ_GUARD(A.guard);
+    const int d = blockIdx.x;
+    const int64_t* row = A.off + ((int64_t)A.n_dnms + 1);
+    const int64_t c0 = row[d];
+    const int32_t n = (int32_t)(row[d + 1] - c0);
+    if ((int64_t)blockIdx.y * CH_FLAT_THREADS >= n) return;
+    const UnfzDnm dn = A.dnms[d];
+    const CandSites cs = cand_sites(A, d, dn, n);
+    const int32_t rank0 = A.S.crank[c0];
+    const int64_t nd = A.n_dnms;
+    const int64_t a_lo = A.win[d], a_hi = A.win[nd + d], b_lo = A.win[2 * nd + d], b_hi = A.win[3 * nd + d];
+    auto slot_of = [&](int64_t r) -> int {
+        if (r >= a_lo && r < a_hi) return (int)(r - a_lo);
+        if (r >= b_lo && r < b_hi) return (int)((a_hi - a_lo) + (r - b_lo));
+        return -1;
+    };
+    int i = -1;
+    for (int32_t j = blockIdx.y * CH_FLAT_THREADS + threadIdx.x; j < n; j += gridDim.y * CH_FLAT_THREADS) {
+        if (!A.S.cflag[c0 + j]) continue;
+        i = cs.site_of(j, i);
+        const int64_t r = cs.first_read(i) + (j - __ldg(cs.co + i));
+        const int64_t dst = c0 + (A.S.crank[c0 + j] - rank0);
+        const int64_t m = rs_mate(A.rsum, r);
+        const int sr = slot_of(r), sm = m >= 0 ? slot_of(m) : -1;
+        A.S.inc_r[dst] = (int32_t)r;
+        A.S.inc_x[dst] = sr < 0 ? sm : (sm < 0 ? sr : (m < r ? sm : sr));
+        A.S.inc_site[dst] = i;
+    }
+}
+
+__global__ void __launch_bounds__(CH_FLAT_THREADS)
+chain_alleles_kernel(ChainArgs A) {
+    UNFZ_GUARD(A.guard);
+    const int d = blockIdx.x;
+    const int32_t* meta = A.S.meta + (int64_t)d * 8;
+    if (meta[0] <= 0 || meta[3] <= 0) return;
+    const int n_inc = meta[1], n = n_inc + meta[2];
+    if ((int64_t)blockIdx.y * CH_FLAT_THREADS >= n) return;
+    const int64_t n1 = (int64_t)A.n_dnms + 1;
+    const int64_t o_inc = A.off[n1 + d], o_sinc = A.off[3 * n1 + d];
+    const int32_t* prim = A.S.prim + o_inc + A.off[2 * n1 + d];
+    const int32_t* H = A.het_list + A.seg_pair_off[A.dnms[d].seg_lo];
+    for (int t = blockIdx.y * CH_FLAT_THREADS + threadIdx.x; t < n; t += gridDim.y * CH_FLAT_THREADS) {
+        const bool sd = t >= n_inc;
+        const int64_t g = sd ? o_sinc + (t - n_inc) : o_inc + t;
+        const int px = sd ? A.S.sinc_px[g] : A.S.inc_x[g];
+        const int i = sd ? A.S.sinc_site[g] : A.S.inc_site[g];
+        const int64_t hrow = __ldg(H + i);
+        const uint8_t al = allele_info(A, A.S, (int64_t)__ldg(prim + px), hrow, (char)__ldg(A.sites.ref + hrow),
+                                       (char)__ldg(A.sites.alt + hrow));
+        if (sd) A.S.sinc_al[g] = al; else A.S.inc_al[g] = al;
+    }
+}
 
 __global__ void __launch_bounds__(128)
 evidence_lists_kernel(const UnfzDnm* __restrict__ dnms, int32_t n_dnms, const int64_t* __restrict__ seg_pair_off,
@@ -421,7 +529,7 @@
                   const int32_t* __restrict__ blk_maxspan, const int32_t* __restrict__ het_list,
                   const int32_t* __restrict__ n_het, const uint32_t* __restrict__ cand_list,
                   const int32_t* __restrict__ n_cand, int32_t* __restrict__ win, int64_t* __restrict__ need,
-                  int32_t* __restrict__ site_lo, int32_t* __restrict__ site_n, int32_t* __restrict__ seed_win,
+                  int32_t* __restrict__ site_lo, int32_t* __restrict__ site_coff, int32_t* __restrict__ seed_win,
                   const int32_t* __restrict__ guard) {
     UNFZ_GUARD(guard);
     __shared__ int32_t s_hp[4][CS_HP];
@@ -451,20 +559,28 @@
         }
         const int64_t mid = sv ? ((int64_t)dn.pos + (int64_t)dn.end) / 2 : (int64_t)1 << 40;
         int64_t minA = sa_lo, maxA = sa_hi, minB = sv ? sb_lo : ((int64_t)1 << 40), maxB = sv ? sb_hi : -1;
-        int64_t incs = 0;
-        for (int i = lane; i < nh; i += 32) {
-            const int64_t p = sites.pos[H[i]];
-            if (i < CS_HP) hp[i] = (int32_t)p;
-            if (p < mid) { minA = min(minA, p); maxA = max(maxA, p + 1); }
-            else { minB = min(minB, p); maxB = max(maxB, p + 1); }
-            const int64_t a = lb_start(reads.start, blk_lo, blk_hi, p - maxspan + 1);
-            const int64_t b = lb_start_near(reads.start, a, blk_hi, p + 1);
-            site_lo[lbase + i] = (int32_t)(a - blk_lo);
-            site_n[lbase + i] = (int32_t)(b - a);
-            incs += b - a;
+        int32_t incs = 0;
+        for (int i0 = 0; i0 < nh; i0 += 32) {
+            const int i = i0 + lane;
+            int32_t cnt = 0;
+            if (i < nh) {
+                const int64_t p = sites.pos[H[i]];
+                if (i < CS_HP) hp[i] = (int32_t)p;
+                if (p < mid) { minA = min(minA, p); maxA = max(maxA, p + 1); }
+                else { minB = min(minB, p); maxB = max(maxB, p + 1); }
+                const int64_t a = lb_start(reads.start, blk_lo, blk_hi, p - maxspan + 1);
+                const int64_t b = lb_start_near(reads.start, a, blk_hi, p + 1);
+                site_lo[lbase + i] = (int32_t)(a - blk_lo);
+                cnt = (int32_t)(b - a);
+            }
+            int32_t x = cnt;
+#pragma unroll
+            for (int o = 1; o < 32; o <<= 1) { const int32_t y = __shfl_up_sync(0xffffffffu, x, o); if (lane >= o) x += y; }
+            if (i < nh) site_coff[lbase + i] = incs + x - cnt;
+            incs += __shfl_sync(0xffffffffu, x, 31);
         }
         minA = warp_min64(minA); maxA = warp_max64(maxA); minB = warp_min64(minB); maxB = warp_max64(maxB);
-        nd[1] = warp_sum64(incs);
+        nd[1] = incs;
         __syncwarp();
         a_lo = warp_lb_start(reads.start, blk_lo, blk_hi, minA - maxspan + 1, lane);
         a_hi = warp_lb_start(reads.start, a_lo, blk_hi, maxA, lane);
@@ -606,14 +722,15 @@
     S.p_tmp = (int32_t*)carve<int32_t>(p, pairs); S.p_label = (uint8_t*)carve<uint8_t>(p, pairs);
     S.adj = (int32_t*)carve<int32_t>(p, adjs); S.adj_off = (int32_t*)carve<int32_t>(p, pairs + 2 * n_dnms + 2);
     S.front0 = (int32_t*)carve<int32_t>(p, pairs); S.front1 = (int32_t*)carve<int32_t>(p, pairs);
-    S.spos = (int32_t*)carve<int32_t>(p, hets); S.sref = (uint8_t*)carve<uint8_t>(p, hets);
-    S.salt = (uint8_t*)carve<uint8_t>(p, hets); S.site_off = (int32_t*)carve<int32_t>(p, hets + n_dnms + 1);
-    S.cand_off = (int32_t*)carve<int32_t>(p, hets + n_dnms + 1);
+    S.spos = (int32_t*)carve<int32_t>(p, hets); S.site_off = (int32_t*)carve<int32_t>(p, hets + n_dnms + 1);
     S.bestkey = (unsigned long long*)carve<unsigned long long>(p, hets);
     S.site_cnt = (int32_t*)carve<int32_t>(p, hets); S.site_base = (int32_t*)carve<int32_t>(p, hets);
     S.active = (int32_t*)carve<int32_t>(p, hets);
     S.cpos = (int32_t*)carve<int32_t>(p, cands);
     S.meta = (int32_t*)carve<int32_t>(p, n_dnms * 8);
+    S.cflag = (uint8_t*)carve<uint8_t>(p, incs);
+    S.crank = (int32_t*)carve<int32_t>(p, incs + 1);
+    S.scan_work = (void*)carve<char>(p, unfz_scan_work_bytes(incs));
     *total = (int64_t)(p - base);
     return S;
 }
@@ -631,13 +748,13 @@
                                const int64_t* seg_pair_off, const UnfzSiteCols* sites, const UnfzReadCols* reads,
                                const UnfzReadSum* rsum, const int32_t* blk_maxspan, const int32_t* het_list,
                                const int32_t* n_het, const uint32_t* cand_list, const int32_t* n_cand,
-                               int32_t* win, int64_t* need, int32_t* site_lo, int32_t* site_n, int32_t* seed_win,
+                               int32_t* win, int64_t* need, int32_t* site_lo, int32_t* site_coff, int32_t* seed_win,
                                void* stream) {
     (void)segs;
     if (n_dnms <= 0) return 0;
     chain_size_kernel<<<(n_dnms + 3) / 4, 128, 0, (cudaStream_t)stream>>>(
         dnms, n_dnms, seg_pair_off, *sites, *reads, rsum, blk_maxspan, het_list, n_het, cand_list, n_cand, win, need,
-        site_lo, site_n, seed_win, ctx->guard);
+        site_lo, site_coff, seed_win, ctx->guard);
     UNFZ_LAUNCH_CHECK(ctx);
     return 0;
 }
@@ -657,7 +774,7 @@
                                 const UnfzReadSum* rsum, const int32_t* blk_maxspan, const uint32_t* hits,
                                 const uint32_t* hit_tile_base, int32_t hit_tile_reads, const int32_t* mark_prefix, const int32_t* het_list, const int32_t* n_het,
                                 const uint32_t* cand_list, const int32_t* n_cand, const uint8_t* alleles,
-                                const int32_t* win, const int32_t* site_lo, const int32_t* site_n, const int32_t* seed_win,
+                                const int32_t* win, const int32_t* site_lo, const int32_t* site_coff, const int32_t* seed_win,
                                 const int64_t* off, const int64_t* h_totals, const UnfzParams* hp, void* scratch, int64_t scratch_bytes,
                                 uint8_t* slot_label, uint8_t* slot_evid, uint8_t* cand_evid, UnfzTally* tally,
                                 int64_t* ev_need, void* stream) {
@@ -669,7 +786,7 @@
     A.het_list = het_list; A.n_het = n_het; A.cand_list = cand_list; A.n_cand = n_cand; A.alleles = alleles;
     A.win = win; A.off = off; A.split_margin = hp->split_error_margin;
     A.hit_tile_base = hit_tile_base; A.hit_tile_reads = hit_tile_reads;
-    A.site_lo = site_lo; A.site_n = site_n; A.seed_win = seed_win;
+    A.site_lo = site_lo; A.site_coff = site_coff; A.seed_win = seed_win;
     A.readlen = hp->readlen;
     A.ext_goal = hp->ext_read_goal;
     A.no_extended = hp->no_extended;
@@ -686,20 +803,36 @@
     }
     bool wide = h_totals[1] / n_dnms >= UNFZ_CHAIN_WIDE_MIN_INC;
     if (const char* force = getenv("UNFZ_CHAIN_SHAPE")) wide = force[0] == 'w' ? true : (force[0] == 's' ? false : wide);
+    cudaStream_t st = (cudaStream_t)stream;
+    auto flat_grid = [n_dnms](int64_t items) {
+        const int64_t y = (items / n_dnms + CH_FLAT_THREADS - 1) / CH_FLAT_THREADS;
+        return dim3((unsigned)n_dnms, (unsigned)(y < 1 ? 1 : (y > 65535 ? 65535 : y)));
+    };
+    const int64_t cap_inc = h_totals[1], cap_sinc = h_totals[3];
+    if (!A.no_extended && cap_inc > 0) {
+        chain_filter_kernel<<<flat_grid(cap_inc), CH_FLAT_THREADS, 0, st>>>(A);
+        UNFZ_LAUNCH_CHECK(ctx);
+        const int rc = unfz_exclusive_scan_u8_i32(ctx, A.S.cflag, A.S.crank, cap_inc, A.S.scan_work, stream);
+        if (rc) return rc;
+        chain_compact_kernel<<<flat_grid(cap_inc), CH_FLAT_THREADS, 0, st>>>(A);
+        UNFZ_LAUNCH_CHECK(ctx);
+    }
+    if (wide) cta_wide::chain_setup_kernel<<<n_dnms, cta_wide::CH_THREADS, 0, st>>>(A);
+    else cta_small::chain_setup_kernel<<<n_dnms, cta_small::CH_THREADS, 0, st>>>(A);
+    UNFZ_LAUNCH_CHECK(ctx);
+    if (!A.no_extended && cap_inc + cap_sinc > 0) {
+        chain_alleles_kernel<<<flat_grid(cap_inc + cap_sinc), CH_FLAT_THREADS, 0, st>>>(A);
+        UNFZ_LAUNCH_CHECK(ctx);
+    }
     if (wide) {
-        cta_wide::chain_setup_kernel<<<n_dnms, cta_wide::CH_THREADS, 0, (cudaStream_t)stream>>>(A);
+        cta_wide::chain_bfs_kernel<<<n_dnms, cta_wide::CH_THREADS, 0, st>>>(A);
         UNFZ_LAUNCH_CHECK(ctx);
-        cta_wide::chain_bfs_kernel<<<n_dnms, cta_wide::CH_THREADS, 0, (cudaStream_t)stream>>>(A);
+        cta_wide::chain_evidence_kernel<<<n_dnms, cta_wide::CH_THREADS, 0, st>>>(A);
+    } else {
+        cta_small::chain_bfs_kernel<<<n_dnms, cta_small::CH_THREADS, 0, st>>>(A);
         UNFZ_LAUNCH_CHECK(ctx);
-        cta_wide::chain_evidence_kernel<<<n_dnms, cta_wide::CH_THREADS, 0, (cudaStream_t)stream>>>(A);
-        UNFZ_LAUNCH_CHECK(ctx);
-        return 0;
-    }
-    cta_small::chain_setup_kernel<<<n_dnms, cta_small::CH_THREADS, 0, (cudaStream_t)stream>>>(A);
-    UNFZ_LAUNCH_CHECK(ctx);
-    cta_small::chain_bfs_kernel<<<n_dnms, cta_small::CH_THREADS, 0, (cudaStream_t)stream>>>(A);
-    UNFZ_LAUNCH_CHECK(ctx);
-    cta_small::chain_evidence_kernel<<<n_dnms, cta_small::CH_THREADS, 0, (cudaStream_t)stream>>>(A);
+        cta_small::chain_evidence_kernel<<<n_dnms, cta_small::CH_THREADS, 0, st>>>(A);
+    }
     UNFZ_LAUNCH_CHECK(ctx);
     return 0;
 }
diff --git a/unfazed_b200/csrc/chain_cta.inc b/unfazed_b200/csrc/chain_cta.inc
--- a/unfazed_b200/csrc/chain_cta.inc
+++ b/unfazed_b200/csrc/chain_cta.inc
@@ -13,6 +13,22 @@
     __syncthreads();
     *total = tot;
     return base + __popc(b & ((1u << lane) - 1u));
+}
+
+__device__ __forceinline__ int2 block_prefix2(bool fa, bool fb, int* total_a, int* total_b) {
+    __shared__ int wsum4[CH_WARPS];
+    const unsigned ba = __ballot_sync(0xffffffffu, fa), bb = __ballot_sync(0xffffffffu, fb);
+    const int lane = threadIdx.x & 31, w = threadIdx.x >> 5;
+    if (lane == 0) wsum4[w] = __popc(ba) | (__popc(bb) << 16);
+    __syncthreads();
+    int base = 0, tot = 0;
+#pragma unroll
+    for (int i = 0; i < CH_WARPS; ++i) { if (i < w) base += wsum4[i]; tot += wsum4[i]; }
+    __syncthreads();
+    *total_a = tot & 0xffff;
+    *total_b = tot >> 16;
+    const unsigned below = (1u << lane) - 1u;
+    return make_int2((base & 0xffff) + __popc(ba & below), (base >> 16) + __popc(bb & below));
 }
 
 __device__ __forceinline__ int block_prefix_sum(int v, int* total) {
@@ -169,6 +185,34 @@
     __syncthreads();
 }
 
+template <typename PT, typename ST>
+__device__ void build_adjacency(const BfsView<PT, ST>& V, int P, int n_inc, int n_sinc) {
+    const int tid = threadIdx.x;
+    for (int k = tid; k < n_inc; k += CH_THREADS)
+        if (V.inc_al[k] & 3) atomicAdd(V.tmp + (int)V.inc_px[k], 1);
+    for (int k = tid; k < n_sinc; k += CH_THREADS)
+        if (V.sinc_al[k] & 3) atomicAdd(V.tmp + (int)V.sinc_px[k], 1);
+    __syncthreads();
+    int run = 0;
+    for (int base = 0; base < P; base += CH_THREADS) {
+        const int p = base + tid;
+        const int c = p < P ? V.tmp[p] : 0;
+        int tot;
+        const int o = run + block_prefix_sum(c, &tot);
+        if (p < P) { V.adj_off[p] = (PT)o; V.tmp[p] = 0; }
+        run += tot;
+    }
+    if (tid == 0) V.adj_off[P] = (PT)run;
+    __syncthreads();
+    for (int k = tid; k < n_inc; k += CH_THREADS)
+        if (V.inc_al[k] & 3) { const int px = (int)V.inc_px[k]; V.adj[(int)V.adj_off[px] + atomicAdd(V.tmp + px, 1)] = (PT)k; }
+    for (int k = tid; k < n_sinc; k += CH_THREADS)
+        if (V.sinc_al[k] & 3) { const int px = (int)V.sinc_px[k]; V.adj[(int)V.adj_off[px] + atomicAdd(V.tmp + px, 1)] = (PT)(n_inc + k); }
+    __syncthreads();
+    for (int p = tid; p < P; p += CH_THREADS) V.tmp[p] = 0;
+    __syncthreads();
+}
+
 constexpr int META_INTS = 8;
 
 __global__ void __launch_bounds__(CH_THREADS, CH_MINB)
@@ -178,7 +222,7 @@
     long long ch_t0 = clock64();
 #endif
     const int d = blockIdx.x;
-    const int tid = threadIdx.x, lane = tid & 31, warp = tid >> 5;
+    const int tid = threadIdx.x;
     const UnfzDnm dn = A.dnms[d];
     const Scratch& S0 = A.S;
 
@@ -205,27 +249,19 @@
     const int64_t o_sinc = off[3 * n1 + d], o_het = off[4 * n1 + d], o_cand = off[5 * n1 + d];
     const int64_t cap_inc = off[1 * n1 + d + 1] - o_inc, cap_seed = off[2 * n1 + d + 1] - o_seed;
     const int64_t cap_sinc = off[3 * n1 + d + 1] - o_sinc;
-    const int64_t o_pair = o_inc + o_seed, o_adj = o_inc + o_sinc;
+    const int64_t o_pair = o_inc + o_seed;
 
     SlotRec* rec = S0.slot + o_slot;
     int32_t* inc_r = S0.inc_r + o_inc; int32_t* inc_x = S0.inc_x + o_inc; int32_t* inc_site = S0.inc_site + o_inc;
     int32_t* seed_e = S0.seed_e + o_seed; uint8_t* seed_hap = S0.seed_hap + o_seed; uint32_t* seed_reg = S0.seed_reg + o_seed;
     int32_t* x_of = S0.x_of + o_pair; int32_t* prim = S0.prim + o_pair;
-    __shared__ int32_t sh_spos[CH_SMEM_SITES], sh_site_off[CH_SMEM_SITES + 1], sh_cand_off[CH_SMEM_SITES + 1];
-    __shared__ int32_t sh_site_cnt[CH_SMEM_SITES], sh_site_base[CH_SMEM_SITES];
-    __shared__ uint8_t sh_sref[CH_SMEM_SITES], sh_salt[CH_SMEM_SITES];
+    __shared__ int32_t sh_spos[CH_SMEM_SITES], sh_site_off[CH_SMEM_SITES + 1];
     const bool small_sites = nh <= CH_SMEM_SITES;
     int32_t* spos = small_sites ? sh_spos : S0.spos + o_het;
-    uint8_t* sref = small_sites ? sh_sref : S0.sref + o_het;
-    uint8_t* salt = small_sites ? sh_salt : S0.salt + o_het;
     int32_t* site_off = small_sites ? sh_site_off : S0.site_off + o_het + d;
-    int32_t* cand_off = small_sites ? sh_cand_off : S0.cand_off + o_het + d;
-    int32_t* site_cnt = small_sites ? sh_site_cnt : S0.site_cnt + o_het;
-    int32_t* site_base = small_sites ? sh_site_base : S0.site_base + o_het;
     int32_t* cpos = S0.cpos + o_cand;
 
     const UnfzReadCols& R = A.reads;
-    const int64_t blk_lo = R.blk_off[dn.rblk];
     const int64_t nd_ = A.n_dnms;
     const int64_t a_lo = A.win[d], a_hi = A.win[nd_ + d], b_lo = A.win[2 * nd_ + d], b_hi = A.win[3 * nd_ + d];
     auto slot_of = [&](int64_t r) -> int {
@@ -262,10 +298,7 @@
     }
 #endif
     for (int i = tid; i < nh; i += CH_THREADS) {
-        const int64_t row = H[i];
-        spos[i] = __ldg(A.sites.pos + row);
-        sref[i] = __ldg(A.sites.ref + row);
-        salt[i] = __ldg(A.sites.alt + row);
+        spos[i] = __ldg(A.sites.pos + (int64_t)H[i]);
     }
     for (int j = tid; j < nc; j += CH_THREADS) {
         cpos[j] = __ldg(A.sites.pos + (int64_t)(C[j] & 0x3fffffffu));
@@ -352,96 +385,11 @@
     int P = 0;
     const int nh_reg = A.no_extended ? 0 : nh;
     if (!A.no_extended) {
-        for (int i = tid; i < nh; i += CH_THREADS) {
-            site_base[i] = A.site_lo[lbase + i];
-            site_cnt[i] = A.site_n[lbase + i];
-        }
-        __syncthreads();
-        if (warp == 0) {
-            int run = 0;
-            for (int b0 = 0; b0 < nh; b0 += 32) {
-                const int i = b0 + lane;
-                const int v = i < nh ? site_cnt[i] : 0;
-                int x = v;
-#pragma unroll
-                for (int o = 1; o < 32; o <<= 1) { const int y = __shfl_up_sync(0xffffffffu, x, o); if (lane >= o) x += y; }
-                if (i < nh) cand_off[i] = run + x - v;
-                run += __shfl_sync(0xffffffffu, x, 31);
-            }
-            if (lane == 0) cand_off[nh] = run;
-        }
+        n_inc = S0.crank[o_inc + cap_inc] - S0.crank[o_inc];
+        if (n_inc > cap_inc) { n_inc = (int)cap_inc; T.status |= 2; }
         for (int i = tid; i <= nh; i += CH_THREADS) site_off[i] = 0x7fffffff;
         __syncthreads();
-        const int n_candidates = cand_off[nh];
-    CH_MARK(2);
-        constexpr int CH_SB = 32;
-        __shared__ uint32_t s_bal[CH_SB * CH_WARPS];
-        __shared__ int32_t s_bpre[CH_SB * CH_WARPS];
-        __shared__ int32_t s_btot;
-        for (int c0 = 0; c0 < n_candidates; c0 += CH_SB * CH_THREADS) {
-            const int nb = min(CH_SB, (n_candidates - c0 + CH_THREADS - 1) / CH_THREADS);
-            int i0 = 0;
-            if (c0 + tid < n_candidates) {
-                int lo = 0, hi = nh;
-                while (hi - lo > 1) { const int mid = (lo + hi) >> 1; if (cand_off[mid] <= c0 + tid) lo = mid; else hi = mid; }
-                i0 = lo;
-            }
-            int i = i0;
-#pragma unroll 4
-            for (int b = 0; b < nb; ++b) {
-                const int c = c0 + b * CH_THREADS + tid;
-                bool ok = false;
-                if (c < n_candidates) {
-                    while (cand_off[i + 1] <= c) ++i;
-                    const int64_t r = blk_lo + site_base[i] + (c - cand_off[i]);
-                    const int32_t p = spos[i];
-                    bool ov = A.rsum[r].end > p;
-                    if (ov && site_cnt[i] > A.ext_goal) {
-                        int idx = 0;
-                        for (int64_t q = blk_lo + site_base[i]; q < r; ++q) idx += A.rsum[q].end > p;
-                        ov = idx <= A.ext_goal;
-                    }
-                    ok = ov && pair_ok(A, r, true);
-                }
-                const unsigned bal = __ballot_sync(0xffffffffu, ok);
-                if (lane == 0) s_bal[b * CH_WARPS + warp] = bal;
-            }
-            __syncthreads();
-            if (warp == 0) {
-                int run = 0;
-                for (int j0 = 0; j0 < nb * CH_WARPS; j0 += 32) {
-                    const int j = j0 + lane;
-                    const int v = j < nb * CH_WARPS ? __popc(s_bal[j]) : 0;
-                    int x = v;
-#pragma unroll
-                    for (int o = 1; o < 32; o <<= 1) { const int y = __shfl_up_sync(0xffffffffu, x, o); if (lane >= o) x += y; }
-                    if (j < nb * CH_WARPS) s_bpre[j] = run + x - v;
-                    run += __shfl_sync(0xffffffffu, x, 31);
-                }
-                if (lane == 0) s_btot = run;
-            }
-            __syncthreads();
-            i = i0;
-            for (int b = 0; b < nb; ++b) {
-                const int c = c0 + b * CH_THREADS + tid;
-                const unsigned bal = s_bal[b * CH_WARPS + warp];
-                if (c < n_candidates && ((bal >> lane) & 1u)) {
-                    while (cand_off[i + 1] <= c) ++i;
-                    const int64_t r = blk_lo + site_base[i] + (c - cand_off[i]);
-                    const int k = n_inc + s_bpre[b * CH_WARPS + warp] + __popc(bal & ((1u << lane) - 1u));
-                    if (k < cap_inc) {
-                        inc_r[k] = (int32_t)r;
-                        inc_x[k] = canon(r);
-                        inc_site[k] = i;
-                    }
-                }
-            }
-            n_inc += s_btot;
-            __syncthreads();
-        }
     CH_MARK(3);
-        if (n_inc > cap_inc) { n_inc = (int)cap_inc; T.status |= 2; }
-        __syncthreads();
         for (int k = tid; k < n_inc; k += CH_THREADS) {
             if (k == 0 || inc_site[k - 1] != inc_site[k]) site_off[inc_site[k]] = k;
             init_slot(inc_x[k]);
@@ -472,12 +420,8 @@
     }
     CH_MARK(4);
     int n_ref_entries = 0;
-    for (int base = 0; base < n_seed; base += CH_THREADS) {
-        const int k = base + tid;
-        int tot;
-        block_prefix(k < n_seed && seed_hap[k] == 1, &tot);
-        n_ref_entries += tot;
-    }
+    for (int k = tid; k < n_seed; k += CH_THREADS) n_ref_entries += seed_hap[k] == 1;
+    n_ref_entries = block_sum(n_ref_entries);
     for (int k = tid; k < n_inc; k += CH_THREADS) rec[inc_x[k]].key = 0ull;
     for (int k = tid; k < n_seed; k += CH_THREADS) { const int x = canon(seed_e[k]); if (x >= 0) rec[x].key = 0ull; }
     __syncthreads();
@@ -488,8 +432,8 @@
             const bool live = k < n_seed;
             const int hap = live ? seed_hap[k] : 0;
             int tot_ref, tot_alt;
-            const int pr = block_prefix(hap == 1, &tot_ref);
-            const int pa = block_prefix(hap == 2, &tot_alt);
+            const int2 pra = block_prefix2(hap == 1, hap == 2, &tot_ref, &tot_alt);
+            const int pr = pra.x, pa = pra.y;
             if (live) {
                 const int32_t e = seed_e[k];
                 const int x = canon(e);
@@ -546,8 +490,8 @@
             const bool live = k < n_seed;
             const int hap = live ? seed_hap[k] : 0;
             int tot_ref, tot_alt;
-            const int pr = block_prefix(hap == 1, &tot_ref);
-            const int pa = block_prefix(hap == 2, &tot_alt);
+            const int2 pra = block_prefix2(hap == 1, hap == 2, &tot_ref, &tot_alt);
+            const int pr = pra.x, pa = pra.y;
             int n_match = 0, piv = -1, px = -1;
             int32_t st = 0, en = 0;
             unsigned reg = 0;
@@ -597,39 +541,6 @@
         n_front0 = s_front;
         for (int p = tid; p < P; p += CH_THREADS) { V.label[p] = (uint8_t)V.tmp[p]; V.tmp[p] = 0; }
         __syncthreads();
-        if (A.no_extended) return;
-    CH_MARK(5);
-        for (int k = tid; k < n_inc; k += CH_THREADS) {
-            const int i = (int)V.inc_site[k], px = (int)V.inc_px[k];
-            const uint8_t al = allele_info(A, S0, (int64_t)prim[px], (int64_t)H[i], (char)sref[i], (char)salt[i]);
-            V.inc_al[k] = al;
-            if (al & 3) atomicAdd(V.tmp + px, 1);
-        }
-        for (int k = tid; k < n_sinc; k += CH_THREADS) {
-            const int i = (int)V.sinc_site[k], px = (int)V.sinc_px[k];
-            const uint8_t al = allele_info(A, S0, (int64_t)prim[px], (int64_t)H[i], (char)sref[i], (char)salt[i]);
-            V.sinc_al[k] = al;
-            if (al & 3) atomicAdd(V.tmp + px, 1);
-        }
-        __syncthreads();
-        int run = 0;
-        for (int base = 0; base < P; base += CH_THREADS) {
-            const int p = base + tid;
-            const int c = p < P ? V.tmp[p] : 0;
-            int tot;
-            const int o = run + block_prefix_sum(c, &tot);
-            if (p < P) { V.adj_off[p] = (PT)o; V.tmp[p] = 0; }
-            run += tot;
-        }
-        if (tid == 0) V.adj_off[P] = (PT)run;
-        __syncthreads();
-        for (int k = tid; k < n_inc; k += CH_THREADS)
-            if (V.inc_al[k] & 3) { const int px = (int)V.inc_px[k]; V.adj[(int)V.adj_off[px] + atomicAdd(V.tmp + px, 1)] = (PT)k; }
-        for (int k = tid; k < n_sinc; k += CH_THREADS)
-            if (V.sinc_al[k] & 3) { const int px = (int)V.sinc_px[k]; V.adj[(int)V.adj_off[px] + atomicAdd(V.tmp + px, 1)] = (PT)(n_inc + k); }
-        __syncthreads();
-        for (int p = tid; p < P; p += CH_THREADS) V.tmp[p] = 0;
-        __syncthreads();
     };
     BfsView<int32_t, int32_t> VG;
     VG.ord = S0.p_ord + o_pair; VG.fpos = S0.p_fpos + o_pair; VG.tmp = S0.p_tmp + o_pair; VG.minkey = S0.p_minkey + o_pair;
@@ -637,10 +548,10 @@
     VG.inc_px = inc_x; VG.inc_site = inc_site; VG.inc_al = S0.inc_al + o_inc;
     VG.sinc_px = S0.sinc_px + o_sinc; VG.sinc_site = S0.sinc_site + o_sinc;
     VG.sinc_sidx = S0.sinc_sidx + o_sinc; VG.sinc_al = S0.sinc_al + o_sinc;
-    VG.adj = S0.adj + o_adj; VG.adj_off = S0.adj_off + o_pair + 2 * (int64_t)d;
+    VG.adj = nullptr; VG.adj_off = nullptr;
     VG.front[0] = S0.front0 + o_pair; VG.front[1] = S0.front1 + o_pair;
-    VG.spos = spos; VG.site_off = site_off; VG.bestkey = nullptr; VG.site_cnt = site_cnt; VG.site_base = site_base;
-    VG.active = S0.active + o_het;
+    VG.spos = spos; VG.site_off = site_off; VG.bestkey = nullptr; VG.site_cnt = nullptr; VG.site_base = nullptr;
+    VG.active = nullptr;
 
     setup(VG);
     __syncthreads();
@@ -654,7 +565,7 @@
         int32_t* m = S0.meta + (int64_t)d * META_INTS;
         m[0] = P; m[1] = n_inc; m[2] = n_sinc; m[3] = n_front0; m[4] = T.status;
     }
-    CH_MARK(6);
+    CH_MARK(5);
 }
 
 constexpr int SM_P = 512;
@@ -685,8 +596,8 @@
     G.front[0] = S0.front0 + o_pair; G.front[1] = S0.front1 + o_pair;
     G.spos = S0.spos + o_het; G.site_off = S0.site_off + o_het + d; G.bestkey = S0.bestkey + o_het;
     G.site_cnt = S0.site_cnt + o_het; G.site_base = S0.site_base + o_het; G.active = S0.active + o_het;
-    const int n_adj = G.adj_off[P];
     if (!(nh <= CH_SMEM_SITES && P <= SM_P && n_inc <= SM_I && n_sinc <= SM_SI)) {
+        build_adjacency(G, P, n_inc, n_sinc);
         bfs_levels(G, nh, n_inc, n_front0);
         return;
     }
@@ -698,10 +609,9 @@
     __shared__ uint8_t sm_label[SM_P], sm_inc_site[SM_I], sm_inc_al[SM_I], sm_sinc_site[SM_SI], sm_sinc_al[SM_SI];
     __shared__ uint8_t sm_active[CH_SMEM_SITES];
     for (int p = tid; p < P; p += CH_THREADS) {
-        sm_ord[p] = G.ord[p]; sm_label[p] = G.label[p]; sm_adj_off[p] = (uint16_t)G.adj_off[p];
+        sm_ord[p] = G.ord[p]; sm_label[p] = G.label[p];
         sm_fpos[p] = -1; sm_tmp[p] = 0; sm_minkey[p] = KEY_NONE;
     }
-    if (tid == 0) sm_adj_off[P] = (uint16_t)n_adj;
     for (int k = tid; k < n_inc; k += CH_THREADS) {
         sm_inc_px[k] = (uint16_t)G.inc_px[k]; sm_inc_site[k] = (uint8_t)G.inc_site[k]; sm_inc_al[k] = G.inc_al[k];
     }
@@ -709,7 +619,6 @@
         sm_sinc_px[k] = (uint16_t)G.sinc_px[k]; sm_sinc_site[k] = (uint8_t)G.sinc_site[k];
         sm_sinc_sidx[k] = G.sinc_sidx[k]; sm_sinc_al[k] = G.sinc_al[k];
     }
-    for (int q = tid; q < n_adj; q += CH_THREADS) sm_adj[q] = (uint16_t)G.adj[q];
     for (int f = tid; f < n_front0; f += CH_THREADS) sm_front[0][f] = (uint16_t)G.front[0][f];
     for (int i = tid; i < nh; i += CH_THREADS) sm_spos[i] = G.spos[i];
     for (int i = tid; i <= nh; i += CH_THREADS) sm_site_off[i] = G.site_off[i];
@@ -721,6 +630,7 @@
     V.adj = sm_adj; V.adj_off = sm_adj_off; V.front[0] = sm_front[0]; V.front[1] = sm_front[1];
     V.spos = sm_spos; V.site_off = sm_site_off; V.bestkey = sm_bestkey; V.site_cnt = sm_site_cnt; V.site_base = sm_site_base;
     V.active = sm_active;
+    build_adjacency(V, P, n_inc, n_sinc);
     bfs_levels(V, nh, n_inc, n_front0);
     for (int p = tid; p < P; p += CH_THREADS) G.label[p] = sm_label[p];
 }
diff --git a/unfazed_b200/engine.py b/unfazed_b200/engine.py
--- a/unfazed_b200/engine.py
+++ b/unfazed_b200/engine.py
@@ -13,6 +13,17 @@
 from . import _lib as L
 from .plan import Plan
 from .schema import ReadTable, SiteTable, min_base_qual
+
+
+def _scan_launches(n: int) -> int:
+    return 1 if n <= 2048 else 2 + _scan_launches((n + 2047) // 2048)
+
+
+def _chain_tally_launches(totals, no_extended: bool) -> int:
+    cap_inc, cap_sinc = int(totals[1]), int(totals[3])
+    if no_extended:
+        return 3
+    return 3 + ((2 + _scan_launches(cap_inc)) if cap_inc > 0 else 0) + (1 if cap_inc + cap_sinc > 0 else 0)
 
 
 def make_params(ab_homref=(0.0, 0.2), ab_homalt=(0.8, 1.0), ab_het=(0.2, 0.8), min_gt_qual=20, min_depth=10,
@@ -493,7 +504,7 @@
             e.add("cand_list", 4 * n_pairs_)
             if has_reads:
                 e.add("site_lo", 4 * n_pairs_)
-                e.add("site_n", 4 * n_pairs_)
+                e.add("site_coff", 4 * n_pairs_)
                 e.add("seed_win", 16 * n)
             z.add("cand_evid", n_pairs_ + 8)
             if want_ev:
@@ -568,7 +579,7 @@
                 b.blk_maxspan, b.need, b.off = z1.ptr["blk_maxspan"], z1.ptr["need"], z1.ptr["off"]
                 b.rsum = e1.ptr["rsum"]
                 b.tile_tot, b.tile_base, b.tile_info = e1.ptr["tile_tot"], e1.ptr["tile_base"], e1.ptr["tile_info"]
-                b.site_lo, b.site_n, b.seed_win = e2.ptr["site_lo"], e2.ptr["site_n"], e2.ptr["seed_win"]
+                b.site_lo, b.site_coff, b.seed_win = e2.ptr["site_lo"], e2.ptr["site_coff"], e2.ptr["seed_win"]
                 b.hits, b.scratch, b.scratch_bytes = e3.ptr["hits"], e3.ptr["scratch"], nbytes
                 b.slot_label, b.slot_evid = z3.ptr["slot_label"], z3.ptr["slot_evid"]
                 if want_ev:
@@ -581,7 +592,7 @@
                 self._check(lib.unfz_run_batch_graph(ctx, C.byref(b), spans, len(zs), None, None, 0, s), "run_batch_graph")
             else:
                 self._check(lib.unfz_run_batch(ctx, C.byref(b), s), "run_batch")
-            launches += (22 if has_reads else 11) + (2 if want_ev else 0)
+            launches += (19 + _chain_tally_launches(caps["chain"], params.no_extended) if has_reads else 11) + (2 if want_ev else 0)
             h_pair_off, h_off = None, None
             res = BatchResult(plan=plan, n_pairs=int(caps["pairs"]), n_hits=int(caps["hits"]) if has_reads else 0,
                               seg_row_lo=None, seg_pair_off=None, n_het=None, n_cand=None, cnv_dad=None, cnv_mom=None)
@@ -654,7 +665,7 @@
                 mark("scan_hits")
                 self._check(lib.unfz_chain_size(ctx, p_dnm, n, p_seg, z1.ptr["seg_pair_off"], sc, rc_, e1.ptr["rsum"],
                                                 z1.ptr["blk_maxspan"], e2.ptr["het_list"], rp["n_het"], e2.ptr["cand_list"],
-                                                rp["n_cand"], rp["win"], z1.ptr["need"], e2.ptr["site_lo"], e2.ptr["site_n"],
+                                                rp["n_cand"], rp["win"], z1.ptr["need"], e2.ptr["site_lo"], e2.ptr["site_coff"],
                                                 e2.ptr["seed_win"], s), "chain_size")
                 self._check(lib.unfz_exclusive_scan_rows_i64(ctx, z1.ptr["need"], off_ptr, 6, n, s), "scan(need)")
                 launches += 2
@@ -686,13 +697,13 @@
                 self._check(lib.unfz_chain_tally(ctx, p_dnm, n, p_seg, z1.ptr["seg_pair_off"], sc, rc_, e1.ptr["rsum"],
                                                  z1.ptr["blk_maxspan"], e3.ptr["hits"], e1.ptr["tile_base"], tile_reads, z1.ptr["mark_prefix"],
                                                  e2.ptr["het_list"],
-                                                 rp["n_het"], e2.ptr["cand_list"], rp["n_cand"], p_all, rp["win"], e2.ptr["site_lo"], e2.ptr["site_n"],
+                                                 rp["n_het"], e2.ptr["cand_list"], rp["n_cand"], p_all, rp["win"], e2.ptr["site_lo"], e2.ptr["site_coff"],
                                                  e2.ptr["seed_win"], off_ptr,
                                                  totals.ctypes.data, C.byref(params), e3.ptr["scratch"], nbytes,
                                                  z3.ptr["slot_label"], z3.ptr["slot_evid"], z2.ptr["cand_evid"], rp["tally"],
                                                  z1.ptr["ev_need"] if want_ev else None, s),
                             "chain_tally")
-                launches += 3
+                launches += _chain_tally_launches(totals, params.no_extended)
                 mark("chain_tally")
                 if want_ev:
                     self._check(lib.unfz_exclusive_scan_rows_i64(ctx, z1.ptr["ev_need"], z1.ptr["ev_off"], 4, n, s), "scan(ev)")
```
